# DedalusProject/dedalus

Measured on AMD Instinct MI355X. Metric: timesteps/sec, 3D Rayleigh-Benard 512x512x256 (Fourier x Fourier x Chebyshev, RK222), higher is better.
Workload: dtype f64; 1 GPU; 3-D Rayleigh-Benard IVP 512x512x256, dealias 3/2, RK222, fixed dt=0.001, Ra=2e6 Pr=1, example-script initial condition (fill_random seed 42); pencils=65536, rows_per_pencil_real=5156, parallelism=1 GPU

## Files before the change

### dedalus_amd/core/solvers.py

```python

import time

import os

import numpy as np

from . import operators as ops
from . import timesteppers as ts_mod
from .evaluator import Evaluator, SystemBuffer, _full_sep
from .field import Field
from .ivp_common import IVPLifecycle
from .polyop import flatten
from .problems import LinCtx

import logging
logger = logging.getLogger(__name__)


class SolverBase:
    def __init__(self, problem, **kw):
        self.problem = problem
        self.dist = dist = problem.dist
        self.ex = dist.executor
        self.variables = list(problem.variables)
# ... 816 lines not shown
            elif any(v.domain.by_axis[ax] is not None for ax in sep):
                return False
        return True

    def _enable_state_tiling(self):
        self.x_tiled = 0
        if not self._state_tiling_ok():
            return
        ex = self.ex
        mode = 2 if os.environ.get("DDH_X_TILED", "1") == "2" else 1
        self.sync_state_to_device()
        tmp = ex.empty((self.R, self.nx, self.ny))
        ex.tile_rows(self.X, tmp, self.R, self.nx, self.ny, True, self.R if mode == 2 else 0)
        ex.copy(self.X, tmp)
        del tmp
        sb = self.sysbuf
        sb.tiled = int(self.ny)
        sb.banded = int(self.R) if mode == 2 else 0
        for info in self.var_info:
            sb.ranges.append((info["row0"], info["rows"]))
            sb.valid[info["row0"]] = False
            if info["aliased"]:
                v = info["field"]
                v._tiled, v._nrows = sb, info["rows"]
                v._c = sb.state_rows(info["row0"], info["rows"])
        self.pack.set_state_tiled(mode)
        self.x_tiled = int(self.ny)
        self.x_banded = sb.banded

    def state_natural(self):
        return self.sysbuf.natural(self.ex)

    def rhs_tiling(self, lus):
        if getattr(self, "_rhs_tiling_problem", None) is None:
            self._rhs_tiling_problem = self._rhs_tiling_of_problem()
        if not self._rhs_tiling_problem:
            return 0
        for lu in ([lus] if isinstance(lus, (int, np.integer)) else list(lus)):
            info = self.pack.lu_info(lu)
            if info["forward"] != "lean" or not info["real"]:
                return 0
        return self._rhs_tiling_problem

    def _rhs_tiling_of_problem(self):
        ex = self.ex
        if (os.environ.get("DDH_NO_RHS_TILING") is not None or not getattr(self.pack, "supports_tiled_rhs", False)
                or self.nf != 2 or self.nx % 8 or self.ny % 8 or self.F_direct is None or self.P_id is None
                or self.real_grading is None or self.nx * self.ny < int(os.environ.get("DDH_RHS_TILING_MIN", 4 * 16384))
                or not hasattr(ex, "tiled_forward_ok")):
            return 0
        if self.F_const is not None and np.any(np.asarray(self._F_const_index) % (self.nx * self.ny) != 0):
            return 0
        tr = self.dist.transformer
        for einfo, _scale in self.F_direct.values():
            edom = einfo["eq"]["domain"]
            pos, b, spec = tr._steps(edom, edom.dealias)[0]
            if pos != 0 or not ex.tiled_forward_ok(spec, b, self.nx * self.ny, self.ny):
                return 0
        return int(self.ny)

    def untile_rows(self, vec, banded=False):
        R, nx, ny = self.R, self.nx, self.ny
        if banded:
            return vec.reshape(nx // 8, R, ny // 8, 8, 8).permute(1, 0, 3, 2, 4).contiguous().reshape(R, nx, ny)
        v = vec.reshape(R, nx // 8, ny // 8, 8, 8)
        if hasattr(v, "permute"):
            return v.permute(0, 1, 3, 2, 4).contiguous().reshape(R, nx, ny)
        return np.ascontiguousarray(np.transpose(v, (0, 1, 3, 2, 4))).reshape(R, nx, ny)

    def solve(self, lu, rhs, out):
        if getattr(self, "modal", None) is not None:
            a, b = self._modal_lus[lu]
            self.modal.solve(a, b, [rhs], [1.0], out)
        elif self.P_id is None:
            self.pack.solve(lu, rhs, out)
        elif hasattr(self.pack, "solve_recombined"):
            Y = self.ex.empty((self.R, self.nx, self.ny))
            self.pack.solve_recombined(lu, [rhs], [1.0], self.P_id, Y, out)
        else:
            Y = self.ex.empty((self.R, self.nx, self.ny))
            self.pack.solve(lu, rhs, Y)
            self.pack.matvec(self.P_id, Y, out)
        if getattr(self, "solve_probe", None) is not None:
            self._probe_record(lu, rhs, out, path="ddh_pencil_solve_recombined (one materialised right-hand side)")

    def _probe_record(self, lu, rhs, out, path, skip_rows=None, terms=1, zero_rows=None):
        probe = self.solve_probe
        a, b = self._lu_params[lu]
        if getattr(self, "x_tiled", 0):
            out = self.untile_rows(out, banded=bool(getattr(self, "x_banded", 0)))
        rec = dict(a=a, b=b, path=path, terms=int(terms), zero_rows=bool(zero_rows), skip_rows=skip_rows is not None,
                   rhs=[self.gather_pencil(rhs, "equations", gx, gy) for gx, gy in probe["groups"]],
                   x=[self.gather_pencil(out, "variables", gx, gy) for gx, gy in probe["groups"]])
        if skip_rows is not None:
            rec["skipped"] = [self.gather_rows_mask(skip_rows, "variables", gx, gy) for gx, gy in probe["groups"]]
        probe["records"].append(rec)

    def zero_rows_host(self):
        if self.F_direct is None:
            return None
        mask = np.ones(self.R, dtype=np.uint8)
        mask[np.unique(np.asarray(self.M_tl.row))] = 0
        for einfo, _scale in self.F_direct.values():
            mask[einfo["row0"]:einfo["row0"] + einfo["rows"]] = 0
        if self.F_const is not None:
            mask[self._F_const_rows] = 0
        return mask

    def skip_rows_host(self):
        used = set()
        for einfo in self.eq_info:
            F = einfo["eq"]["F"]
            if F is not None and hasattr(F, "leaves"):
                used |= {id(f) for f in F.leaves()}
        mask = np.zeros(self.R, dtype=np.uint8)
        mcols = np.zeros(self.R, dtype=bool)
        mcols[np.unique(np.asarray(self.M_tl.col))] = True
        for info in self.var_info:
            r0, r1 = info["row0"], info["row0"] + info["rows"]
            if id(info["field"]) not in used and not mcols[r0:r1].any():
                mask[r0:r1] = 1
        return mask

    def _device_mask(self, mask):
        t = self.ex.torch
        return (t.as_tensor(mask, device=self.ex.dev.tdev), float(mask.mean()))

    def mx_f_zero_rows(self):
        if getattr(self, "_zrows", "unset") != "unset":
            return self._zrows
        self._zrows = None
        if not getattr(self.pack, "supports_zero_rows", False) or self.P_id is None:
            return None
        if os.environ.get("DDH_NO_ZERO_ROWS") is not None:
            return None
        mask = self.zero_rows_host()
        if mask is not None and mask.any():
            self._zrows = self._device_mask(mask)
        return self._zrows

    def intermediate_skip_rows(self):
        if getattr(self, "_skiprows", "unset") != "unset":
            return self._skiprows
        self._skiprows = None
        if not getattr(self.pack, "supports_zero_rows", False) or self.P_id is None or self.F_direct is None:
            return None
        if os.environ.get("DDH_NO_SKIP_ROWS") is not None:
            return None
        mask = self.skip_rows_host()
        if mask.any():
            self._skiprows = self._device_mask(mask)
        return self._skiprows

    def solve_lincomb(self, lu, xs, alphas, out, zero_rows=None, skip_rows=None, tiled=False):
        probe = getattr(self, "solve_probe", None)
        if getattr(self, "modal", None) is not None and probe is None and len(xs) <= self.modal.MAX_RHS_TERMS and not tiled:
            a, b = self._modal_lus[lu]
            self.modal.solve(a, b, xs, alphas, out)
            return
        if getattr(self, "modal", None) is not None:
            if tiled:
                raise RuntimeError("tile-major right-hand sides need the fused recombined solve")
            rhs = self.ex.empty((self.R, self.nx, self.ny))
            self.ex.lincomb(rhs, xs, alphas)
            self._last_rhs = rhs
            return self.solve(lu, rhs, out)
        if tiled and (self.P_id is None or not hasattr(self.pack, "solve_recombined") or len(xs) > self.pack.MAX_RHS_TERMS):
            raise RuntimeError("tile-major right-hand sides need the fused recombined solve")
        if len(xs) > self.pack.MAX_RHS_TERMS or not hasattr(self.pack, "solve_lincomb"):
            rhs = self.ex.empty((self.R, self.nx, self.ny))
            self.ex.lincomb(rhs, xs, alphas)
            self._last_rhs = rhs
            return self.solve(lu, rhs, out)
        rhs_rec = None
        if probe is not None:
            rhs_rec = self.ex.empty((self.R, self.nx, self.ny))
            self.ex.lincomb(rhs_rec, xs, alphas)
            if tiled:
                rhs_rec = self.untile_rows(rhs_rec)
            self._last_rhs = rhs_rec
        path = "ddh_pencil_solve_lincomb"
        if self.P_id is None:
            self.pack.solve_lincomb(lu, xs, alphas, out)
        elif hasattr(self.pack, "solve_recombined"):
            Y = self.ex.empty((self.R, self.nx, self.ny))
            if tiled:
                self.pack.solve_recombined(lu, xs, alphas, self.P_id, Y, out, zero_rows=zero_rows, skip_rows=skip_rows,
                                           tiled=True)
                path = "ddh_pencil_solve_recombined_tiled"
            elif zero_rows is not None or skip_rows is not None:
                self.pack.solve_recombined(lu, xs, alphas, self.P_id, Y, out, zero_rows=zero_rows, skip_rows=skip_rows)
                path = "ddh_pencil_solve_recombined_sparse"
            else:
                self.pack.solve_recombined(lu, xs, alphas, self.P_id, Y, out)
                path = "ddh_pencil_solve_recombined"
        else:
            Y = self.ex.empty((self.R, self.nx, self.ny))
            self.pack.solve_lincomb(lu, xs, alphas, Y)
            self.pack.matvec(self.P_id, Y, out)
        if probe is not None:
            skip_h = None
            if skip_rows is not None:
                skip_h = np.asarray(skip_rows[0].cpu().numpy() if hasattr(skip_rows[0], "cpu") else skip_rows[0], dtype=np.uint8)
            self._probe_record(lu, rhs_rec, out, path + " (%d fused terms%s%s)" % (
                len(xs), ", zero_rows" if zero_rows is not None else "", ", skip_rows" if skip_rows is not None else ""),
                skip_rows=skip_h, terms=len(xs), zero_rows=zero_rows is not None)
        if skip_rows is not None and os.environ.get("DDH_POISON_SKIPPED") is not None:
            t = self.ex.torch
            idx = t.nonzero(skip_rows[0]).flatten()
            if getattr(self, "x_banded", 0):
                out.reshape(self.nx // 8, self.R, -1)[:, idx] = float("nan")
            else:
                out.reshape(self.R, -1)[idx] = float("nan")

    def gather_pencil(self, vec, which, gx, gy=0):
        lx = gx - (self.dist._mx_offset if self.nf >= 1 else 0)
        cx = slice(2 * lx, 2 * lx + 2) if self.nf >= 1 else slice(0, 1)
        cy = slice(2 * gy, 2 * gy + 2) if self.nf >= 2 else slice(0, 1)
        slab = vec.reshape(self.R, self.nx, self.ny)[:, cx, cy]
        cell = np.array(self.ex.download(slab.contiguous() if hasattr(slab, "contiguous") else slab), dtype=float)
        cell = cell.reshape(self.R, cell.shape[-2], cell.shape[-1])
        if which != "variables" and self.eq_Tinv is not None:
            rows = self._eq_T_rows
            cell[rows] = (self.eq_Tinv[rows][:, rows] @ cell[rows].reshape(len(rows), -1)).reshape(cell[rows].shape)
        return self._gather_cell(cell, which, gx, gy)

    def gather_rows_mask(self, mask, which, gx, gy=0):
        wx = 2 if self.nf >= 1 else 1
        wy = 2 if self.nf >= 2 else 1
        cell = np.broadcast_to(np.asarray(mask, dtype=float)[:, None, None], (self.R, wx, wy))
        return self._gather_cell(cell, which, gx, gy) != 0

    def _gather_cell(self, cell, which, gx, gy):
        infos = self.var_info if which == "variables" else self.eq_info
        parts = []
        for info in infos:
            bits = info["bits"]
            if self.nf >= 1:
                sx = slice(0, 2) if (bits & 1) else (slice(0, 1) if gx == 0 else slice(0, 0))
            else:
                sx = slice(0, 1)
            if self.nf >= 2:
                sy = slice(0, 2) if (bits & 2) else (slice(0, 1) if gy == 0 else slice(0, 0))
            else:
                sy = slice(0, 1)
            blk = cell[info["row0"]:info["row0"] + info["rows"]].reshape(info["ncomp"], info["nz"], cell.shape[1], cell.shape[2])
            blk = blk[:, :, sx, sy].transpose(0, 2, 3, 1)
            if self.nf < 2:
                blk = blk[:, :, 0, :] if self.nf == 1 else blk[:, 0, 0, :]
            parts.append(np.ascontiguousarray(blk).ravel())
        return np.concatenate(parts)

    def factor(self, a, b, reuse=-1):
        if getattr(self, "modal", None) is not None:
            if reuse >= 0:
                lu = reuse
                self._modal_lus[lu] = (float(a), float(b))
            else:
                lu = len(self._modal_lus)
                self._modal_lus.append((float(a), float(b)))
            self.__dict__.setdefault("_lu_params", {})[lu] = (float(a), float(b))
            return lu
        self.factor_calls = getattr(self, "factor_calls", 0) + 1
        lu = self.pack.factor(self.MP_id, self.LP_id, a, b, self.row_perm, self.col_perm, self.n_interior,
                              self.kl, self.ku, self.row_axes, self.col_axes, reuse=reuse,
                              real=self.real_grading)
        if not hasattr(self, "_lu_params"):
            self._lu_params = {}
        self._lu_params[lu] = (float(a), float(b))
        self._block_inverses(lu, a, b)
        return lu

    def _block_inverse_plan(self, any_executor=False):
        if getattr(self, "_binv", None) is not None:
            return self._binv
        self._binv = False
        rg, n = self.real_grading, self.n_interior
        if not getattr(self, "allow_block_inverse", False):
            return False
        if os.environ.get("DDH_BLOCK_INVERSE", "1") == "0" or self.nf != 1 or rg is None or getattr(self.dist, "size", 1) > 1 or n < 128:
            return False
        if not any_executor and (getattr(self.ex, "name", "") != "hip" or not hasattr(self.pack, "set_block_inverse")):
            return False
        ns = self.n_blocks if (self.n_blocks > 1 and len(set(self.block_sizes)) == 1 and os.environ.get("DDH_SPLIT_THREADS", "1") != "0") else 1
        nh = n // ns
        ncells = self.nx // 2
        nb = self.R - n
        if nb and (np.any(self.row_axes[self.row_perm[n:]] & 1) or np.any(self.col_axes[self.col_perm[n:]] & 1)):
            return False
        ng = ncells * ns
        if ns * nh != n or nh > 1024 or ng * nh * nh * 8 > 2.5e9 or ng * (nh + 112) * (nh + 63) * 8 > 3e9:
            return False
        rinv, cinv = np.empty(self.R, dtype=np.int64), np.empty(self.R, dtype=np.int64)
        rinv[self.row_perm] = np.arange(self.R)
        cinv[self.col_perm] = np.arange(self.R)
        kx = np.asarray(self.pack.kx, dtype=np.float64)[:ncells]
        gmx = np.arange(ncells) + self.dist._mx_offset
        sel = []
        for mid in (rg["matM"], rg["matL"]):
            tl = self.pack.matrices[mid]
            i, j = rinv[tl.row], cinv[tl.col]
            ok = (i < n) & (j < n)
            if np.any(ok & (i // nh != j // nh)):
                return False
            sel.append((tl, i, j, ok))
        kl_b = max(int((i[ok] - j[ok]).max()) if ok.any() else 0 for (_, i, j, ok) in sel)
        ku_b = max(int((j[ok] - i[ok]).max()) if ok.any() else 0 for (_, i, j, ok) in sel)
        klT, kuT = max(ku_b, 0), max(kl_b, 0)
        if klT > 35 or klT + kuT > 96:
            return False
        W = klT + kuT + 1
        bands = []
        for (tl, i, j, ok) in sel:
            B = np.zeros((ng, nh, W))
            t = np.flatnonzero(ok)
            val = tl.coef[t].real[None, :] * kx[:, None] ** tl.ex[t].astype(float)[None, :]
            val = np.where((tl.dx[t] != 0)[None, :] & (gmx != 0)[:, None], 0.0, val)
            blk, ii, jj = i[t] // nh, i[t] % nh, j[t] % nh
            g = np.arange(ncells)[:, None] * ns + blk[None, :]
            np.add.at(B, (g, np.broadcast_to(jj, g.shape), np.broadcast_to(ii - jj + klT, g.shape)), val)
            bands.append(B)
        plan = type("BlockBandPlan", (), {})()
        plan.nl, plan.nmax, plan.kl, plan.ku, plan.mp, plan.nbc = ng, nh, klT, kuT, 0, 0
        plan.n = np.full(ng, nh, dtype=np.int32)
        plan.nbc_of = np.zeros(ng, dtype=np.int32)
        plan.T = np.zeros((ng, 1, 1))
        plan.P = np.zeros((ng, nh, 1))
        plan.MB, plan.LB = bands
        plan.row_index = plan.col_index = None
        self._binv = dict(plan=plan, ns=ns, nh=nh, ng=ng, ncells=ncells, dev=None, rhs=None, x={}, n_set=None)
        return self._binv

    def _drop_block_inverses(self, bi=None):
        bi = bi if isinstance(bi, dict) else getattr(self, "_binv", None)
        if isinstance(bi, dict):
            for k in list(bi["x"]):
                self.pack.set_block_inverse(k, None)
            bi["x"] = {}

    def _block_inverses(self, lu, a, b):
        bi = self._block_inverse_plan()
        if not bi:
            return
        ex, plan, ns, nh, ng = self.ex, bi["plan"], bi["ns"], bi["nh"], bi["ng"]
        self.pack.set_block_inverse(lu, None)
        info = self.pack.lu_info(lu)
        if info["nsplit"] != ns or info["rows_per_block"] != nh or not info["real"] or info["pair"]:
            self._drop_block_inverses(bi)
            self._binv = False
            return
        flagged = sorted(getattr(self.pack, "flagged", {}).get(lu, []))
        nb = self.R - self.n_interior
        if nb:
            k0 = np.flatnonzero(np.arange(bi["ncells"]) + self.dist._mx_offset == 0)
            if any(int(c) not in flagged for c in k0):
                return
        if bi["dev"] is None or bi["n_set"] != flagged:
            self._drop_block_inverses(bi)
            plan.n = np.full(ng, nh, dtype=np.int32)
            for cell in flagged:
                plan.n[cell * ns:(cell + 1) * ns] = 0
            rowoff = np.broadcast_to(np.arange(nh, dtype=np.int64)[None, :] * nh, (ng, nh))
            coloff = np.arange(ng, dtype=np.int64)[:, None] * (nh * nh) + np.arange(nh, dtype=np.int64)[None, :] * nh
            try:
                bi["dev"] = ex.make_ell_band(plan, 1, nh, ng, nh, [nh] * ng, offsets=(rowoff, coloff, 1))
            except Exception as e:
                logger.info("block inverses not available (%s): the sweeps stay" % (e,))
                self._binv = False
                return
            bi["rhs"] = ex.from_host(np.eye(nh))
            bi["n_set"] = flagged
            logger.info("LHS of %d pencils: explicit inverses of %d x %d diagonal blocks (%d rows), %.2f GB per factorization"
                        % (bi["ncells"], ng, ns, nh, ng * nh * nh * 8 / 1e9))
        if lu not in bi["x"]:
            if len(bi["x"]) >= 2:
                return
            bi["x"][lu] = (len(bi["x"]), ex.zeros((ng, nh, nh)))
        idx, x = bi["x"][lu]
        try:
            bi["dev"].factor(a, b, index=idx)
        except Exception as e:
            logger.warning("block inverses switched off (%s)" % (e,))
            self._drop_block_inverses(bi)
            self._binv = False
            return
        bi["dev"].solve(idx, bi["rhs"], x)
        if not self._block_inverse_residual_ok(bi, idx, x, a, b):
            self._drop_block_inverses(bi)
            self._binv = False
            return
        self.pack.set_block_inverse(lu, x)

    def _block_inverse_residual_ok(self, bi, idx, x, a, b, tol=1e-8):
        if os.environ.get("DDH_BLOCK_INVERSE_CHECK", "1") == "0":
            return True
        plan, nh = bi["plan"], bi["nh"]
        live = np.flatnonzero(plan.n > 0)
        if live.size == 0:
            return True
        worst = left = 0.0
        for g in sorted({int(live[0]), int(live[live.size // 2]), int(live[-1])}):
            band = a * plan.MB[g] + b * plan.LB[g]
            Bt = np.zeros((nh, nh))
            for d in range(band.shape[1]):
                off = d - plan.kl
                i = np.arange(max(0, -off), min(nh, nh - off))
                Bt[i, i + off] = band[i, d]
            Xg = self.ex.download(x[g])
            scale = max(1.0, float(np.abs(Bt).max()))
            worst = max(worst, float(np.abs(Bt @ Xg - np.eye(nh)).max()) / scale)
            left = max(left, float(np.abs(Xg @ Bt - np.eye(nh)).max()))
        bi["residual"], bi["left_residual"] = worst, left
        if not (worst <= tol):
            logger.warning("explicit block inverses: ||B^T X - I|| = %.1e > %.0e, the sweeps stay" % (worst, tol))
            return False
        return True


def _two_colour(n, row, col, label):
    from collections import deque
    adj_r = [[] for _ in range(n)]
    adj_c = [[] for _ in range(n)]
    seen = {}
    for r, c, l in zip(row.tolist(), col.tolist(), np.asarray(label).tolist()):
        key = (r, c)
        if key in seen:
            if seen[key] != l:
                return None
            continue
        seen[key] = l
        adj_r[r].append((c, l))
        adj_c[c].append((r, l))
    xr = np.full(n, -1, dtype=int)
    xc = np.full(n, -1, dtype=int)
    for start in range(n):
        if xr[start] != -1 or not adj_r[start]:
            continue
        xr[start] = 0
        dq = deque([("r", start)])
        while dq:
            kind, i = dq.popleft()
            if kind == "r":
                for c, l in adj_r[i]:
                    want = (l - xr[i]) % 2
                    if xc[c] == -1:
                        xc[c] = want
                        dq.append(("c", c))
                    elif xc[c] != want:
                        return None
            else:
                for r, l in adj_c[i]:
                    want = (l - xc[i]) % 2
                    if xr[r] == -1:
                        xr[r] = want
                        dq.append(("r", r))
                    elif xr[r] != want:
                        return None
    xr[xr == -1] = 0
    xc[xc == -1] = 0
    return xr, xc


def _matrix_times_termlist(T, tl):
    from ..pencilpack import TermList
    if tl.nterms == 0:
        return tl
    T = T.tocsc()
    ident = np.ones(T.shape[0], dtype=bool)
    coo = T.tocoo()
    off = (coo.row != coo.col) | (coo.data != 1.0)
    ident[coo.row[off]] = False
    ident[coo.col[off]] = False
    plain = ident[tl.row]
    parts = [[tl.row[plain]], [tl.col[plain]], [tl.coef[plain]], [tl.ex[plain]], [tl.ey[plain]], [tl.dx[plain]], [tl.dy[plain]]]
    for t in np.flatnonzero(~plain):
        c = T.getcol(int(tl.row[t])).tocoo()
        n = c.nnz
        parts[0].append(c.row); parts[1].append(np.full(n, tl.col[t])); parts[2].append(c.data * tl.coef[t])
        for k, name in enumerate(("ex", "ey", "dx", "dy")):
            parts[3 + k].append(np.full(n, getattr(tl, name)[t]))
    out = TermList(tl.nrows, tl.ncols, *[np.concatenate(x) for x in parts])
    if (~plain).any():
        out = out.consolidated(0.0)
        rowmax = np.zeros(tl.nrows)
        np.maximum.at(rowmax, out.row, np.abs(out.coef))
        keep = ident[out.row] | (np.abs(out.coef) > 1e-14 * rowmax[out.row])
        out = TermList(out.nrows, out.ncols, out.row[keep], out.col[keep], out.coef[keep], out.ex[keep], out.ey[keep],
                       out.dx[keep], out.dy[keep])
    return out


def _termlist_times_matrix(tl, P, cutoff=1e-12):
    from scipy import sparse
    from ..pencilpack import TermList
    if tl.nterms == 0:
        return tl
    key = np.stack([tl.ex, tl.ey, tl.dx, tl.dy], axis=1).astype(np.int64)
    uniq, inv = np.unique(key, axis=0, return_inverse=True)
    inv = inv.ravel()
    rows, cols, coefs, exs = [], [], [], []
    for u in range(len(uniq)):
        sel = inv == u
        A = sparse.coo_matrix((tl.coef[sel], (tl.row[sel], tl.col[sel])), shape=(tl.nrows, tl.ncols)).tocsr()
        AP = (A @ P).tocoo()
        keep = np.abs(AP.data) > cutoff * (np.abs(AP.data).max() if AP.nnz else 1.0)
        rows.append(AP.row[keep]); cols.append(AP.col[keep]); coefs.append(AP.data[keep])
        exs.append(np.tile(uniq[u], (int(keep.sum()), 1)))
    e = np.concatenate(exs)
    return TermList(tl.nrows, tl.ncols, np.concatenate(rows), np.concatenate(cols), np.concatenate(coefs),
                    e[:, 0], e[:, 1], e[:, 2], e[:, 3])


class InitialValueSolver(IVPLifecycle, SolverBase):

    def __init__(self, problem, timestepper, enforce_real_cadence=100, warmup_iterations=10, **kw):
        t0 = time.time()
        SolverBase.__init__(self, problem, **kw)
        self._enable_state_tiling()
        self.sim_time_field = problem.time
        self._sim_time = 0.0
        self._init_lifecycle(enforce_real_cadence, warmup_iterations)
        if isinstance(timestepper, str):
            timestepper = ts_mod.schemes[timestepper]
        self.allow_block_inverse = True
        self.timestepper = timestepper(self)
        self.setup_time = time.time() - t0
        self.total_modes = self.R * self.nx * self.ny
        state_ids = {id(v) for v in self.variables}
        rhs_fields, opaque = set(), False
        for eq in self.equations:
            F = eq["F"]
            if F is None or isinstance(F, (int, float, complex)):
                continue
            if hasattr(F, "leaves"):
                rhs_fields |= {id(f) for f in F.leaves() if not getattr(f, "_is_number", False)}
            else:
                opaque = True
        if not opaque and rhs_fields <= state_ids:
            self.step_graph_auto_modes = 1 << 22
        self.handlers = []
        from .output import OutputEvaluator
        self.evaluator = OutputEvaluator(self)
        self._step_hooks = [self.evaluator.step_hook]

    @property
    def sim_time(self):
        return self._sim_time

    @sim_time.setter
    def sim_time(self, t):
        self._sim_time = float(t)
        self.sim_time_field["g"] = float(t)

    def _hermitian_round_trip(self, f):
        if self.dist.size > 1 and any(b is None for b in f.domain.by_axis):
            return
        scales = f.scales
        f.require_grid_space(f.domain.dealias)
        f.require_coeff_space()
        f.change_scales(scales)


class LinearBoundaryValueSolver(SolverBase):

    _lu = None

    def solve(self, rebuild_matrices=False):
        self.sync_state_to_device()
        if getattr(self, "_F_lbvp", None) is None:
            self._F_lbvp = self.ex.empty((self.R, self.nx, self.ny))
        F = self._F_lbvp
# ... 6 lines not shown
```

### dedalus_amd/core/timesteppers.py

```python

import math
from collections import deque

import numpy as np

schemes = {}


def add_scheme(cls):
    schemes[cls.__name__] = cls
    return cls


def _fd_weights(nodes, x0, deriv):
    nodes = np.asarray(nodes, dtype=np.longdouble) - np.longdouble(x0)
    n = len(nodes)
    V = np.vander(nodes, n, increasing=True).T
    rhs = np.zeros(n, dtype=np.longdouble)
    rhs[deriv] = math.factorial(deriv)
    return _solve_ld(V, rhs)


def _solve_ld(A, b):
    A = np.array(A, dtype=np.longdouble)
    b = np.array(b, dtype=np.longdouble)
    n = len(b)
    for k in range(n):
        p = k + int(np.argmax(np.abs(A[k:, k])))
        if p != k:
            A[[k, p]] = A[[p, k]]
            b[[k, p]] = b[[p, k]]
        for i in range(k + 1, n):
            m = A[i, k] / A[k, k]
            A[i, k:] -= m * A[k, k:]
            b[i] -= m * b[k]
    x = np.zeros(n, dtype=np.longdouble)
    for k in range(n - 1, -1, -1):
        x[k] = (b[k] - A[k, k + 1:] @ x[k + 1:]) / A[k, k]
    return x.astype(np.float64)


def _times(timesteps, n):
    t = [0.0]
    for j in range(n):
        t.append(t[-1] - timesteps[j])
    return t



class _SolveMixin:
    _RHS = None

    @property
    def RHS(self):
        if self._RHS is None:
            s = self.solver
            self._RHS = s.ex.zeros((s.R, s.nx, s.ny))
        return self._RHS

    def _solve_combination(self, xs, al, lu, zero_rows=None, skip_rows=None, tiled=False):
        s = self.solver
        if hasattr(s, "solve_lincomb"):
            if tiled:
                s.solve_lincomb(lu, xs, al, s.X, zero_rows=zero_rows, skip_rows=skip_rows, tiled=True)
            elif zero_rows is not None or skip_rows is not None:
                s.solve_lincomb(lu, xs, al, s.X, zero_rows=zero_rows, skip_rows=skip_rows)
            else:
                s.solve_lincomb(lu, xs, al, s.X)
        else:
            s.ex.lincomb(self.RHS, xs, al)
            s.solve(lu, self.RHS, s.X)


class MultistepIMEX(_SolveMixin):
    stages = 1

    def __init__(self, solver):
        self.solver = solver
        ex, shape = solver.ex, (solver.R, solver.nx, solver.ny)
        self.dt = deque([0.0] * self.steps)
        self.MX = deque(ex.zeros(shape) for _ in range(self.amax))
        self.F = deque(ex.zeros(shape) for _ in range(self.cmax))
        if hasattr(solver, "_F_zeroed"):
            solver._F_zeroed = set()
        self._iteration = 0
        self._LHS_params = None
        self._lu = -1
        self._need_lx = False
        for it in range(self.steps + 1):
            _, b, _ = self.compute_coefficients([1.0] * self.steps, it)
            self._need_lx = self._need_lx or bool(np.any(np.asarray(b)[1:] != 0.0))
        self.LX = deque((ex.zeros(shape) if self._need_lx else None) for _ in range(self.bmax))

    def graph_phase(self, dt):
        if self._iteration < self.steps + 1 or any(h != dt for h in self.dt):
            return None
        period = int(np.lcm.reduce([len(self.MX), len(self.LX), len(self.F)]))
        return period, self._iteration % period

    def graph_snapshot(self):
        return (list(self.dt), self._iteration, list(self.MX), list(self.LX), list(self.F), self._LHS_params, self._lu)

    def graph_rollback(self, snap):
        dts, self._iteration, mx, lx, f, self._LHS_params, self._lu = snap
        self.dt, self.MX, self.LX, self.F = deque(dts), deque(mx), deque(lx), deque(f)

    def graph_advance(self, dt):
        self.dt.rotate()
        self.dt[0] = dt
        self._iteration += 1
        self.MX.rotate()
        self.LX.rotate()
        self.F.rotate()

    def step(self, dt, wall_time=None):
        s = self.solver
        ex, pack = s.ex, s.pack
        self.dt.rotate()
        self.dt[0] = dt
        a, b, c = self.compute_coefficients(list(self.dt), self._iteration)
        self._iteration += 1
        self.MX.rotate()
        self.LX.rotate()
        self.F.rotate()
        s.sync_state_to_device()
        pack.matvec(s.M_id, s.X, self.MX[0])
        if self._need_lx:
            pack.matvec(s.L_id, s.X, self.LX[0])
        s.evaluate_F(self.F[0], persistent=True)
        xs, al = [], []
        for j in range(1, len(c)):
            if c[j] != 0.0:
                xs.append(self.F[j - 1]); al.append(c[j])
        for j in range(1, len(a)):
            if a[j] != 0.0:
                xs.append(self.MX[j - 1]); al.append(-a[j])
        for j in range(1, len(b)):
            if b[j] != 0.0:
                xs.append(self.LX[j - 1]); al.append(-b[j])
        if (a[0], b[0]) != self._LHS_params:
            self._lu = s.factor(a[0], b[0], reuse=self._lu)
            self._LHS_params = (a[0], b[0])
        self._solve_combination(xs, al, self._lu)
        s.mark_state_current()
        s.sim_time = s.sim_time + dt


def _pad(v, n):
    out = np.zeros(n + 1)
    out[:len(v)] = v
    return out


@add_scheme
class CNAB1(MultistepIMEX):
    amax = bmax = cmax = steps = 1

    @classmethod
    def compute_coefficients(cls, timesteps, iteration):
        k0 = timesteps[0]
        a = _fd_weights(_times(timesteps, 1), 0.0, 1)
        return _pad(a, cls.amax), _pad([0.5, 0.5], cls.bmax), _pad([0.0, 1.0], cls.cmax)


@add_scheme
class SBDF1(MultistepIMEX):
    amax = bmax = cmax = steps = 1

    @classmethod
    def compute_coefficients(cls, timesteps, iteration):
        a = _fd_weights(_times(timesteps, 1), 0.0, 1)
        return _pad(a, cls.amax), _pad([1.0], cls.bmax), _pad([0.0, 1.0], cls.cmax)


def _adams_bashforth(timesteps, order):
    t = _times(timesteps, order)
    nodes = np.array(t[1:order + 1], dtype=np.longdouble)
    k = np.longdouble(timesteps[0])
    V = np.vander(nodes, order, increasing=True).T
    p = np.arange(order, dtype=np.longdouble)
    rhs = (np.longdouble(t[0]) ** (p + 1) - np.longdouble(t[1]) ** (p + 1)) / (p + 1) / k
    return np.concatenate([[0.0], _solve_ld(V, rhs)])


def _extrapolation(timesteps, order):
    t = _times(timesteps, order)
    w = _fd_weights(t[1:order + 1], t[0], 0)
    return np.concatenate([[0.0], w])


@add_scheme
class CNAB2(MultistepIMEX):
    amax = bmax = cmax = steps = 2

    @classmethod
    def compute_coefficients(cls, timesteps, iteration):
        if iteration < 1:
            a, b, c = CNAB1.compute_coefficients(timesteps, iteration)
            return _pad(a, 2), _pad(b, 2), _pad(c, 2)
        a = _fd_weights(_times(timesteps, 1), 0.0, 1)
        return _pad(a, 2), _pad([0.5, 0.5], 2), _pad(_adams_bashforth(timesteps, 2), 2)


@add_scheme
class MCNAB2(MultistepIMEX):
    amax = bmax = cmax = steps = 2

    @classmethod
    def compute_coefficients(cls, timesteps, iteration):
        if iteration < 1:
            a, b, c = CNAB1.compute_coefficients(timesteps, iteration)
            return _pad(a, 2), _pad(b, 2), _pad(c, 2)
        w = timesteps[0] / timesteps[1]
        a = _fd_weights(_times(timesteps, 1), 0.0, 1)
        b = [(8 + 1 / w) / 16, (7 - 1 / w) / 16, 1 / 16]
        return _pad(a, 2), _pad(b, 2), _pad(_adams_bashforth(timesteps, 2), 2)


class _SBDF(MultistepIMEX):
    @classmethod
    def _coeffs(cls, timesteps, order, size):
        a = _fd_weights(_times(timesteps, order), 0.0, 1)
        return _pad(a, size), _pad([1.0], size), _pad(_extrapolation(timesteps, order), size)


@add_scheme
class SBDF2(_SBDF):
    amax = bmax = cmax = steps = 2

    @classmethod
    def compute_coefficients(cls, timesteps, iteration):
        order = min(2, iteration + 1)
        return cls._coeffs(timesteps, order, 2)


@add_scheme
class CNLF2(MultistepIMEX):
    amax = bmax = cmax = steps = 2

    @classmethod
    def compute_coefficients(cls, timesteps, iteration):
        if iteration < 1:
            a, b, c = CNAB1.compute_coefficients(timesteps, iteration)
            return _pad(a, 2), _pad(b, 2), _pad(c, 2)
        t = _times(timesteps, 2)
        w = timesteps[0] / timesteps[1]
        a = _fd_weights(t, t[1], 1)
        b = [1 / w / 2, (1 - 1 / w) / 2, 1 / 2]
        return _pad(a, 2), _pad(b, 2), _pad([0.0, 1.0], 2)


@add_scheme
class SBDF3(_SBDF):
    amax = bmax = cmax = steps = 3

    @classmethod
    def compute_coefficients(cls, timesteps, iteration):
        order = min(3, iteration + 1)
        return cls._coeffs(timesteps, order, 3)


@add_scheme
class SBDF4(_SBDF):
    amax = bmax = cmax = steps = 4

    @classmethod
    def compute_coefficients(cls, timesteps, iteration):
        order = min(4, iteration + 1)
        return cls._coeffs(timesteps, order, 4)



class RungeKuttaIMEX(_SolveMixin):
    steps = 1

    def __init__(self, solver):
        import os
        self.solver = solver
        ex, shape = solver.ex, (solver.R, solver.nx, solver.ny)
        H = self.H
        self.MX0 = ex.zeros(shape)
        self.F = [ex.zeros(shape) for _ in range(self.stages)]
        if hasattr(solver, "_F_zeroed"):
            solver._F_zeroed = set()
        self._need_lx = [any(H[m, j] != 0.0 for m in range(j + 1, self.stages + 1)) for j in range(self.stages + 1)]
        self._direct = os.environ.get("DDH_RK_DIRECT_LX", "0") == "1"
        self.LX = [ex.zeros(shape) if (self._need_lx[j] and (self._direct or j == 0)) else None
                   for j in range(self.stages + 1)]
        self.MX = [None] + [ex.zeros(shape) if (self._need_lx[j] and not self._direct) else None
                            for j in range(1, self.stages + 1)]
        self._k = None
        self._lus = {}

    def step(self, dt, wall_time=None):
        s = self.solver
        ex, pack = s.ex, s.pack
        k = dt
        A, H, c = self.A, self.H, self.c
        if k != self._k:
            old = self._lus
            self._lus = {}
            reuse = list(old.values())
            for i in range(1, self.stages + 1):
                h = float(H[i, i])
                if h not in self._lus:
                    self._lus[h] = s.factor(1.0, k * h, reuse=(reuse.pop() if reuse else -1))
            self._k = k
        t0 = s.sim_time
        s.sync_state_to_device()
        own = dict(owned=True) if getattr(pack, "supports_zero_rows", False) else {}
        stamp = (tuple(self._lus.values()), getattr(pack, "variant_epoch", 0))
        if getattr(self, "_tiled_stamp", None) != stamp:
            tiled_now = 0
            if own and not self._direct and not any(v is not None for v in self.LX) and hasattr(s, "rhs_tiling"):
                tiled_now = s.rhs_tiling(self._lus.values())
            if getattr(self, "_tiled", None) is not None and bool(tiled_now) != bool(self._tiled):
                for buf in [self.MX0] + self.F + [v for v in self.MX if v is not None]:
                    ex.fill_zero(buf)
                s._F_zeroed = set(b.data_ptr() if hasattr(b, "data_ptr") else id(b) for b in self.F)
            self._tiled, self._tiled_stamp = tiled_now, stamp
        tiled = self._tiled
        if tiled:
            own = dict(owned=True, tiled=True)
        later = []
        defer_mv = bool(getattr(s, "overlaps_rhs_work", lambda: False)())
        (later.append if defer_mv else (lambda f: f()))(lambda: pack.matvec(s.M_id, s.X, self.MX0, **own))
        combs = {}
        for i in range(1, self.stages + 1):
            j = i - 1
            if self._need_lx[j]:
                if self._direct or j == 0:
                    mv = (lambda j=j: pack.matvec(s.L_id, s.X, self.LX[j]))
                else:
                    mv = (lambda j=j: pack.matvec(s.M_id, s.X, self.MX[j], **own))
                (later.append if defer_mv else (lambda f: f()))(mv)
            if later:
                s._overlap_work = list(later)
                del later[:]
            if tiled:
                s.evaluate_F(self.F[i - 1], persistent=True, tiled_row=tiled)
            else:
                s.evaluate_F(self.F[i - 1], persistent=True)
            comb = {("MX0",): 1.0}
            for j in range(i):
                if A[i, j] != 0.0:
                    comb[("F", j)] = comb.get(("F", j), 0.0) + k * A[i, j]
                if H[i, j] != 0.0:
                    if self._direct or j == 0:
                        comb[("LX", j)] = comb.get(("LX", j), 0.0) - k * H[i, j]
                    else:
                        r = H[i, j] / H[j, j]
                        for key, v in combs[j].items():
                            comb[key] = comb.get(key, 0.0) - r * v
                        comb[("MX", j)] = comb.get(("MX", j), 0.0) + r
            combs[i] = comb
            vec = {"MX0": lambda q: self.MX0, "F": lambda q: self.F[q], "LX": lambda q: self.LX[q], "MX": lambda q: self.MX[q]}
            xs = [vec[key[0]](key[1] if len(key) > 1 else None) for key, v in comb.items() if v != 0.0]
            al = [v for v in comb.values() if v != 0.0]
            zrows = None
            if not any(key[0] == "LX" and v != 0.0 for key, v in comb.items()) and hasattr(s, "mx_f_zero_rows"):
                zrows = s.mx_f_zero_rows()
            skip = None
            if i < self.stages and not self._direct and hasattr(s, "intermediate_skip_rows"):
                skip = s.intermediate_skip_rows()
            self._solve_combination(xs, al, self._lus[float(H[i, i])], zero_rows=zrows, skip_rows=skip, tiled=bool(tiled))
            s.mark_state_current()
            s.sim_time = t0 + k * c[i]


@add_scheme
class RK111(RungeKuttaIMEX):
    stages = 1
    c = np.array([0.0, 1.0])
    A = np.array([[0.0, 0.0], [1.0, 0.0]])
    H = np.array([[0.0, 0.0], [0.0, 1.0]])


@add_scheme
class RK222(RungeKuttaIMEX):
    stages = 2
    _g = 1.0 - np.sqrt(0.5)
    _d = 1.0 - 1.0 / (2.0 * _g)
    c = np.array([0.0, _g, 1.0])
    A = np.array([[0.0, 0.0, 0.0], [_g, 0.0, 0.0], [_d, 1.0 - _d, 0.0]])
    H = np.array([[0.0, 0.0, 0.0], [0.0, _g, 0.0], [0.0, 1.0 - _g, _g]])


@add_scheme
class RK443(RungeKuttaIMEX):
    stages = 4
    c = np.array([0.0, 1 / 2, 2 / 3, 1 / 2, 1.0])
    A = np.array([[0, 0, 0, 0, 0],
                  [1 / 2, 0, 0, 0, 0],
                  [11 / 18, 1 / 18, 0, 0, 0],
                  [5 / 6, -5 / 6, 1 / 2, 0, 0],
                  [1 / 4, 7 / 4, 3 / 4, -7 / 4, 0]], dtype=float)
    H = np.array([[0, 0, 0, 0, 0],
                  [0, 1 / 2, 0, 0, 0],
                  [0, 1 / 6, 1 / 2, 0, 0],
                  [0, -1 / 2, 1 / 2, 1 / 2, 0],
                  [0, 3 / 2, -3 / 2, 1 / 2, 1 / 2]], dtype=float)


@add_scheme
class RKSMR(RungeKuttaIMEX):
    stages = 3
    _al = (29 / 96, -3 / 40, 1 / 6)
    _be = (37 / 160, 5 / 24, 1 / 6)
    _ga = (8 / 15, 5 / 12, 3 / 4)
    _ze = (0.0, -17 / 60, -5 / 12)
    c = np.array([0.0, 8 / 15, 2 / 3, 1.0])
    A = np.zeros((4, 4))
    H = np.zeros((4, 4))
    for _i in range(1, 4):
        for _j in range(1, _i + 1):
            A[_i, _j - 1] += _ga[_j - 1]
            if _j >= 2:
                A[_i, _j - 2] += _ze[_j - 1]
            H[_i, _j - 1] += _al[_j - 1]
            H[_i, _j] += _be[_j - 1]
    del _i, _j


class RKGFY(RungeKuttaIMEX):
    stages = 2
    c = np.array([0.0, 1.0, 1.0])
    A = np.array([[0, 0, 0], [1, 0, 0], [0.5, 0.5, 0]], dtype=float)
    H = np.array([[0, 0, 0], [0.5, 0.5, 0], [0.5, 0, 0.5]], dtype=float)
```

### dedalus_amd/csrc/ddh_pencil.hip

```cpp
#include "ddh_common.h"

#include <algorithm>
#include <cmath>
#include <cstdlib>
#include <type_traits>

namespace ddh {

constexpr int KLMAX = 16;
constexpr int NBMAX = 8;

struct PencilDev {
    int nf;
    int S;
    int nrows;
    long nx, ny;
    long ncx, ncy;
    long ncells;
    long G;
    long mx_offset;
    const double *kx, *ky;
    int xtile;
};

struct MatDev {
    int nrows_out;
    int nterms;
    const int *rowptr;
    const int *col;
    const double2 *coef;
    const unsigned *expo;
    const int *order;
    const double *band;
    const int *base;
};
constexpr int MV_W = 5;

struct PostSolve {
    int nz;
    int nbands;
    int off[4];
    const double *bands;
};

struct Matrix {
    MatDev dev;
    std::vector<int> row_h, col_h;
    std::vector<double2> coef_h;
    std::vector<unsigned> expo_h;
    void *d_rowptr = nullptr, *d_col = nullptr, *d_coef = nullptr, *d_expo = nullptr, *d_order = nullptr;
    void *d_band = nullptr, *d_base = nullptr;
};

struct LuDev {
    int n, nb, N, kl, ku, W, BW;
    int real;
    long GL;
    long nblk;
    int rows_aw;
    int pk, pk63;
    int kpad;
    void *Aw;
    void *Ab;
    unsigned char *piv;
    unsigned char *flag;
    double2 *scratch;
    const int *rowperm, *colperm;
    const unsigned char *row_axes, *col_axes;
    const unsigned char *row_code, *col_code;
    const double *pband;
    int nsplit, nh;
    long Gp;
    int pair;
    const int *wrow;
    const long *vcell;
    const int *vslot;
    const long *slot_cell;
    const int *rowperm2, *colperm2;
};

constexpr int PBW = 12;

struct LuFactor {
    LuDev dev;
    size_t bytes = 0;
    void *d_rowperm = nullptr, *d_colperm = nullptr, *d_raxes = nullptr, *d_caxes = nullptr;
    void *d_rcode = nullptr, *d_ccode = nullptr;
    int nflag = 0;
    std::vector<long> flag_cells;
    void *d_flag_cells = nullptr;
    void *d_inv = nullptr;
    void *d_dense_rhs = nullptr;
    std::vector<int> colperm_h;
    std::vector<unsigned char> ccode_h;
    void *d_rhs_tmp = nullptr;
    const double *d_binv = nullptr;
    void *d_pband = nullptr;
    void *d_vcell = nullptr, *d_vslot = nullptr, *d_rowperm2 = nullptr, *d_colperm2 = nullptr;
    void *d_wrow = nullptr;
    std::vector<long> slot_cells_h;
    void *d_slot_cell = nullptr;
    int pband_mat = -1;
};

struct PencilPack : HandleBase {
    PencilDev dev;
    void *d_kx = nullptr, *d_ky = nullptr;
    std::vector<Matrix *> mats;
    std::vector<LuFactor *> lus;
    std::vector<PostSolve> posts;
    std::vector<void *> post_mem;
    int coop_mode = 1, coop_fwd = -1, coop_cb = -1;
    std::vector<int> pair_rows, pair_cols;
    long pair_min = 0;
    int row_blocks = 1;
    std::vector<double> kx_h, ky_h;
    ~PencilPack() override;
};

static void free_lu(LuFactor *lu) {
    if (!lu) return;
    (void)hipFree(lu->dev.Aw);
    (void)hipFree(lu->dev.Ab);
    (void)hipFree(lu->dev.piv);
    (void)hipFree(lu->dev.flag);
    (void)hipFree(lu->dev.scratch);
    (void)hipFree(lu->d_rowperm);
    (void)hipFree(lu->d_colperm);
    (void)hipFree(lu->d_raxes);
    (void)hipFree(lu->d_caxes);
    (void)hipFree(lu->d_rcode);
    (void)hipFree(lu->d_ccode);
    (void)hipFree(lu->d_flag_cells);
    (void)hipFree(lu->d_inv);
    (void)hipFree(lu->d_dense_rhs);
    (void)hipFree(lu->d_pband);
    (void)hipFree(lu->d_rhs_tmp);
    (void)hipFree(lu->d_vcell);
    (void)hipFree(lu->d_vslot);
    (void)hipFree(lu->d_slot_cell);
    (void)hipFree(lu->d_rowperm2);
    (void)hipFree(lu->d_colperm2);
    (void)hipFree(lu->d_wrow);
    delete lu;
}

PencilPack::~PencilPack() {
    (void)hipFree(d_kx);
    (void)hipFree(d_ky);
    for (auto m : mats) {
        (void)hipFree(m->d_rowptr);
        (void)hipFree(m->d_col);
        (void)hipFree(m->d_coef);
        (void)hipFree(m->d_expo);
        if (m->d_order) (void)hipFree(m->d_order);
        if (m->d_band) (void)hipFree(m->d_band);
        if (m->d_base) (void)hipFree(m->d_base);
        delete m;
    }
    for (auto l : lus) free_lu(l);
    for (auto m : post_mem) (void)hipFree(m);
}

__device__ __forceinline__ double2 cmul(double2 a, double2 b) {
    return make_double2(a.x * b.x - a.y * b.y, a.x * b.y + a.y * b.x);
}
__device__ __forceinline__ void cfma(double2 &acc, double2 a, double2 b) {
    acc.x += a.x * b.x - a.y * b.y;
    acc.y += a.x * b.y + a.y * b.x;
}
__device__ __forceinline__ void cfms(double2 &acc, double2 a, double2 b) {
    acc.x -= a.x * b.x - a.y * b.y;
    acc.y -= a.x * b.y + a.y * b.x;
}
__device__ __forceinline__ double cabs2(double2 a) { return a.x * a.x + a.y * a.y; }
__device__ __forceinline__ double2 cinv(double2 a) {
    const double d = 1.0 / (a.x * a.x + a.y * a.y);
    return make_double2(a.x * d, -a.y * d);
}
__device__ __forceinline__ double ipow(double k, unsigned e) {
    double r = 1.0, b = k;
    if (e & 1u) r *= b;
    b *= b;
    if (e & 2u) r *= b;
    b *= b;
    if (e & 4u) r *= b;
    return r;
}

template <bool REAL> struct El;
template <> struct El<false> {
    typedef double2 T;
    static __device__ __forceinline__ T zero() { return make_double2(0.0, 0.0); }
    static __device__ __forceinline__ T one() { return make_double2(1.0, 0.0); }
    static __device__ __forceinline__ T mul(T a, T b) { return cmul(a, b); }
    static __device__ __forceinline__ T inv(T a) { return cinv(a); }
    static __device__ __forceinline__ double abs2(T a) { return cabs2(a); }
    static __device__ __forceinline__ bool is_zero(T a) { return a.x == 0.0 && a.y == 0.0; }
    static __device__ __forceinline__ void fms(T &acc, T m, T v) { cfms(acc, m, v); }
    static __device__ __forceinline__ void add(T &acc, double2 v) { acc.x += v.x; acc.y += v.y; }
    static __device__ __forceinline__ void fms2(double2 &acc, T m, double2 v) { cfms(acc, m, v); }
    static __device__ __forceinline__ void fma2(double2 &acc, T m, double2 v) { cfma(acc, m, v); }
    static __device__ __forceinline__ double2 mul2(double2 a, T m) { return cmul(a, m); }
    static __device__ __forceinline__ T scale(T a, double f) { return make_double2(a.x * f, a.y * f); }
};
template <> struct El<true> {
    typedef double T;
    static __device__ __forceinline__ T zero() { return 0.0; }
    static __device__ __forceinline__ T one() { return 1.0; }
    static __device__ __forceinline__ T mul(T a, T b) { return a * b; }
    static __device__ __forceinline__ T inv(T a) { return 1.0 / a; }
    static __device__ __forceinline__ double abs2(T a) { return a * a; }
    static __device__ __forceinline__ bool is_zero(T a) { return a == 0.0; }
    static __device__ __forceinline__ void fms(T &acc, T m, T v) { acc -= m * v; }
    static __device__ __forceinline__ void add(T &acc, double2 v) { acc += v.x; }
    static __device__ __forceinline__ void fms2(double2 &acc, T m, double2 v) { acc.x -= m * v.x; acc.y -= m * v.y; }
    static __device__ __forceinline__ void fma2(double2 &acc, T m, double2 v) { acc.x += m * v.x; acc.y += m * v.y; }
    static __device__ __forceinline__ double2 mul2(double2 a, T m) { return make_double2(a.x * m, a.y * m); }
    static __device__ __forceinline__ T scale(T a, double f) { return a * f; }
};

typedef unsigned ddh_u4v __attribute__((ext_vector_type(4)));
typedef unsigned ddh_u2v __attribute__((ext_vector_type(2)));
__device__ __forceinline__ __amdgpu_buffer_rsrc_t wave_rsrc(const void *first_lane_ptr) {
    const unsigned long long a = (unsigned long long)first_lane_ptr;
    const unsigned lo = __builtin_amdgcn_readfirstlane((unsigned)a);
    const unsigned hi = __builtin_amdgcn_readfirstlane((unsigned)(a >> 32));
    void *base = (void *)(((unsigned long long)hi << 32) | lo);
    return __builtin_amdgcn_make_buffer_rsrc(base, 0, 0xffffffff, 0x00020000);
}
__device__ __forceinline__ unsigned wave_lane_off(const void *lane_ptr) {
    const unsigned long long a = (unsigned long long)lane_ptr;
    const unsigned lo = __builtin_amdgcn_readfirstlane((unsigned)a);
    const unsigned hi = __builtin_amdgcn_readfirstlane((unsigned)(a >> 32));
    return (unsigned)(a - (((unsigned long long)hi << 32) | lo));
}
__device__ __forceinline__ double2 bload16(__amdgpu_buffer_rsrc_t r, unsigned lane_off, unsigned uni_off) {
    const ddh_u4v q = __builtin_amdgcn_raw_buffer_load_b128(r, lane_off, uni_off, 0);
    return make_double2(__hiloint2double((int)q.y, (int)q.x), __hiloint2double((int)q.w, (int)q.z));
}
__device__ __forceinline__ double bload8(__amdgpu_buffer_rsrc_t r, unsigned lane_off, unsigned uni_off) {
    const ddh_u2v q = __builtin_amdgcn_raw_buffer_load_b64(r, lane_off, uni_off, 0);
    return __hiloint2double((int)q.y, (int)q.x);
}

__device__ __forceinline__ long lu_eoff(const LuDev &L, int e) {
    return ((long)e << 6) - (long)(L.pk63 * (e & 1));
}
__device__ __forceinline__ long lu_aw(const LuDev &L, long gl, int row, int d) {
    return ((((gl >> 6) * (long)L.rows_aw + row) * L.BW) << 6) + lu_eoff(L, d + L.kpad) + ((gl & 63) << (L.pk ? 1 : 0));
}
__device__ __forceinline__ long lu_ab(const LuDev &L, long gl, int col, int rb) {
    return ((((gl >> 6) * (long)L.N + col) * L.nb + rb) << 6) + (gl & 63);
}
__device__ __forceinline__ long lu_pv(const LuDev &L, long gl, int row) {
    return (((gl >> 6) * (long)L.rows_aw + row) << 6) + (gl & 63);
}

struct CellCtx {
    long mx, my;
    long gmx;
    double kx, ky;
};

__device__ __forceinline__ CellCtx cell_ctx(const PencilDev &P, long cell) {
    CellCtx c;
    if (P.nf == 2) {
        c.mx = cell / P.ncy;
        c.my = cell % P.ncy;
    } else {
        c.mx = cell;
        c.my = 0;
    }
    c.gmx = c.mx + P.mx_offset;
    c.kx = (P.nf >= 1) ? P.kx[c.mx] : 0.0;
    c.ky = (P.nf == 2) ? P.ky[c.my] : 0.0;
    return c;
}

struct SysId {
    long cell, gl, G;
    int s;
    bool partner, ok;
};
template <bool REAL>
__device__ __forceinline__ SysId sys_id(const PencilDev &P, const LuDev &L, long g) {
    SysId id;
    id.partner = false;
    id.G = P.G;
    id.ok = g < P.G;
    id.cell = id.ok ? g / P.S : 0;
    id.s = (int)(g % P.S);
    if (L.pair) {
        const int vs = L.vslot[id.cell];
        id.gl = vs >> 1;
        id.partner = (vs & 1) != 0;
// ... 1339 lines not shown
        if (code & 1) v = make_double2(v.y, -v.x);
        return v;
    };

    double2 w[KLT + 1];
#pragma unroll
    for (int d = 0; d <= KLT; ++d) w[d] = make_double2(0.0, 0.0);
#pragma unroll 1
    for (int t = 0; t <= KLT; ++t) {
        const double2 v = (row0 + t < row1) ? load_row(row0 + t) : make_double2(0.0, 0.0);
#pragma unroll
        for (int d = 0; d < KLT; ++d) w[d] = w[d + 1];
        w[KLT] = v;
    }
    double2 gb[NBT];
#pragma unroll
    for (int rb = 0; rb < NBT; ++rb) gb[rb] = make_double2(0.0, 0.0);
#pragma unroll 1
    for (int t = 0; t < NBT; ++t) {
        const double2 v = (t < nb && blk == 0) ? load_row(n + t) : make_double2(0.0, 0.0);
#pragma unroll
        for (int rb = 0; rb + 1 < NBT; ++rb) gb[rb] = gb[rb + 1];
        gb[NBT - 1] = v;
    }
    double m[PD][KLT], ab[PD][NBT];
    int pv[PD];
    double2 raw[PD][NT];
#pragma unroll
    for (int d = 0; d < PD; ++d) {
        pv[d] = 0;
#pragma unroll
        for (int i = 0; i < KLT; ++i) m[d][i] = 0.0;
#pragma unroll
        for (int rb = 0; rb < NBT; ++rb) ab[d][rb] = 0.0;
#pragma unroll
        for (int t = 0; t < NT; ++t) raw[d][t] = make_double2(0.0, 0.0);
    }
    const long cell_off = rhs.tiled ? tile_offset(2 * c.mx + s, 2 * c.my, P.ny) : (2 * c.mx + s) * P.ny + 2 * c.my;
    const double *pt[NT];
    double at[NT];
#pragma unroll
    for (int t = 0; t < NT; ++t) {
        pt[t] = t < rhs.n ? rhs.p[t] : rhs.p[0];
        at[t] = t < rhs.n ? rhs.a[t] : 0.0;
    }
    auto request = [&](int jrow, double *mm, double *aa, int &p, double2 *q) {
        const unsigned jr = (unsigned)((jrow < row1 ? jrow : row1 - 1) - row0);
        const unsigned mo_j = jr * row_step8;
        p = pvp[(long)jr << 6];
#pragma unroll
        for (int i = 0; i < KLT; ++i) mm[i] = *reinterpret_cast<const double *>(awl + (mo_j + md[i]));
        const double *abj = abp + (long)jr * ab_step;
#pragma unroll
        for (int rb = 0; rb < NBT; ++rb) aa[rb] = abj[rb << 6];
        const int nxt = jrow + KLT + 1;
        const long off = (long)my_perm[nxt < row1 ? nxt : row1 - 1] * plane + cell_off;
#pragma unroll
        for (int t = 0; t < NT; ++t) q[t] = *reinterpret_cast<const double2 *>(pt[t] + off);
        __builtin_amdgcn_sched_barrier(0);
    };
    auto entering = [&](int jrow, const double2 *q) -> double2 {
        const int nxt = jrow + KLT + 1;
        if (nxt >= row1 || s_zero[nxt]) return make_double2(0.0, 0.0);
        double2 v;
        if (rhs.n == 1 && !rhs.tiled) {
            const double2 mine = q[0];
            double2 other;
            other.x = __shfl_xor(mine.x, 1);
            other.y = __shfl_xor(mine.y, 1);
            v = s == 0 ? make_double2(mine.x - other.y, mine.y + other.x) : make_double2(other.x + mine.y, other.y - mine.x);
            if (rhs.a[0] != 1.0) v = make_double2(rhs.a[0] * v.x, rhs.a[0] * v.y);
        } else {
            double2 mine = make_double2(0.0, 0.0);
#pragma unroll
            for (int t = 0; t < NT; ++t) {
                mine.x += at[t] * q[t].x;
                mine.y += at[t] * q[t].y;
            }
            double2 other;
            other.x = __shfl_xor(mine.x, 1);
            other.y = __shfl_xor(mine.y, 1);
            v = s == 0 ? make_double2(mine.x - other.y, mine.y + other.x) : make_double2(other.x + mine.y, other.y - mine.x);
        }
        if (conjq) v.y = -v.y;
        const unsigned char code = s_code[nxt];
        if ((code & 2) && s == 1) v = make_double2(-v.x, -v.y);
        if (code & 1) v = make_double2(v.y, -v.x);
        return v;
    };
    auto step = [&](const double *mm, const double *aa, int p, double2 rnew) {
        double2 yj = w[0];
#pragma unroll
        for (int d = 1; d <= KLT; ++d) {
            if (d == p) {
                yj = w[d];
                w[d] = w[0];
            }
        }
        *scr = yj;
        scr += G;
#pragma unroll
        for (int i = 1; i <= KLT; ++i) {
            w[i].x -= mm[i - 1] * yj.x;
            w[i].y -= mm[i - 1] * yj.y;
        }
#pragma unroll
        for (int rb = 0; rb < NBT; ++rb) {
            gb[rb].x -= aa[rb] * yj.x;
            gb[rb].y -= aa[rb] * yj.y;
        }
#pragma unroll
        for (int d = 0; d < KLT; ++d) w[d] = w[d + 1];
        w[KLT] = rnew;
    };
#pragma unroll
    for (int d = 0; d < PD; ++d) request(row0 + d, m[d], ab[d], pv[d], raw[d]);
    int j = row0;
    for (; j + PD - 1 < row1; j += PD) {
#pragma unroll
        for (int d = 0; d < PD; ++d) {
            const double2 rnew = entering(j + d, raw[d]);
            step(m[d], ab[d], pv[d], rnew);
            request(j + d + PD, m[d], ab[d], pv[d], raw[d]);
        }
    }
#pragma unroll
    for (int d = 0; d < PD; ++d)
        if (j + d < row1) step(m[d], ab[d], pv[d], entering(j + d, raw[d]));
    if (L.nsplit > 1) {
#pragma unroll
        for (int r = 0; r < NBT; ++r)
            if (r < nb) L.scratch[(long)(n + nb + blk * nb + r) * G + g] = gb[r];
        return;
    }
    const double *Ab = (const double *)L.Ab;
#pragma unroll
    for (int r = 0; r < NBT; ++r) {
        if (r < nb) {
            double2 acc = make_double2(0.0, 0.0);
#pragma unroll
            for (int cidx = 0; cidx < NBT; ++cidx)
                if (cidx < nb) El<true>::fma2(acc, Ab[lu_ab(L, id.gl, n + cidx, r)], gb[cidx]);
            L.scratch[(long)(n + r) * G + g] = acc;
            double2 v = acc;
            const unsigned char code = s_code[N + r];
            if (code & 1) v = make_double2(-v.y, v.x);
            if ((code & 2) && s == 1) v = make_double2(-v.x, -v.y);
            if (conjq) v.y = -v.y;
            store_sys<NF>(xout, plane, my_perm[N + r], P, c, s, v);
        }
    }
}

template <int NF, int WT, bool REAL, bool PREF, bool PFUSE = false, int MINW = 1>
__global__ void __launch_bounds__(256, MINW)
solve_backward_kernel(PencilDev P, LuDev L, double *__restrict__ xout, const double *__restrict__ pband,
                      const unsigned char *__restrict__ skip) {
    typedef typename El<REAL>::T E;
    extern __shared__ int s_lds[];
    const int n = L.n, nb = L.nb, kl = L.kl, W = L.W;
    int *s_perm = s_lds;
    int *s_perm2 = s_lds + (L.pair ? n : 0);
    unsigned char *s_code = (unsigned char *)(s_perm2 + n);
    unsigned char *s_skip = s_code + n;
    unsigned char *s_nq = s_skip + n;
    for (int i = threadIdx.x; i < n; i += blockDim.x) {
        s_perm[i] = L.colperm[i];
        if (L.pair) s_perm2[i] = L.colperm2[i];
        s_code[i] = REAL ? L.col_code[i] : 0;
        s_skip[i] = skip ? (skip[L.colperm[i]] && (!L.pair || skip[L.colperm2[i]])) : 0;
        if (REAL) {
            const int full = (WT + 2) / 2;
            const int need = L.wrow ? (L.wrow[i] + 2) >> 1 : full;
            s_nq[i] = (unsigned char)(need < full ? need : full);
        }
    }
    __syncthreads();
    const int blk = (REAL && L.nsplit > 1) ? __builtin_amdgcn_readfirstlane((int)(((long)blockIdx.x * blockDim.x) / L.Gp)) : 0;
    const long g = (long)blockIdx.x * blockDim.x + threadIdx.x - (long)blk * L.Gp;
    const int row0 = (REAL && L.nsplit > 1) ? blk * L.nh : 0, row1 = (REAL && L.nsplit > 1) ? row0 + L.nh : n;
    const SysId id = sys_id<REAL>(P, L, g);
    if (!id.ok) return;
    const int s = id.s;
    const CellCtx c = cell_ctx(P, id.cell);
    const long G = id.G;
    const long gl = id.gl;
    const int *my_perm = id.partner ? s_perm2 : s_perm;
    const bool conjq = id.partner && s == 1;
    const E *Aw = (const E *)L.Aw;
    const long plane = P.nx * P.ny;

    double2 win[WT];
#pragma unroll
    for (int d = 0; d < WT; ++d) {
        win[d] = make_double2(0.0, 0.0);
        if (d < nb && row1 == n) win[d] = L.scratch[(long)(n + d) * G + g];
    }
    E ua[WT + 1], ub[WT + 1];
    double pa[PBW], pb[PBW];
    double2 ya = make_double2(0.0, 0.0), yb = ya;
#pragma unroll
    for (int d = 0; d < PBW; ++d) pa[d] = pb[d] = 0.0;
#pragma unroll
    for (int d = 0; d <= WT; ++d) ua[d] = ub[d] = El<REAL>::zero();
    constexpr bool FULL = REAL;
    const E *const ur0 = Aw + lu_aw(L, gl, 0, kl);
    const long ur_stride = (long)L.BW << 6;
    const double2 *const y0 = L.scratch + g;
    const __amdgpu_buffer_rsrc_t ur_rs = wave_rsrc(ur0);
    const unsigned ur_lane = wave_lane_off(ur0);
    const __amdgpu_buffer_rsrc_t y_rs = wave_rsrc(y0);
    const unsigned y_lane = wave_lane_off(y0);
    const unsigned ur_row8 = (unsigned)L.BW << 9, y_row16 = (unsigned)(G * (long)sizeof(double2));
    auto fetch = [&](int j, E *u, double2 &y, double *pr) {
        if constexpr (REAL) y = bload16(y_rs, y_lane, (unsigned)j * y_row16);
        else y = y0[(long)j * G];
        if (PFUSE) {
            const double *prow = pband + (long)j * PBW;
#pragma unroll
            for (int d = 0; d < PBW; ++d) pr[d] = prow[d];
        }
        const E *Ur = ur0 + (long)j * ur_stride;
        if constexpr (REAL) {
            const unsigned urow = (unsigned)j * ur_row8;
            constexpr int NQMIN = (WT >= 13) ? 6 : (WT + 2) / 2;
            const int nq = __builtin_amdgcn_readfirstlane((int)s_nq[j]);
#pragma unroll
            for (int q = 0; 2 * q <= WT; ++q) {
                double2 uu = make_double2(0.0, 0.0);
                if (q < NQMIN || q < nq) uu = bload16(ur_rs, ur_lane, urow + (unsigned)(q << 10));
                u[2 * q] = uu.x;
                if (2 * q + 1 <= WT) u[2 * q + 1] = uu.y;
            }
        } else {
#pragma unroll
            for (int d = 0; d <= WT; ++d)
                if (FULL || d <= W) u[d] = Ur[(long)d << 6];
        }
        __builtin_amdgcn_sched_barrier(0);
    };
    auto emit = [&](int j, double2 v) {
        if (s_skip[j]) return;
        if (REAL) {
            const unsigned char code = s_code[j];
            if (code & 1) v = make_double2(-v.y, v.x);
            if ((code & 2) && s == 1) v = make_double2(-v.x, -v.y);
        }
        if (conjq) v.y = -v.y;
        store_sys<NF>(xout, plane, my_perm[j], P, c, s, v);
    };
    auto row_even = [&](int j, const E *u, double2 y, const double *pr) -> double2 {
        double2 acc = y;
#pragma unroll
        for (int d = 0; d < WT; ++d)
            if (FULL || d < W) El<REAL>::fms2(acc, u[d + 1], win[d]);
        const double2 xj = El<REAL>::mul2(acc, u[0]);
        double2 v = xj;
        if (PFUSE) {
#pragma unroll
            for (int d = 0; d < PBW; ++d)
                if (d < WT) { v.x += pr[d] * win[d].x; v.y += pr[d] * win[d].y; }
        }
        emit(j, v);
        return xj;
    };
    auto row_odd = [&](int j, const E *u, double2 y, double2 xprev, const double *pr) {
        double2 acc = y;
        El<REAL>::fms2(acc, u[1], xprev);
#pragma unroll
        for (int d = 1; d < WT; ++d)
            if (FULL || d < W) El<REAL>::fms2(acc, u[d + 1], win[d - 1]);
        const double2 xj = El<REAL>::mul2(acc, u[0]);
        double2 v = xj;
        if (PFUSE) {
            v.x += pr[0] * xprev.x;
            v.y += pr[0] * xprev.y;
#pragma unroll
            for (int d = 1; d < PBW; ++d)
                if (d - 1 < WT) { v.x += pr[d] * win[d - 1].x; v.y += pr[d] * win[d - 1].y; }
        }
        emit(j, v);
#pragma unroll
        for (int d = WT - 1; d > 1; --d) win[d] = win[d - 2];
        win[1] = xprev;
        win[0] = xj;
    };
    int j = row1 - 1;
    if (PREF) {
        if (j >= row0) fetch(j, ua, ya, pa);
        while (j >= row0 + 1) {
            fetch(j - 1, ub, yb, pb);
            const double2 xe = row_even(j, ua, ya, pa);
            if (j - 2 >= row0) fetch(j - 2, ua, ya, pa);
            row_odd(j - 1, ub, yb, xe, pb);
            j -= 2;
        }
        if (j == row0) row_even(row0, ua, ya, pa);
    } else {
        while (j >= row0 + 1) {
            fetch(j, ua, ya, pa);
            const double2 xe = row_even(j, ua, ya, pa);
            fetch(j - 1, ua, ya, pa);
            row_odd(j - 1, ua, ya, xe, pa);
            j -= 2;
        }
        if (j == row0) {
            fetch(row0, ua, ya, pa);
            row_even(row0, ua, ya, pa);
        }
    }
}

template <int WT, int PD>
__global__ void __launch_bounds__(256, 1)
solve_backward_deep_kernel(PencilDev P, LuDev L, double *__restrict__ xout, const double *__restrict__ pband,
                           const unsigned char *__restrict__ skip) {
    constexpr int NF = 2;
    static_assert(PD >= 2 && PD % 2 == 0, "rows are processed in pairs");
    extern __shared__ int s_lds[];
    const int n = L.n, nb = L.nb, kl = L.kl;
    int *s_perm = s_lds;
    int *s_perm2 = s_lds + (L.pair ? n : 0);
    unsigned char *s_code = (unsigned char *)(s_perm2 + n);
    unsigned char *s_skip = s_code + n;
    for (int i = threadIdx.x; i < n; i += blockDim.x) {
        s_perm[i] = L.colperm[i];
        if (L.pair) s_perm2[i] = L.colperm2[i];
        s_code[i] = L.col_code[i];
        s_skip[i] = skip ? (skip[L.colperm[i]] && (!L.pair || skip[L.colperm2[i]])) : 0;
    }
    __syncthreads();
    const int blk = (L.nsplit > 1) ? __builtin_amdgcn_readfirstlane((int)(((long)blockIdx.x * blockDim.x) / L.Gp)) : 0;
    const long g = (long)blockIdx.x * blockDim.x + threadIdx.x - (long)blk * L.Gp;
    const int row0 = (L.nsplit > 1) ? blk * L.nh : 0, row1 = (L.nsplit > 1) ? row0 + L.nh : n;
    const SysId id = sys_id<true>(P, L, g);
    if (!id.ok) return;
    const int s = id.s;
    const CellCtx c = cell_ctx(P, id.cell);
    const long G = id.G;
    const int *my_perm = id.partner ? s_perm2 : s_perm;
    const bool conjq = id.partner && s == 1;
    const long plane = P.nx * P.ny;

    double2 win[WT];
#pragma unroll
    for (int d = 0; d < WT; ++d) {
        win[d] = make_double2(0.0, 0.0);
        if (d < nb && row1 == n) win[d] = L.scratch[(long)(n + d) * G + g];
    }
    constexpr int NQ = (WT + 2) / 2;
    ddh_u4v u[PD][NQ];
    double pr[PD][PBW];
    ddh_u4v yv[PD];
    const double *const ur0 = (const double *)L.Aw + lu_aw(L, id.gl, 0, kl);
    const double2 *const y0 = L.scratch + g;
    const __amdgpu_buffer_rsrc_t ur_rs = wave_rsrc(ur0);
    const unsigned ur_lane = wave_lane_off(ur0);
    const __amdgpu_buffer_rsrc_t y_rs = wave_rsrc(y0);
    const unsigned y_lane = wave_lane_off(y0);
    const unsigned ur_row8 = (unsigned)L.BW << 9, y_row16 = (unsigned)(G * (long)sizeof(double2));
    auto lo = [](const ddh_u4v &q) -> double { return __hiloint2double((int)q.y, (int)q.x); };
    auto hi = [](const ddh_u4v &q) -> double { return __hiloint2double((int)q.w, (int)q.z); };
    auto fetch = [&](int j, ddh_u4v *uu, ddh_u4v &y, double *p) {
        y = __builtin_amdgcn_raw_buffer_load_b128(y_rs, y_lane, (unsigned)j * y_row16, 0);
        const double *prow = pband + (long)j * PBW;
#pragma unroll
        for (int d = 0; d < PBW; ++d) p[d] = prow[d];
        const unsigned urow = (unsigned)j * ur_row8;
#pragma unroll
        for (int q = 0; q < NQ; ++q) uu[q] = __builtin_amdgcn_raw_buffer_load_b128(ur_rs, ur_lane, urow + (unsigned)(q << 10), 0);
        __builtin_amdgcn_sched_barrier(0);
    };
    auto emit = [&](int j, double2 v) {
        if (s_skip[j]) return;
        const unsigned char code = s_code[j];
        if (code & 1) v = make_double2(-v.y, v.x);
        if ((code & 2) && s == 1) v = make_double2(-v.x, -v.y);
        if (conjq) v.y = -v.y;
        store_sys<NF>(xout, plane, my_perm[j], P, c, s, v);
    };
    auto ent = [&](const ddh_u4v *uu, int e) -> double { return (e & 1) ? hi(uu[e >> 1]) : lo(uu[e >> 1]); };
    auto row_even = [&](int j, const ddh_u4v *uu, const ddh_u4v &yr, const double *p) -> double2 {
        double2 acc = make_double2(lo(yr), hi(yr));
#pragma unroll
        for (int d = 0; d < WT; ++d) El<true>::fms2(acc, ent(uu, d + 1), win[d]);
        const double2 xj = El<true>::mul2(acc, ent(uu, 0));
        double2 v = xj;
#pragma unroll
        for (int d = 0; d < PBW; ++d)
            if (d < WT) { v.x += p[d] * win[d].x; v.y += p[d] * win[d].y; }
        emit(j, v);
        return xj;
    };
    auto row_odd = [&](int j, const ddh_u4v *uu, const ddh_u4v &yr, double2 xprev, const double *p) {
        double2 acc = make_double2(lo(yr), hi(yr));
        El<true>::fms2(acc, ent(uu, 1), xprev);
#pragma unroll
        for (int d = 1; d < WT; ++d) El<true>::fms2(acc, ent(uu, d + 1), win[d - 1]);
        const double2 xj = El<true>::mul2(acc, ent(uu, 0));
        double2 v = xj;
        v.x += p[0] * xprev.x;
        v.y += p[0] * xprev.y;
#pragma unroll
        for (int d = 1; d < PBW; ++d)
            if (d - 1 < WT) { v.x += p[d] * win[d - 1].x; v.y += p[d] * win[d - 1].y; }
        emit(j, v);
#pragma unroll
        for (int d = WT - 1; d > 1; --d) win[d] = win[d - 2];
        win[1] = xprev;
        win[0] = xj;
    };
    int j = row1 - 1;
#pragma unroll
    for (int d = 0; d < PD; ++d) fetch(max(j - d, row0), u[d], yv[d], pr[d]);
    for (; j - (PD - 1) >= row0; j -= PD) {
#pragma unroll
        for (int d = 0; d < PD; d += 2) {
            const double2 xe = row_even(j - d, u[d], yv[d], pr[d]);
            fetch(max(j - d - PD, row0), u[d], yv[d], pr[d]);
            row_odd(j - d - 1, u[d + 1], yv[d + 1], xe, pr[d + 1]);
            fetch(max(j - d - 1 - PD, row0), u[d + 1], yv[d + 1], pr[d + 1]);
        }
    }
#pragma unroll
    for (int d = 0; d < PD; d += 2) {
        if (j - d - 1 >= row0) {
            const double2 xe = row_even(j - d, u[d], yv[d], pr[d]);
            row_odd(j - d - 1, u[d + 1], yv[d + 1], xe, pr[d + 1]);
        } else if (j - d >= row0) {
            row_even(j - d, u[d], yv[d], pr[d]);
        }
    }
}

// ... 244 lines not shown
            pu[slot][t] = u_ptr[(dd << 6) - pk63 * (dd & 1)];
        }
        const bool adv = jj > row0;
        u_ptr -= adv ? aw_rs : 0;
        y_ptr -= adv ? G : 0;
    };
#pragma unroll
    for (int r = 0; r < PD; ++r) issue(row1 - 1 - r, r);
#define DDH_COOP_BWD_ROW(r, j)                                                                                     \
    {                                                                                                              \
        E u[TT];                                                                                                   \
        const int ej = (h - (j) - 1) & (CB - 1);                                                                   \
        _Pragma("unroll") for (int t = 0; t < TT; ++t) u[t] = (1 + ej + CB * t <= W) ? pu[r][t] : El<REAL>::zero(); \
        const E u0 = pu0[r];                                                                                       \
        const double2 y = py[r];                                                                                   \
        issue((j) - PD, r);                                                                                    \
        double2 acc = make_double2(0.0, 0.0);                                                                      \
        _Pragma("unroll") for (int t = 0; t < TT; ++t) El<REAL>::fma2(acc, u[t], xr[t]);                           \
        acc.x = group_sum<CB>(acc.x);                                                                                  \
        acc.y = group_sum<CB>(acc.y);                                                                                  \
        const double2 xj = El<REAL>::mul2(make_double2(y.x - acc.x, y.y - acc.y), u0);                             \
        double2 v = xj;                                                                                            \
        if (REAL) {                                                                                                \
            const unsigned char code = s_code[j];                                                                  \
            if (code & 1) v = make_double2(-v.y, v.x);                                                             \
            if ((code & 2) && s == 1) v = make_double2(-v.x, -v.y);                                                \
        }                                                                                                          \
        store_sys<NF, CB>(xout, plane, s_perm[j], P, c, s, v);       \
        if ((((j) - h) & (CB - 1)) == 0) {                       \
            _Pragma("unroll") for (int t = TT - 1; t > 0; --t) xr[t] = xr[t - 1];                                  \
            xr[0] = xj;                                                                                            \
        }                                                                                                          \
    }
    int jt0 = 0;
    const int nrows = row1 - row0;
    for (; jt0 + PD <= nrows; jt0 += PD) {
#pragma unroll
        for (int r = 0; r < PD; ++r) DDH_COOP_BWD_ROW(r, row1 - 1 - (jt0 + r))
    }
#pragma unroll
    for (int r = 0; r < PD; ++r)
        if (jt0 + r < nrows) DDH_COOP_BWD_ROW(r, row1 - 1 - (jt0 + r))
#undef DDH_COOP_BWD_ROW
}

template <int NF>
__global__ void __launch_bounds__(256)
dense_gather_kernel(PencilDev P, LuDev L, const long *__restrict__ cells, int ncellsf,
                    const RhsSrc rhs, double2 *__restrict__ out) {
    const long t = (long)blockIdx.x * blockDim.x + threadIdx.x;
    const long per = (long)L.N * P.S;
    if (t >= per * ncellsf) return;
    const long f = t / per;
    const int i = (int)((t % per) / P.S);
    const int s = (int)(t % P.S);
    const CellCtx c = cell_ctx(P, cells[f]);
    const double2 v = load_sys<NF>(rhs, P.nx * P.ny, L.rowperm[i], P, c, s);
    out[(f * P.S + s) * L.N + i] = v;
}

__global__ void __launch_bounds__(256)
dense_apply_kernel(int N, const double2 *__restrict__ inv, const double2 *__restrict__ rhs, double2 *__restrict__ x) {
    const int sys = blockIdx.y;
    const int row = blockIdx.x * 4 + (threadIdx.x >> 6);
    const int lane = threadIdx.x & 63;
    if (row >= N) return;
    const double2 *a = inv + ((long)sys * N + row) * N;
    const double2 *b = rhs + (long)sys * N;
    double2 acc = make_double2(0.0, 0.0);
    for (int k = lane; k < N; k += 64) cfma(acc, a[k], b[k]);
    for (int off = 32; off > 0; off >>= 1) {
        acc.x += __shfl_down(acc.x, off);
        acc.y += __shfl_down(acc.y, off);
    }
    if (lane == 0) x[(long)sys * N + row] = acc;
}

template <int NF>
__global__ void __launch_bounds__(256)
dense_scatter_kernel(PencilDev P, LuDev L, const long *__restrict__ cells, int ncellsf,
                     const double2 *__restrict__ xin, double *__restrict__ xout, int apply_p) {
    const long t = (long)blockIdx.x * blockDim.x + threadIdx.x;
    const long per = (long)L.N * P.S;
    if (t >= per * ncellsf) return;
    const long f = t / per;
    const int i = (int)((t % per) / P.S);
    const int s = (int)(t % P.S);
    const CellCtx c = cell_ctx(P, cells[f]);
    const double2 *xs = xin + (f * P.S + s) * L.N;
    double2 v = xs[i];
    if (apply_p && L.pband && i < L.n) {
        const double *pr = L.pband + (long)i * PBW;
        for (int d = 1; d <= PBW; ++d)
            if (i + d < L.n) { v.x += pr[d - 1] * xs[i + d].x; v.y += pr[d - 1] * xs[i + d].y; }
    }
    store_sys<NF>(xout, P.nx * P.ny, L.colperm[i], P, c, s, v);
}

template <typename T>
static int upload_vec(void **dptr, const T *src, size_t count) {
    DDH_HIP(hipMalloc(dptr, count * sizeof(T) + 16));
    if (count) DDH_HIP(hipMemcpy(*dptr, src, count * sizeof(T), hipMemcpyHostToDevice));
    return 0;
}

__global__ void __launch_bounds__(1024)
blockinv_solve_kernel(PencilDev P, LuDev L, const RhsSrc rhs, const double *__restrict__ binv, double *__restrict__ yout) {
    extern __shared__ double2 s_rb[];
    const int nh = L.nh, ns = L.nsplit;
    const long cell = blockIdx.x / ns;
    const int blk = (int)(blockIdx.x - cell * ns);
    if (L.flag[cell]) return;
    const CellCtx c = cell_ctx(P, cell);
    const long plane = P.nx * P.ny;
    const int row0 = blk * nh, tid = threadIdx.x, NT = blockDim.x;
    for (int i = tid; i < nh; i += NT) {
        const int phys = L.rowperm[row0 + i];
        double2 v = make_double2(0.0, 0.0);
        if (!(rhs.zrow && rhs.zrow[phys])) v = load_sys<1>(rhs, plane, phys, P, c, 0);
        if (L.row_code[row0 + i] & 1) v = make_double2(v.y, -v.x);
        s_rb[i] = v;
    }
    __syncthreads();
    const double *B = binv + (size_t)blockIdx.x * nh * nh;
    for (int i = tid; i < nh; i += NT) {
        double2 acc = make_double2(0.0, 0.0);
        const double *bi = B + i;
        int k = 0;
        for (; k + 8 <= nh; k += 8) {
            double b[8];
#pragma unroll
            for (int q = 0; q < 8; ++q) b[q] = bi[(size_t)(k + q) * nh];
#pragma unroll
            for (int q = 0; q < 8; ++q) {
                const double2 r = s_rb[k + q];
                acc.x += b[q] * r.x;
                acc.y += b[q] * r.y;
            }
        }
        for (; k < nh; ++k) {
            const double b = bi[(size_t)k * nh];
            const double2 r = s_rb[k];
            acc.x += b * r.x;
            acc.y += b * r.y;
        }
        double2 v = acc;
        if (L.col_code[row0 + i] & 1) v = make_double2(-v.y, v.x);
        store_sys<1>(yout, plane, L.colperm[row0 + i], P, c, 0, v);
    }
    if (blk == 0)
        for (int r = tid; r < L.nb; r += NT) store_sys<1>(yout, plane, L.colperm[L.n + r], P, c, 0, make_double2(0.0, 0.0));
}

template <int NF>
static int finish_solve(PencilPack *pp, LuFactor *lu, const RhsSrc &rhs, double *x, hipStream_t s, int apply_p) {
    const PencilDev &P = pp->dev;
    const LuDev &d = lu->dev;
    if (lu->nflag) {
        if (!lu->d_inv) return fail("pencil_solve: flagged pencils need ddh_pencil_set_dense_inverse first");
        const int nsys = lu->nflag * P.S;
        double2 *drhs = (double2 *)lu->d_dense_rhs;
        double2 *dx = drhs + (size_t)nsys * d.N;
        const long work = (long)lu->nflag * d.N * P.S;
        const unsigned gb = (unsigned)((work + 255) / 256);
        hipLaunchKernelGGL(dense_gather_kernel<NF>, dim3(gb), dim3(256), 0, s, P, d, (const long *)lu->d_flag_cells,
                           lu->nflag, rhs, drhs);
        hipLaunchKernelGGL(dense_apply_kernel, dim3((unsigned)((d.N + 3) / 4), (unsigned)nsys), dim3(256), 0, s, d.N,
                           (const double2 *)lu->d_inv, (const double2 *)drhs, dx);
        hipLaunchKernelGGL(dense_scatter_kernel<NF>, dim3(gb), dim3(256), 0, s, P, d, (const long *)lu->d_flag_cells,
                           lu->nflag, (const double2 *)dx, x, apply_p);
        DDH_HIP(hipGetLastError());
    }
    return 0;
}

static int forward_window(int kl) { return kl <= 6 ? 6 : (kl <= 12 ? 12 : 16); }
static int backward_window(int W) { return W <= 17 ? 17 : (W <= 32 ? 32 : (W <= 34 ? 34 : (W <= 48 ? 48 : 64))); }

static bool lean_forward_ok(const LuDev &d) {
    return d.real && d.n > 0 && d.kpad + d.kl == forward_window(d.kl) && d.rows_aw >= d.n + forward_window(d.kl) &&
           d.kl <= 12 && d.nb <= 2;
}

static bool sweep_deep(const LuDev &d) {
    static const int env = getenv("DDH_SWEEP_DEEP") ? atoi(getenv("DDH_SWEEP_DEEP")) : -1;
    if (!d.real || d.n <= 0) return false;
    if (env >= 0) return env != 0;
    return (long)d.nsplit * d.Gp <= 2L * 1024 * 64;
}

static unsigned deep_block(long threads) {
    if (threads / 256 >= 256) return 256u;
    return threads / 128 >= 256 ? 128u : 64u;
}

enum class FwdSweep {
    coop,
    deep,
    lean_occ4,
    lean,
    general
};
enum class BwdSweep {
    none,
    coop,
    deep,
    fused_occ4,
    fused,
    plain
};
struct SweepPlan {
    FwdSweep fwd;
    int fwd_kl, fwd_nb;
    bool border_finish;
    BwdSweep bwd;
    int bwd_w;
    int cb, tt;
    bool fuse_p;
    dim3 fwd_grid, fwd_block, bwd_grid, bwd_block;
    size_t lds_f, lds_b;
    bool lean_forward() const { return fwd == FwdSweep::deep || fwd == FwdSweep::lean_occ4 || fwd == FwdSweep::lean; }
};

static SweepPlan sweep_plan(const PencilPack *pp, const LuDev &d, int nterms, bool want_p) {
    const PencilDev &P = pp->dev;
    const int NF = P.nf, W = d.W;
    SweepPlan pl{};
    const size_t per_entry = d.pair ? 9 : 5;
    pl.lds_f = (size_t)(d.N + d.nb) * (per_entry + 1) + 16;
    pl.lds_b = (size_t)(d.n > 0 ? d.n : 1) * (per_entry + 2) + 16;
    const unsigned blocks = (unsigned)((P.G + 255) / 256);
    const long threads = (long)d.nsplit * d.Gp;
    const unsigned blocks_split = (unsigned)((threads + 255) / 256);
    auto coop_grid = [&](int lanes) {
        return (d.real && d.nsplit > 1) ? (unsigned)(threads / (256 / lanes)) : (unsigned)((P.G + (256 / lanes) - 1) / (256 / lanes));
    };

    const int coop_mode = pp->coop_mode;
    const bool coop_auto = coop_mode == 1 && NF > 0;
    bool coop_fwd = coop_mode == 2 || (coop_auto && P.G <= 16384);
    int cb = 0;
    if (coop_mode == 2 || (coop_auto && P.G <= 1024)) cb = 16;
    else if (coop_auto && P.G <= 16384) cb = 4;
    if (coop_auto && d.nsplit > 1 && P.G > 4096) {
        coop_fwd = false;
        cb = 0;
    }
    if (pp->coop_fwd >= 0) coop_fwd = pp->coop_fwd != 0;
    if (pp->coop_cb >= 0) cb = pp->coop_cb;
    if (NF == 0 || d.kl >= CH || d.nb > 8) coop_fwd = false;
    if (NF == 0 || (cb != 4 && cb != 16)) cb = 0;
    if (cb && (W + cb - 1) / cb > (cb == 4 ? 12 : 3)) cb = 0;
    if (d.n <= 0 || d.pair) {
        coop_fwd = false;
        cb = 0;
    }

    pl.fwd_grid = dim3(blocks);
    pl.fwd_block = dim3(256);
    if (coop_fwd) {
        pl.fwd = FwdSweep::coop;
        pl.fwd_nb = d.nb <= 2 ? 2 : 8;
        pl.fwd_grid = dim3(coop_grid(CH));
        pl.border_finish = d.real && d.nsplit > 1 && d.nb > 0;
    } else if (NF == 2 && lean_forward_ok(d)) {
        const bool w6 = forward_window(d.kl) == 6;
        pl.fwd_kl = w6 ? 6 : 12;
        pl.fwd_nb = w6 && d.nb <= 1 ? 1 : 2;
        pl.fwd_grid = dim3(blocks_split);
        if (w6 && d.nb == 1 && nterms >= 1 && nterms <= 4 && sweep_deep(d)) {
            pl.fwd = FwdSweep::deep;
            pl.fwd_block = dim3(deep_block(threads));
            pl.fwd_grid = dim3(blocks_split * (256 / pl.fwd_block.x));
        } else if (w6 && d.nsplit > 1 && d.nb <= 1) {
            pl.fwd = FwdSweep::lean_occ4;
        } else {
            pl.fwd = FwdSweep::lean;
        }
        pl.border_finish = d.nsplit > 1 && d.nb > 0;
    } else {
        pl.fwd = FwdSweep::general;
        pl.fwd_kl = d.kl <= 12 ? 12 : 16;
        pl.fwd_nb = d.nb <= 2 ? 2 : 8;
    }

    pl.bwd_grid = dim3(blocks_split);
    pl.bwd_block = dim3(256);
    if (cb) {
        pl.bwd = BwdSweep::coop;
        pl.cb = cb;
        const int tt = (W + cb - 1) / cb;
        pl.tt = cb == 16 ? (tt <= 2 ? 2 : 3) : (tt <= 9 ? 9 : 12);
        pl.bwd_grid = dim3(coop_grid(cb));
    } else if (d.n <= 0) {
        pl.bwd = BwdSweep::none;
    } else if (NF == 2 && want_p && d.real && d.pband != nullptr && W <= 48) {
        pl.fuse_p = true;
        pl.bwd_w = backward_window(W);
        if (W <= 17 && sweep_deep(d)) {
            pl.bwd = BwdSweep::deep;
            pl.bwd_block = dim3(deep_block(threads));
            pl.bwd_grid = dim3(blocks_split * (256 / pl.bwd_block.x));
        } else if (W <= 17 && d.nsplit > 1) {
            pl.bwd = BwdSweep::fused_occ4;
        } else {
            pl.bwd = BwdSweep::fused;
        }
    } else {
        pl.bwd = BwdSweep::plain;
        pl.bwd_w = backward_window(W);
        if (!d.real) pl.bwd_grid = dim3(blocks);
    }
    return pl;
}

template <int NF>
static int launch_solve(PencilPack *pp, LuFactor *lu, const RhsSrc &rhs, double *x, hipStream_t s, const SweepPlan &pl) {
    const PencilDev &P = pp->dev;
    const LuDev &d = lu->dev;
    if (pl.lds_f > 64 * 1024) return fail("pencil_solve: system too large for the LDS permutation cache");
    const int kl = pl.fwd_kl, nb = pl.fwd_nb, w = pl.bwd_w;
    switch (pl.fwd) {
        case FwdSweep::coop:
            if constexpr (NF > 0) {
                const double *rhs1 = rhs.p[0];
                if (rhs.n != 1 || rhs.a[0] != 1.0) {
                    const long nel = (long)P.nrows * P.nx * P.ny;
                    if (!lu->d_rhs_tmp) DDH_HIP(hipMalloc(&lu->d_rhs_tmp, (size_t)nel * sizeof(double) + 16));
                    if (int st0 = ddh_lincomb((double *)lu->d_rhs_tmp, rhs.n, rhs.p, rhs.a, nel, (void *)s)) return st0;
                    rhs1 = (const double *)lu->d_rhs_tmp;
                }
                auto k = nb == 2 ? solve_forward_coop_kernel<NF, true, 2> : solve_forward_coop_kernel<NF, true, 8>;
                if (!d.real) k = nb == 2 ? solve_forward_coop_kernel<NF, false, 2> : solve_forward_coop_kernel<NF, false, 8>;
                hipLaunchKernelGGL(k, pl.fwd_grid, pl.fwd_block, pl.lds_f, s, P, d, rhs1, x);
            }
            break;
        case FwdSweep::deep:
            if constexpr (NF == 2)
                hipLaunchKernelGGL((solve_forward_deep_kernel<6, 1, 4, 4>), pl.fwd_grid, pl.fwd_block, pl.lds_f, s, P, d, rhs, x);
            break;
        case FwdSweep::lean_occ4:
            if constexpr (NF == 2)
                hipLaunchKernelGGL((solve_forward_lean_kernel<6, 1, 4>), pl.fwd_grid, pl.fwd_block, pl.lds_f, s, P, d, rhs, x);
            break;
        case FwdSweep::lean:
            if constexpr (NF == 2) {
                auto k = kl == 12 ? solve_forward_lean_kernel<12, 2>
                                  : (nb == 1 ? solve_forward_lean_kernel<6, 1> : solve_forward_lean_kernel<6, 2>);
                hipLaunchKernelGGL(k, pl.fwd_grid, pl.fwd_block, pl.lds_f, s, P, d, rhs, x);
            }
            break;
        case FwdSweep::general: {
            auto k = kl == 12 ? (nb == 2 ? solve_forward_kernel<NF, true, 12, 2> : solve_forward_kernel<NF, true, 12, 8>)
                              : (nb == 2 ? solve_forward_kernel<NF, true, 16, 2> : solve_forward_kernel<NF, true, 16, 8>);
            if (!d.real)
                k = kl == 12 ? (nb == 2 ? solve_forward_kernel<NF, false, 12, 2> : solve_forward_kernel<NF, false, 12, 8>)
                             : (nb == 2 ? solve_forward_kernel<NF, false, 16, 2> : solve_forward_kernel<NF, false, 16, 8>);
            hipLaunchKernelGGL(k, pl.fwd_grid, pl.fwd_block, pl.lds_f, s, P, d, rhs, x);
            break;
        }
    }
    if constexpr (NF > 0)
        if (pl.border_finish)
            hipLaunchKernelGGL(border_finish_kernel<NF>, dim3((unsigned)((P.G + 255) / 256)), dim3(256), 0, s, P, d, x);
    switch (pl.bwd) {
        case BwdSweep::none:
            break;
        case BwdSweep::coop:
            if constexpr (NF > 0) {
                auto k = pl.cb == 16 ? (pl.tt == 2 ? solve_backward_coop_kernel<NF, 2, true, 16> : solve_backward_coop_kernel<NF, 3, true, 16>)
                                     : (pl.tt == 9 ? solve_backward_coop_kernel<NF, 9, true, 4> : solve_backward_coop_kernel<NF, 12, true, 4>);
                if (!d.real)
                    k = pl.cb == 16 ? (pl.tt == 2 ? solve_backward_coop_kernel<NF, 2, false, 16> : solve_backward_coop_kernel<NF, 3, false, 16>)
                                    : (pl.tt == 9 ? solve_backward_coop_kernel<NF, 9, false, 4> : solve_backward_coop_kernel<NF, 12, false, 4>);
                hipLaunchKernelGGL(k, pl.bwd_grid, pl.bwd_block, pl.lds_b, s, P, d, x);
            }
            break;
        case BwdSweep::deep:
            if constexpr (NF == 2)
                hipLaunchKernelGGL((solve_backward_deep_kernel<17, 2>), pl.bwd_grid, pl.bwd_block, pl.lds_b, s, P, d, x, d.pband, rhs.skip);
            break;
        case BwdSweep::fused_occ4:
            if constexpr (NF == 2)
                hipLaunchKernelGGL((solve_backward_kernel<NF, 17, true, false, true, 4>), pl.bwd_grid, pl.bwd_block, pl.lds_b, s, P, d, x, d.pband, rhs.skip);
            break;
        case BwdSweep::fused:
            if constexpr (NF == 2) {
                auto k = w == 17 ? solve_backward_kernel<NF, 17, true, false, true> : w == 32 ? solve_backward_kernel<NF, 32, true, false, true>
                       : w == 34 ? solve_backward_kernel<NF, 34, true, false, true> : solve_backward_kernel<NF, 48, true, false, true>;
                hipLaunchKernelGGL(k, pl.bwd_grid, pl.bwd_block, pl.lds_b, s, P, d, x, d.pband, rhs.skip);
            }
            break;
        case BwdSweep::plain: {
            auto k = w == 17 ? solve_backward_kernel<NF, 17, true, false> : w == 32 ? solve_backward_kernel<NF, 32, true, false>
                   : w == 34 ? solve_backward_kernel<NF, 34, true, false> : w == 48 ? solve_backward_kernel<NF, 48, true, false>
                   : solve_backward_kernel<NF, 64, true, false>;
            if (!d.real)
                k = w == 17 ? solve_backward_kernel<NF, 17, false, false> : w == 32 ? solve_backward_kernel<NF, 32, false, false>
                  : w == 34 ? solve_backward_kernel<NF, 34, false, false> : w == 48 ? solve_backward_kernel<NF, 48, false, false>
                  : solve_backward_kernel<NF, 64, false, false>;
            hipLaunchKernelGGL(k, pl.bwd_grid, pl.bwd_block, pl.lds_b, s, P, d, x, d.pband, rhs.skip);
            break;
        }
    }
    DDH_HIP(hipGetLastError());
    return finish_solve<NF>(pp, lu, rhs, x, s, pl.fuse_p ? 1 : 0);
}

constexpr int LUW_ROWS = 32;

template <bool REAL>
__global__ void __launch_bounds__(256)
lu_width_kernel(LuDev L, int *__restrict__ wrow) {
    typedef typename El<REAL>::T E;
    const long gl = (long)blockIdx.x * blockDim.x + threadIdx.x;
    const bool act = gl < L.GL;
    const E *Aw = (const E *)L.Aw;
    const int j0 = (int)blockIdx.y * LUW_ROWS, j1 = min(L.n, j0 + LUW_ROWS);
    for (int j = j0; j < j1; ++j) {
        int w = 0;
        if (act) {
            for (int d = L.W; d > 0; --d)
                if (!El<REAL>::is_zero(Aw[lu_aw(L, gl, j, L.kl + d)])) { w = d; break; }
        }
#pragma unroll
        for (int sft = 32; sft > 0; sft >>= 1) w = max(w, __shfl_xor(w, sft, 64));
        if ((threadIdx.x & 63) == 0) atomicMax(&wrow[j], w);
    }
}

}

using namespace ddh;

extern "C" {

int ddh_pencil_create(ddh_handle *pack, const ddh_pencil_geom *geom) {
    if (!geom || geom->nfourier < 0 || geom->nfourier > 2) return fail("pencil_create: nfourier must be 0, 1 or 2");
    PencilPack *pp = new PencilPack();
    pp->kind = H_PENCIL;
    PencilDev &d = pp->dev;
    d.nf = geom->nfourier;
    d.S = (d.nf == 2) ? 2 : 1;
    d.nrows = geom->nrows;
    d.nx = geom->nx;
    d.ny = geom->ny;
    if (d.nf == 0) {
        d.ncx = d.ncy = 1;
        if (d.nx != 1 || d.ny != 1) { delete pp; return fail("pencil_create: nfourier=0 needs nx=ny=1"); }
    } else if (d.nf == 1) {
        if (d.nx % 2 || d.ny != 1) { delete pp; return fail("pencil_create: nfourier=1 needs even nx and ny=1"); }
        d.ncx = d.nx / 2;
        d.ncy = 1;
    } else {
        if (d.nx % 2 || d.ny % 2) { delete pp; return fail("pencil_create: nfourier=2 needs even nx, ny"); }
        d.ncx = d.nx / 2;
        d.ncy = d.ny / 2;
    }
    d.ncells = d.ncx * d.ncy;
    d.G = d.ncells * d.S;
    d.mx_offset = geom->mx_offset;
    d.xtile = 0;
    int st = 0;
    if (d.nf >= 1) st = upload_vec(&pp->d_kx, geom->kx_h, (size_t)d.ncx);
    if (!st && d.nf == 2) st = upload_vec(&pp->d_ky, geom->ky_h, (size_t)d.ncy);
    if (st) { delete pp; return st; }
    d.kx = (const double *)pp->d_kx;
    d.ky = (const double *)pp->d_ky;
    if (d.nf >= 1) pp->kx_h.assign(geom->kx_h, geom->kx_h + d.ncx);
    if (d.nf == 2) pp->ky_h.assign(geom->ky_h, geom->ky_h + d.ncy);
    *pack = register_handle(pp);
    return 0;
}

int ddh_pencil_set_solve_variant(ddh_handle pack, int mode, int fwd, int backward_lanes) {
    PencilPack *pp = (PencilPack *)lookup_handle(pack, H_PENCIL);
    if (!pp) return -1;
    if (mode < 0 || mode > 2) return fail("pencil_set_solve_variant: mode must be 0, 1 or 2");
    if (backward_lanes > 0 && backward_lanes != 4 && backward_lanes != 16)
        return fail("pencil_set_solve_variant: backward lanes per system must be 0, 4 or 16");
    pp->coop_mode = mode;
    pp->coop_fwd = fwd < 0 ? -1 : (fwd ? 1 : 0);
    pp->coop_cb = backward_lanes < 0 ? -1 : backward_lanes;
    return 0;
}

int ddh_pencil_set_pairing(ddh_handle pack, const int *row_swap_h, const int *col_swap_h, long min_systems) {
    PencilPack *pp = (PencilPack *)lookup_handle(pack, H_PENCIL);
    if (!pp) return -1;
    pp->pair_rows.clear();
    pp->pair_cols.clear();
    if (!row_swap_h || !col_swap_h) return 0;
    const int N = pp->dev.nrows;
    if (pp->dev.nf != 2) return fail("pencil_set_pairing: two Fourier axes required");
    for (int i = 0; i < N; ++i) {
        const int r = row_swap_h[i], c = col_swap_h[i];
        if (r < 0 || r >= N || c < 0 || c >= N || row_swap_h[r] != i || col_swap_h[c] != i)
            return fail("pencil_set_pairing: the row and column maps must be involutions of 0..nrows-1");
    }
    pp->pair_rows.assign(row_swap_h, row_swap_h + N);
    pp->pair_cols.assign(col_swap_h, col_swap_h + N);
    pp->pair_min = min_systems;
    return 0;
}

int ddh_pencil_set_row_blocks(ddh_handle pack, int nblocks) {
    PencilPack *pp = (PencilPack *)lookup_handle(pack, H_PENCIL);
    if (!pp) return -1;
    if (nblocks < 1 || nblocks > 8) return fail("pencil_set_row_blocks: 1 .. 8 blocks");
    pp->row_blocks = nblocks;
    return 0;
}

int ddh_pencil_add_matrix(ddh_handle pack, const ddh_polymat *mat, int nrows_out, int *mat_id) {
    PencilPack *pp = (PencilPack *)lookup_handle(pack, H_PENCIL);
    if (!pp) return -1;
    const int nt = mat->nterms;
    std::vector<int> order(nt);
    for (int i = 0; i < nt; ++i) order[i] = i;
    std::stable_sort(order.begin(), order.end(), [&](int a, int b) { return mat->row_h[a] < mat->row_h[b]; });
    Matrix *m = new Matrix();
    std::vector<int> rowptr(nrows_out + 1, 0);
    m->col_h.resize(nt);
    m->coef_h.resize(nt);
    m->expo_h.resize(nt);
    m->row_h.resize(nt);
    for (int k = 0; k < nt; ++k) {
        const int t = order[k];
        const int r = mat->row_h[t];
        if (r < 0 || r >= nrows_out || mat->col_h[t] < 0 || mat->col_h[t] >= pp->dev.nrows) {
            delete m;
            return fail("pencil_add_matrix: term index out of range");
        }
        if (mat->ex_h[t] < 0 || mat->ex_h[t] > 7 || mat->ey_h[t] < 0 || mat->ey_h[t] > 7) {
            delete m;
            return fail("pencil_add_matrix: exponents must be in 0..7");
        }
        rowptr[r + 1]++;
        m->row_h[k] = r;
        m->col_h[k] = mat->col_h[t];
        m->coef_h[k] = make_double2(mat->coef_re_h[t], mat->coef_im_h[t]);
        m->expo_h[k] = (unsigned)mat->ex_h[t] | ((unsigned)mat->ey_h[t] << 8) |
                       ((unsigned)(mat->dx_h[t] ? 1 : 0) << 16) | ((unsigned)(mat->dy_h[t] ? 1 : 0) << 24);
    }
    for (int r = 0; r < nrows_out; ++r) rowptr[r + 1] += rowptr[r];
    int st = upload_vec(&m->d_rowptr, rowptr.data(), rowptr.size());
    if (!st) st = upload_vec(&m->d_col, m->col_h.data(), (size_t)nt);
    if (!st) st = upload_vec(&m->d_coef, m->coef_h.data(), (size_t)nt);
    if (!st) st = upload_vec(&m->d_expo, m->expo_h.data(), (size_t)nt);
    if (st) { delete m; return st; }
    m->dev.nrows_out = nrows_out;
    m->dev.nterms = nt;
    m->dev.rowptr = (const int *)m->d_rowptr;
    m->dev.col = (const int *)m->d_col;
    m->dev.coef = (const double2 *)m->d_coef;
    m->dev.expo = (const unsigned *)m->d_expo;
    m->dev.order = nullptr;
    {
        const char *e = getenv("DDH_MV_LOCALITY");
// ... 395 lines not shown
int ddh_pencil_factor(ddh_handle pack, int matM_id, int matL_id, double a, double b, const int *row_perm_h,
                      const int *col_perm_h, int n_interior, int kl, int ku, const unsigned char *row_axes_h,
                      const unsigned char *col_axes_h, int reuse_lu_id, int *lu_id, void *stream) {
    return factor_impl(pack, matM_id, matL_id, a, b, row_perm_h, col_perm_h, n_interior, kl, ku, row_axes_h,
                       col_axes_h, nullptr, nullptr, reuse_lu_id, lu_id, stream);
}

int ddh_pencil_factor_real(ddh_handle pack, int matM_id, int matL_id, double a, double b, const int *row_perm_h,
                           const int *col_perm_h, int n_interior, int kl, int ku,
                           const unsigned char *row_axes_h, const unsigned char *col_axes_h,
                           const unsigned char *row_code_h, const unsigned char *col_code_h, int reuse_lu_id,
                           int *lu_id, void *stream) {
    if (!row_code_h || !col_code_h) return fail("pencil_factor_real: grading codes required");
    return factor_impl(pack, matM_id, matL_id, a, b, row_perm_h, col_perm_h, n_interior, kl, ku, row_axes_h,
                       col_axes_h, row_code_h, col_code_h, reuse_lu_id, lu_id, stream);
}

int ddh_pencil_flagged(ddh_handle pack, int lu_id, int *count, long *cells_h, int max_cells) {
    PencilPack *pp = (PencilPack *)lookup_handle(pack, H_PENCIL);
    if (!pp) return -1;
    if (lu_id < 0 || lu_id >= (int)pp->lus.size()) return fail("pencil_flagged: bad LU id");
    LuFactor *lu = pp->lus[lu_id];
    *count = lu->nflag;
    for (int i = 0; i < lu->nflag && i < max_cells; ++i) cells_h[i] = lu->flag_cells[i];
    return 0;
}

int ddh_pencil_set_dense_inverse(ddh_handle pack, int lu_id, const double *inv_h) {
    PencilPack *pp = (PencilPack *)lookup_handle(pack, H_PENCIL);
    if (!pp) return -1;
    if (lu_id < 0 || lu_id >= (int)pp->lus.size()) return fail("pencil_set_dense_inverse: bad LU id");
    LuFactor *lu = pp->lus[lu_id];
    if (!lu->nflag) return 0;
    const size_t N = (size_t)lu->dev.N, nsys = (size_t)lu->nflag * pp->dev.S;
    (void)hipFree(lu->d_inv);
    (void)hipFree(lu->d_dense_rhs);
    DDH_HIP(hipMalloc(&lu->d_inv, nsys * N * N * sizeof(double2)));
    DDH_HIP(hipMalloc(&lu->d_dense_rhs, 2 * nsys * N * sizeof(double2)));
    DDH_HIP(hipMemcpy(lu->d_inv, inv_h, nsys * N * N * sizeof(double2), hipMemcpyHostToDevice));
    return 0;
}

__global__ void __launch_bounds__(256) widen_inverse_kernel(const double *__restrict__ src, double2 *__restrict__ dst, long nn,
                                                            int cx) {
    for (long e = (long)blockIdx.x * 256 + threadIdx.x; e < nn; e += (long)gridDim.x * 256)
        dst[e] = cx ? make_double2(src[2 * e], src[2 * e + 1]) : make_double2(src[e], 0.0);
}

int ddh_pencil_set_dense_inverse_dev(ddh_handle pack, int lu_id, int sys, const double *inv_d, int is_complex, void *stream) {
    PencilPack *pp = (PencilPack *)lookup_handle(pack, H_PENCIL);
    if (!pp) return -1;
    if (lu_id < 0 || lu_id >= (int)pp->lus.size()) return fail("pencil_set_dense_inverse_dev: bad LU id");
    LuFactor *lu = pp->lus[lu_id];
    const size_t N = (size_t)lu->dev.N, nsys = (size_t)lu->nflag * pp->dev.S;
    if (sys < 0 || (size_t)sys >= nsys) return fail("pencil_set_dense_inverse_dev: system index out of range");
    if (!lu->d_inv || !lu->d_dense_rhs) {
        (void)hipFree(lu->d_inv); lu->d_inv = nullptr;
        (void)hipFree(lu->d_dense_rhs); lu->d_dense_rhs = nullptr;
        void *inv = nullptr, *rhs = nullptr;
        int st = check_hip(hipMalloc(&inv, nsys * N * N * sizeof(double2)), "hipMalloc(dense inverse)");
        if (!st) st = check_hip(hipMalloc(&rhs, 2 * nsys * N * sizeof(double2)), "hipMalloc(dense rhs)");
        if (st) {
            (void)hipFree(inv);
            return st;
        }
        lu->d_inv = inv;
        lu->d_dense_rhs = rhs;
    }
    hipLaunchKernelGGL(widen_inverse_kernel, dim3(2048), dim3(256), 0, as_stream(stream), inv_d,
                       (double2 *)lu->d_inv + (size_t)sys * N * N, (long)(N * N), is_complex);
    DDH_HIP(hipGetLastError());
    return 0;
}

int ddh_pencil_set_block_inverse(ddh_handle pack, int lu_id, const double *binv_d) {
    PencilPack *pp = (PencilPack *)lookup_handle(pack, H_PENCIL);
    if (!pp) return -1;
    if (lu_id < 0 || lu_id >= (int)pp->lus.size()) return fail("pencil_set_block_inverse: bad LU id");
    LuFactor *lu = pp->lus[lu_id];
    if (binv_d) {
        const LuDev &d = lu->dev;
        if (pp->dev.nf != 1 || !d.real || d.pair || d.nsplit < 1 || d.n != d.nsplit * d.nh || d.nh > 4096)
            return fail("pencil_set_block_inverse: one Fourier axis, real-graded factors, equal diagonal blocks");
    }
    lu->d_binv = binv_d;
    return 0;
}

int ddh_pencil_solve(ddh_handle pack, int lu_id, const double *rhs, double *x, void *stream) {
    PencilPack *pp = (PencilPack *)lookup_handle(pack, H_PENCIL);
    if (!pp) return -1;
    if (lu_id < 0 || lu_id >= (int)pp->lus.size()) return fail("pencil_solve: bad LU id");
    if (rhs == x) return fail("pencil_solve: in-place unsupported");
    const double one = 1.0;
    return ddh_pencil_solve_lincomb(pack, lu_id, 1, &rhs, &one, x, stream);
}

int ddh_pencil_solve_lincomb(ddh_handle pack, int lu_id, int nterms, const double *const *xs_h, const double *alpha_h,
                             double *x, void *stream) {
    PencilPack *pp = (PencilPack *)lookup_handle(pack, H_PENCIL);
    if (!pp) return -1;
    if (lu_id < 0 || lu_id >= (int)pp->lus.size()) return fail("pencil_solve: bad LU id");
    if (nterms < 1 || nterms > RHS_MAX) return fail("pencil_solve_lincomb: 1 to 8 right-hand-side terms");
    RhsSrc r;
    memset(&r, 0, sizeof(r));
    r.n = nterms;
    for (int t = 0; t < nterms; ++t) {
        if (xs_h[t] == x) return fail("pencil_solve: in-place unsupported");
        r.p[t] = xs_h[t];
        r.a[t] = alpha_h[t];
    }
    LuFactor *lu = pp->lus[lu_id];
    hipStream_t s = as_stream(stream);
    const SweepPlan pl = sweep_plan(pp, lu->dev, nterms, false);
    if (pp->dev.nf == 2) return launch_solve<2>(pp, lu, r, x, s, pl);
    if (pp->dev.nf == 1) return launch_solve<1>(pp, lu, r, x, s, pl);
    return launch_solve<0>(pp, lu, r, x, s, pl);
}

static int build_pband(PencilPack *pp, LuFactor *lu, int p_mat_id) {
    LuDev &d = lu->dev;
    if (lu->pband_mat == p_mat_id && lu->d_pband) { d.pband = (const double *)lu->d_pband; return 0; }
    d.pband = nullptr;
    lu->pband_mat = p_mat_id;
    if (!d.real || d.n <= 0 || lu->colperm_h.empty()) return 0;
    const Matrix *m = pp->mats[p_mat_id];
    const int N = d.N, n = d.n;
    if (m->dev.nrows_out != N) return 0;
    std::vector<int> cinv(N, -1);
    for (int i = 0; i < N; ++i) cinv[lu->colperm_h[i]] = i;
    std::vector<double> band((size_t)n * PBW, 0.0);
    std::vector<char> diag(N, 0);
    for (size_t t = 0; t < m->row_h.size(); ++t) {
        const int r = cinv[m->row_h[t]], c = cinv[m->col_h[t]];
        const double2 cf = m->coef_h[t];
        if (m->expo_h[t] != 0 || cf.y != 0.0) return 0;
        if (r == c) {
            if (cf.x != 1.0 || diag[r]) return 0;
            diag[r] = 1;
            continue;
        }
        if (r >= n || c >= n || c < r || c - r > PBW) return 0;
        if (lu->ccode_h[r] != lu->ccode_h[c]) return 0;
        band[(size_t)r * PBW + (c - r - 1)] += cf.x;
    }
    for (int i = 0; i < N; ++i)
        if (!diag[i]) return 0;
    if (!lu->d_pband) DDH_HIP(hipMalloc(&lu->d_pband, band.size() * sizeof(double) + 16));
    DDH_HIP(hipMemcpy(lu->d_pband, band.data(), band.size() * sizeof(double), hipMemcpyHostToDevice));
    d.pband = (const double *)lu->d_pband;
    return 0;
}

int ddh_pencil_solve_recombined(ddh_handle pack, int lu_id, int nterms, const double *const *xs_h,
                                const double *alpha_h, int p_mat_id, double *work, double *x, void *stream) {
    return ddh_pencil_solve_recombined_sparse(pack, lu_id, nterms, xs_h, alpha_h, p_mat_id, work, x, nullptr, nullptr, stream);
}

static int solve_recombined_impl(ddh_handle pack, int lu_id, int nterms, const double *const *xs_h, const double *alpha_h,
                                 int p_mat_id, double *work, double *x, const unsigned char *zero_rows,
                                 const unsigned char *skip_rows, int terms_tiled, void *stream);

int ddh_pencil_solve_recombined_sparse(ddh_handle pack, int lu_id, int nterms, const double *const *xs_h,
                                       const double *alpha_h, int p_mat_id, double *work, double *x,
                                       const unsigned char *zero_rows, const unsigned char *skip_rows, void *stream) {
    return solve_recombined_impl(pack, lu_id, nterms, xs_h, alpha_h, p_mat_id, work, x, zero_rows, skip_rows, 0, stream);
}

int ddh_pencil_solve_recombined_tiled(ddh_handle pack, int lu_id, int nterms, const double *const *xs_h,
                                      const double *alpha_h, int p_mat_id, double *work, double *x,
                                      const unsigned char *zero_rows, const unsigned char *skip_rows, void *stream) {
    PencilPack *pp = (PencilPack *)lookup_handle(pack, H_PENCIL);
    if (!pp) return -1;
    if (lu_id < 0 || lu_id >= (int)pp->lus.size()) return fail("pencil_solve: bad LU id");
    if (pp->dev.nf != 2 || (pp->dev.nx & 7) || (pp->dev.ny & 7))
        return fail("pencil_solve_recombined_tiled: two Fourier axes with storage sizes that are multiples of 8");
    if (!sweep_plan(pp, pp->lus[lu_id]->dev, nterms, false).lean_forward())
        return fail("pencil_solve_recombined_tiled: this factorization does not run the lean forward sweep, the only one "
                    "that reads tile-major terms (ddh_pencil_lu_info)");
    return solve_recombined_impl(pack, lu_id, nterms, xs_h, alpha_h, p_mat_id, work, x, zero_rows, skip_rows, 1, stream);
}

static int solve_recombined_impl(ddh_handle pack, int lu_id, int nterms, const double *const *xs_h, const double *alpha_h,
                                 int p_mat_id, double *work, double *x, const unsigned char *zero_rows,
                                 const unsigned char *skip_rows, int terms_tiled, void *stream) {
    PencilPack *pp = (PencilPack *)lookup_handle(pack, H_PENCIL);
    if (!pp) return -1;
    if (lu_id < 0 || lu_id >= (int)pp->lus.size()) return fail("pencil_solve: bad LU id");
    if (p_mat_id < 0 || p_mat_id >= (int)pp->mats.size()) return fail("pencil_solve_recombined: bad matrix id");
    if (nterms < 1 || nterms > RHS_MAX) return fail("pencil_solve_recombined: 1 to 8 right-hand-side terms");
    if (work == x || !work) return fail("pencil_solve_recombined: work and x must be distinct buffers");
    RhsSrc r;
    memset(&r, 0, sizeof(r));
    r.n = nterms;
    for (int t = 0; t < nterms; ++t) {
        if (xs_h[t] == x || xs_h[t] == work) return fail("pencil_solve: in-place unsupported");
        r.p[t] = xs_h[t];
        r.a[t] = alpha_h[t];
    }
    r.zrow = zero_rows;
    r.skip = skip_rows;
    r.tiled = terms_tiled;
    LuFactor *lu = pp->lus[lu_id];
    hipStream_t s = as_stream(stream);
    int st;
    if (pp->dev.nf == 2 && (st = build_pband(pp, lu, p_mat_id))) return st;
    const SweepPlan pl = sweep_plan(pp, lu->dev, nterms, true);
    if (pl.fuse_p) return launch_solve<2>(pp, lu, r, x, s, pl);
    r.skip = nullptr;
    if (pp->dev.nf == 1 && lu->d_binv && lu->dev.real && lu->dev.n == lu->dev.nsplit * lu->dev.nh) {
        const LuDev &d = lu->dev;
        const unsigned nt = (unsigned)std::min(1024, (d.nh + 63) / 64 * 64);
        hipLaunchKernelGGL(blockinv_solve_kernel, dim3((unsigned)(pp->dev.ncells * d.nsplit)), dim3(nt), (size_t)d.nh * sizeof(double2),
                           s, pp->dev, d, r, lu->d_binv, work);
        DDH_HIP(hipGetLastError());
        st = finish_solve<1>(pp, lu, r, work, s, 0);
    } else if (pp->dev.nf == 2) st = launch_solve<2>(pp, lu, r, work, s, pl);
    else if (pp->dev.nf == 1) st = launch_solve<1>(pp, lu, r, work, s, pl);
    else st = launch_solve<0>(pp, lu, r, work, s, pl);
    if (st) return st;
    PostSolve none;
    memset(&none, 0, sizeof(none));
    if (pp->dev.xtile == 2) return fail("pencil_solve_recombined: a kx-band-major state needs the fused recombination");
    return launch_matvec(pp, p_mat_id, work, x, none, stream, 0, pp->dev.xtile);
}

int ddh_pencil_lu_row_widths(ddh_handle pack, int lu_id, int *wrow_h) {
    PencilPack *pp = (PencilPack *)lookup_handle(pack, H_PENCIL);
    if (!pp) return -1;
    if (lu_id < 0 || lu_id >= (int)pp->lus.size()) return fail("pencil_lu_row_widths: bad LU id");
    const LuDev &d = pp->lus[lu_id]->dev;
    if (d.n <= 0) return 0;
    int *dw = nullptr;
    DDH_HIP(hipMalloc((void **)&dw, d.n * sizeof(int)));
    DDH_HIP(hipMemset(dw, 0, d.n * sizeof(int)));
    const unsigned blocks = (unsigned)((d.GL + 255) / 256);
    const dim3 wgrid(blocks, (unsigned)((d.n + LUW_ROWS - 1) / LUW_ROWS));
    if (d.real) hipLaunchKernelGGL(lu_width_kernel<true>, wgrid, dim3(256), 0, 0, d, dw);
    else hipLaunchKernelGGL(lu_width_kernel<false>, wgrid, dim3(256), 0, 0, d, dw);
    DDH_HIP(hipGetLastError());
    DDH_HIP(hipMemcpy(wrow_h, dw, d.n * sizeof(int), hipMemcpyDeviceToHost));
    (void)hipFree(dw);
    return 0;
}

int ddh_pencil_lu_info(ddh_handle pack, int lu_id, int *info_h) {
    PencilPack *pp = (PencilPack *)lookup_handle(pack, H_PENCIL);
    if (!pp) return -1;
    if (lu_id < 0 || lu_id >= (int)pp->lus.size()) return fail("pencil_lu_info: bad LU id");
    const LuDev &d = pp->lus[lu_id]->dev;
    const SweepPlan pl = sweep_plan(pp, d, 1, false);
    const int fwd = pl.fwd == FwdSweep::coop ? 2 : (pl.lean_forward() ? 1 : 0);
    const int v[12] = {d.n, d.nb, d.kl, d.ku, d.W, d.BW, d.nsplit, d.nh, fwd, pl.cb, d.pair, d.real};
    for (int i = 0; i < 12; ++i) info_h[i] = v[i];
    return 0;
}

int ddh_pencil_lu_bytes(ddh_handle pack, int lu_id, size_t *bytes) {
    PencilPack *pp = (PencilPack *)lookup_handle(pack, H_PENCIL);
    if (!pp) return -1;
    if (lu_id < 0 || lu_id >= (int)pp->lus.size()) return fail("pencil_lu_bytes: bad LU id");
    *bytes = pp->lus[lu_id]->bytes;
    return 0;
}

}
```

### dedalus_amd/libhip.py

```python

import ctypes as C
import os

import numpy as np

_HERE = os.path.dirname(os.path.abspath(__file__))
LIB_PATH = os.environ.get("DDH_LIB") or os.path.join(_HERE, "csrc", "libdedalus_hip.so")

_lib = None


class DdhError(RuntimeError):
    pass


class PencilGeom(C.Structure):
    _fields_ = [("nfourier", C.c_int), ("nrows", C.c_int), ("nx", C.c_long), ("ny", C.c_long),
                ("kx_h", C.POINTER(C.c_double)), ("ky_h", C.POINTER(C.c_double)), ("mx_offset", C.c_long)]


class PolyMat(C.Structure):
    _fields_ = [("nterms", C.c_int),
                ("row_h", C.POINTER(C.c_int)), ("col_h", C.POINTER(C.c_int)),
                ("coef_re_h", C.POINTER(C.c_double)), ("coef_im_h", C.POINTER(C.c_double)),
                ("ex_h", C.POINTER(C.c_byte)), ("ey_h", C.POINTER(C.c_byte)),
                ("dx_h", C.POINTER(C.c_byte)), ("dy_h", C.POINTER(C.c_byte))]


_vp, _h, _hp = C.c_void_p, C.c_uint64, C.POINTER(C.c_uint64)
_dp, _ip, _l, _i, _d = C.POINTER(C.c_double), C.POINTER(C.c_int), C.c_long, C.c_int, C.c_double

SIGNATURES = {
    "ddh_init": [_i],
    "ddh_device_count": [_ip],
    "ddh_alloc": [C.POINTER(_vp), C.c_size_t],
    "ddh_free": [_vp],
    "ddh_memset": [_vp, _i, C.c_size_t, _vp],
    "ddh_memcpy_h2d": [_vp, _vp, C.c_size_t, _vp],
    "ddh_memcpy_d2h": [_vp, _vp, C.c_size_t, _vp],
    "ddh_memcpy_d2d": [_vp, _vp, C.c_size_t, _vp],
    "ddh_stream_sync": [_vp],
    "ddh_destroy": [_h],
    "ddh_plan_rfft": [_hp, _i, _i],
    "ddh_scatter_add": [_vp, _vp, _vp, _l, _vp],
    "ddh_scatter_set": [_vp, _vp, _vp, _l, _vp],
    "ddh_pencil_set_state_tiled": [_h, _i],
    "ddh_fft_set_coeff_tiled": [_h, _l, _l],
    "ddh_tile_rows": [_vp, _vp, _l, _l, _l, _i, _l, _vp],
    "ddh_plan_grouped_mmt": [_hp, _i, _i, _vp, _i, _ip, C.POINTER(_vp), C.POINTER(_vp)],
    "ddh_grouped_mmt_set_pairs": [_h, _i, _ip, _ip, _ip, _ip],
    "ddh_grouped_mmt_forward": [_h, _vp, _vp, _l, _l, _l, _l, _l, _vp],
    "ddh_grouped_mmt_backward": [_h, _vp, _vp, _l, _l, _l, _l, _l, _vp],
    "ddh_regularity_recombine": [_vp, _i, _l, _l, _l, _vp, _i, _vp, _vp, _vp],
    "ddh_spin_recombine": [_vp, _vp, _i, _l, _l, _dp, _vp],
    "ddh_sphere_terms_create": [_hp, _i, _i, _i, _i, _ip, _ip, _ip, _dp],
    "ddh_sphere_terms_apply": [_h, _vp, _vp, _vp],
    "ddh_cgemv_batch_create": [_hp, _i, _i, _i, _dp],
    "ddh_cgemv_batch_apply": [_h, _vp, _vp, _vp],
    "ddh_ell_terms_create": [_hp, _i, _i, _i, _i, _i, _i, _ip, _ip, _ip, _i, _dp, _ip],
    "ddh_ell_terms_apply": [_h, _vp, _vp, _vp],
    "ddh_dense_inverse_create": [_hp, _i, _ip, _i, _dp, _dp, C.POINTER(C.c_ubyte), C.POINTER(C.c_ubyte)],
    "ddh_dense_inverse_elements": [_h, C.POINTER(_l)],
    "ddh_dense_inverse_compute": [_h, _d, _d, _vp, _ip, _vp],
    "ddh_cgemv_batch_mats": [_h, C.POINTER(_vp)],
    "ddh_ell_terms_create_dense": [_hp, _i, _i, _i, _i],
    "ddh_ell_terms_mats": [_h, C.POINTER(_vp)],
    "ddh_ell_terms_prune": [_h, _vp],
    "ddh_ell_blocks_from_dense": [_vp, _vp, _i, _i, _i, _vp],
    "ddh_ell_terms_apply_acc": [_h, _vp, _vp, _i, _vp],
    "ddh_ell_mix_create": [_hp, _i, _i, _i, _i, _i, _i, _ip, _ip, _i, _dp, _ip],
    "ddh_ell_mix_apply": [_h, _vp, _vp, _vp],
    "ddh_ellband_create": [_hp, _i, _i, _i, _i, _i, _i, _i, _l, _ip, _ip, _ip, C.POINTER(_l), C.POINTER(_l), _dp, _dp, _dp, _dp],
    "ddh_ellband_create_complex": [_hp, _i, _i, _i, _i, _i, _i, _i, _l, _ip, _ip, _ip, C.POINTER(_l), C.POINTER(_l), _dp, _dp, _dp, _dp],
    "ddh_ellband_factor": [_h, _i, _d, _d, _ip, _vp],
    "ddh_ellband_solve": [_h, _i, _vp, _vp, _vp],
    "ddh_ellband_info": [_h, _ip, _ip, C.POINTER(_l)],
    "ddh_ellband_gather_complex_inverse": [_vp, _vp, _vp, _i, _i, _i, _i, _vp],
    "ddh_ellband_bordered_inverse": [_vp, _i, _i, _vp, _vp, _d, _d, _d, _d, _vp, _vp],
    "ddh_rfft_forward": [_h, _vp, _vp, _l, _l, _vp],
    "ddh_rfft_backward": [_h, _vp, _vp, _l, _l, _vp],
    "ddh_rfft_backward_deriv": [_h, _vp, _vp, _l, _l, _d, _vp],
    "ddh_rfft_backward_dual": [_h, _vp, _vp, _vp, _l, _l, _d, _vp],
    "ddh_cheb_backward_dual": [_h, _vp, _vp, _vp, _vp, _l, _l, _vp],
    "ddh_rfft_bilinear_fused": [_h, _i, C.POINTER(_vp), _dp, _i, C.POINTER(_vp), _dp, _i, C.POINTER(_vp), _l, _i,
                                _ip, _ip, _ip, _dp, _vp],
    "ddh_plan_cfft": [_hp, _i, _i],
    "ddh_cfft_forward": [_h, _vp, _vp, _l, _l, _vp],
    "ddh_cfft_backward": [_h, _vp, _vp, _l, _l, _vp],
    "ddh_plan_cheb": [_hp, _i, _i, _i, _ip, _dp],
    "ddh_cheb_forward": [_h, _vp, _vp, _l, _l, _vp],
    "ddh_cheb_forward_tiled": [_h, _vp, _vp, _l, _l, _l, _vp],
    "ddh_fft_set_stage_layout": [_h, _l],
    "ddh_fft_set_stage_block": [_h, _i],
    "ddh_fft_set_stage_window": [_h, _i, _i],
    "ddh_fft_wave_launches": [C.POINTER(_l)],
    "ddh_fft_wave_size": [_i, _i, _i, _ip],
    "ddh_cheb_backward": [_h, _vp, _vp, _l, _l, _vp],
    "ddh_plan_mmt": [_hp, _i, _i, _dp],
    "ddh_mmt_apply": [_h, _vp, _vp, _l, _l, _vp],
    "ddh_lincomb": [_vp, _i, C.POINTER(_vp), _dp, _l, _vp],
    "ddh_grid_bilinear": [_vp, _i, _vp, _vp, _l, _i, _ip, _ip, _ip, _dp, _vp],
    "ddh_grid_cfl": [_vp, _vp, _i, _l, C.POINTER(_vp), _ip, C.POINTER(_l), _i, _vp],
    "ddh_grid_cfl_spherical": [_vp, _vp, _l, _i, _vp, _vp, _vp],
    "ddh_grid_reduce": [_vp, _vp, _l, _vp, _vp],
    "ddh_grid_map": [_vp, _vp, _l, _i, _d, _vp],
    "ddh_grid_broadcast": [_vp, _vp, _i, C.POINTER(_l), _ip, _vp],
    "ddh_grid_map_launches": [C.POINTER(_l)],
    "ddh_axis_contract": [_vp, _vp, _l, _i, _l, _l, _vp, _i, _vp],
    "ddh_axis_contract_rows": [_vp, _vp, _l, _i, _l, _vp, _vp, _vp, _i, _vp],
    "ddh_pencil_create": [_hp, C.POINTER(PencilGeom)],
    "ddh_pencil_add_matrix": [_h, C.POINTER(PolyMat), _i, _ip],
    "ddh_pencil_matvec": [_h, _i, _vp, _vp, _vp],
    "ddh_pencil_matvec_update": [_h, _i, _vp, _vp, _vp],
    "ddh_pencil_add_upper_bands": [_h, _i, _i, _ip, _dp, _ip],
    "ddh_pencil_matvec_solve": [_h, _i, _i, _vp, _vp, _vp],
    "ddh_pencil_factor": [_h, _i, _i, _d, _d, _ip, _ip, _i, _i, _i,
                          C.POINTER(C.c_ubyte), C.POINTER(C.c_ubyte), _i, _ip, _vp],
    "ddh_pencil_factor_real": [_h, _i, _i, _d, _d, _ip, _ip, _i, _i, _i,
                               C.POINTER(C.c_ubyte), C.POINTER(C.c_ubyte), C.POINTER(C.c_ubyte),
                               C.POINTER(C.c_ubyte), _i, _ip, _vp],
    "ddh_pencil_solve": [_h, _i, _vp, _vp, _vp],
    "ddh_pencil_set_solve_variant": [_h, _i, _i, _i],
    "ddh_pencil_set_pairing": [_h, _ip, _ip, _l],
    "ddh_pencil_set_row_blocks": [_h, _i],
    "ddh_pencil_solve_lincomb": [_h, _i, _i, C.POINTER(_vp), _dp, _vp, _vp],
    "ddh_pencil_solve_recombined": [_h, _i, _i, C.POINTER(_vp), _dp, _i, _vp, _vp, _vp],
    "ddh_pencil_solve_recombined_sparse": [_h, _i, _i, C.POINTER(_vp), _dp, _i, _vp, _vp, _vp, _vp, _vp],
    "ddh_pencil_solve_recombined_tiled": [_h, _i, _i, C.POINTER(_vp), _dp, _i, _vp, _vp, _vp, _vp, _vp],
    "ddh_pencil_matvec_update_tiled": [_h, _i, _vp, _vp, _vp],
    "ddh_pencil_flagged": [_h, _i, _ip, C.POINTER(_l), _i],
    "ddh_pencil_set_dense_inverse": [_h, _i, _dp],
    "ddh_pencil_set_dense_inverse_dev": [_h, _i, _i, _vp, _i, _vp],
    "ddh_pencil_set_block_inverse": [_h, _i, _vp],
    "ddh_pencil_lu_bytes": [_h, _i, C.POINTER(C.c_size_t)],
    "ddh_pencil_lu_info": [_h, _i, _ip],
    "ddh_pencil_lu_row_widths": [_h, _i, _ip],
    "ddh_modal_create": [_hp, _i, _l, _l, _l, _dp, _dp, _dp, _l, _i, _i, _ip, _ip, C.POINTER(C.c_ubyte), _i, _ip, _ip,
                         _dp, _dp, C.POINTER(C.c_ubyte), C.POINTER(C.c_ubyte), C.POINTER(C.c_ubyte), C.POINTER(C.c_ubyte)],
    "ddh_pencil_solve_modal": [_h, _d, _d, _i, C.POINTER(_vp), _dp, _i, _vp, _i, _vp],
    "ddh_modal_launches": [C.POINTER(_l)],
    "ddh_comm_probe": [],
    "ddh_comm_unique_id": [C.POINTER(C.c_ubyte)],
    "ddh_comm_create": [_hp, _i, _i, C.POINTER(C.c_ubyte)],
    "ddh_comm_create_loopback": [_hp, _i, _i],
    "ddh_comm_info": [_h, _ip, _ip],
    "ddh_comm_allreduce": [_h, _vp, _l, _i, _vp],
    "ddh_comm_alltoall": [_h, _vp, _vp, _l, _vp],
    "ddh_comm_alltoall_part": [_h, _vp, _vp, _l, _l, _i, _l, _vp],
    "ddh_a2a_plan": [_hp, _h, _l, _l, _l, _l],
    "ddh_a2a_plan_blocks": [_hp, _h, _l, _l, _l, _l, _l, _l],
    "ddh_a2a_localize_rows": [_h, _vp, _vp, _vp],
    "ddh_a2a_localize_columns": [_h, _vp, _vp, _vp],
    "ddh_a2a_forward": [_h, _vp, _vp, _vp],
    "ddh_a2a_backward": [_h, _vp, _vp, _vp],
    "ddh_a2a_pack": [_vp, _vp, _l, _l, _l, _l, _i, _vp],
    "ddh_a2a_unpack": [_vp, _vp, _l, _l, _l, _l, _i, _vp],
    "ddh_a2av_pack": [_vp, _vp, _l, _l, _l, _i, _vp],
    "ddh_a2av_unpack": [_vp, _vp, _l, _l, _l, _i, _vp],
    "ddh_a2av_pack_b": [_vp, _vp, _l, _l, _l, _i, _l, _vp],
    "ddh_a2av_unpack_b": [_vp, _vp, _l, _l, _l, _i, _l, _vp],
}


class MmtGroup(C.Structure):
    _fields_ = [("mat", C.c_int), ("g_start", C.c_int), ("c_start", C.c_int), ("count", C.c_int),
                ("ell_start", C.c_int), ("ell_step", C.c_int), ("n_ell", C.c_int)]


def load(build_if_missing=False):
    global _lib
    if _lib is not None:
        return _lib
    try:
        import torch
    except ImportError:
        pass
    if not os.path.exists(LIB_PATH):
        if build_if_missing:
            from . import build
            build.build_library()
        else:
            raise DdhError("libdedalus_hip.so not found at %s -- run `python -m dedalus_amd.build` "
                           "(there is no CPU fallback)" % LIB_PATH)
    lib = C.CDLL(LIB_PATH)
    for name, argtypes in SIGNATURES.items():
        if os.environ.get("DDH_LIB") and not hasattr(lib, name):
            continue
        fn = getattr(lib, name)
        fn.argtypes = argtypes
        fn.restype = C.c_int
    lib.ddh_last_error.argtypes = []
    lib.ddh_last_error.restype = C.c_char_p
    _lib = lib
    return lib


def check(status, what=""):
    if status != 0:
        msg = load().ddh_last_error().decode("utf-8", "replace")
        raise DdhError("%s failed (status %d): %s" % (what or "libdedalus_hip call", status, msg))


profiler = None
cost_log = None


def call(name, *args):
    lib = load()
    if profiler is not None:
        check(profiler(name, getattr(lib, name), args), name)
        return
    check(getattr(lib, name)(*args), name)


def note_cost(name, flops, nbytes):
    if cost_log is not None:
        cost_log(name, float(flops), float(nbytes))


def as_dp(a):
    return a.ctypes.data_as(_dp)


def as_ip(a):
    return a.ctypes.data_as(_ip)


def as_bp(a):
    return a.ctypes.data_as(C.POINTER(C.c_byte))


def as_ubp(a):
    return a.ctypes.data_as(C.POINTER(C.c_ubyte))
```

### dedalus_amd/pencilpack.py

```python

import ctypes as C

import numpy as np

from . import libhip
from .device import ptr


class TermList:

    __slots__ = ("nrows", "ncols", "row", "col", "coef", "ex", "ey", "dx", "dy")

    def __init__(self, nrows, ncols, row=(), col=(), coef=(), ex=(), ey=(), dx=(), dy=()):
        self.nrows, self.ncols = int(nrows), int(ncols)
        self.row = np.asarray(row, dtype=np.int32).ravel()
        self.col = np.asarray(col, dtype=np.int32).ravel()
        self.coef = np.asarray(coef, dtype=np.complex128).ravel()
        n = self.row.size
        self.ex = np.asarray(ex, dtype=np.int8).ravel() if np.size(ex) else np.zeros(n, np.int8)
        self.ey = np.asarray(ey, dtype=np.int8).ravel() if np.size(ey) else np.zeros(n, np.int8)
        self.dx = np.asarray(dx, dtype=np.int8).ravel() if np.size(dx) else np.zeros(n, np.int8)
        self.dy = np.asarray(dy, dtype=np.int8).ravel() if np.size(dy) else np.zeros(n, np.int8)

    @property
# ... 88 lines not shown
        t = self._timer()
        if t is not None:
            return t.run("pencil_matvec", (x.numel() + y.numel()) * 8, self._matvec_solve, mat_id, bands_id, x, y)
        return self._matvec_solve(mat_id, bands_id, x, y)

    def _matvec_solve(self, mat_id, bands_id, x, y):
        libhip.call("ddh_pencil_matvec_solve", self.handle, mat_id, bands_id, ptr(x), ptr(y), self.dev.stream)

    def factor(self, matM, matL, a, b, row_perm, col_perm, n_interior, kl, ku, row_axes, col_axes, reuse=-1,
               real=None):
        row_perm = np.ascontiguousarray(row_perm, dtype=np.int32)
        col_perm = np.ascontiguousarray(col_perm, dtype=np.int32)
        ra = np.ascontiguousarray(np.asarray(row_axes, dtype=np.uint8)[row_perm])
        ca = np.ascontiguousarray(np.asarray(col_axes, dtype=np.uint8)[col_perm])
        lu = C.c_int(-1)
        if real is not None:
            rc = np.ascontiguousarray(np.asarray(real["row_code"], dtype=np.uint8)[row_perm])
            cc = np.ascontiguousarray(np.asarray(real["col_code"], dtype=np.uint8)[col_perm])
            libhip.call("ddh_pencil_factor_real", self.handle, real["matM"], real["matL"], float(a), float(b),
                        libhip.as_ip(row_perm), libhip.as_ip(col_perm), int(n_interior), int(kl), int(ku),
                        libhip.as_ubp(ra), libhip.as_ubp(ca), libhip.as_ubp(rc), libhip.as_ubp(cc),
                        int(reuse), C.byref(lu), self.dev.stream)
        else:
            libhip.call("ddh_pencil_factor", self.handle, matM, matL, float(a), float(b), libhip.as_ip(row_perm),
                        libhip.as_ip(col_perm), int(n_interior), int(kl), int(ku), libhip.as_ubp(ra),
                        libhip.as_ubp(ca), int(reuse), C.byref(lu), self.dev.stream)
        lu_id = lu.value
        count = C.c_int(0)
        cells = np.zeros(4096, dtype=np.int64)
        libhip.call("ddh_pencil_flagged", self.handle, lu_id, C.byref(count),
                    cells.ctypes.data_as(C.POINTER(C.c_long)), cells.size)
        nflag = count.value
        self.flagged = {} if not hasattr(self, "flagged") else self.flagged
        self.flagged[lu_id] = [int(c) for c in cells[:min(nflag, cells.size)]]
        if nflag > cells.size or nflag * self.S * self.nrows ** 2 * 16 > 8e9:
            raise libhip.DdhError("%d pencils have a singular band block: problem structure unsupported by the "
                                  "bordered-band solver" % nflag)
        if nflag:
            self._flagged_inverses(lu_id, matM, matL, a, b, row_perm, col_perm, ra, ca, cells[:nflag], n_interior)
        self.lu_meta[lu_id] = dict(nflag=nflag, a=a, b=b)
        return lu_id

    def _bordered_band(self, Md, Ld, n_interior):
        N, n = Md.shape[0], int(n_interior)
        if N - n != 1 or n < 2:
            return None
        absB = np.abs(Md[:n, :n]) + np.abs(Ld[:n, :n])
        zc = np.flatnonzero(absB.sum(axis=0) == 0.0)
        if len(zc) != 1:
            return None
        j0 = int(zc[0])
        if Md[n, j0] == 0.0 and Ld[n, j0] == 0.0:
            return None
        from .executor import BorderedBandInverse, HipExecutor
        ex = self.executor if self.executor is not None else HipExecutor(self.dev)
        try:
            return BorderedBandInverse(ex, Md, Ld, n, j0)
        except libhip.DdhError:
            return None

    def _flagged_inverses(self, lu_id, matM, matL, a, b, row_perm, col_perm, ra, ca, cells, n_interior=None):
        import os
        N, S = self.nrows, self.S
        if n_interior is None:
            n_interior = N
        key = (matM, matL, row_perm.tobytes(), col_perm.tobytes(), tuple(int(c) for c in cells))
        cache = self.__dict__.setdefault("_flag_dinv", {})
        if key not in cache:
            M, L = self.matrices[matM], self.matrices[matL]
            Ms, Ls, rvs, cvs, slots = [], [], [], [], []
            for f, cell in enumerate(int(c) for c in cells):
                mx, my = (cell // self.ncy, cell % self.ncy) if self.nf == 2 else (cell, 0)
                kxv = self.kx[mx] if self.nf >= 1 else 0.0
                kyv = self.ky[my] if self.nf == 2 else 0.0
                gmx = mx + self.mx_offset
                rv = np.array([_valid(ra[i], gmx, my, self.nf) for i in range(N)], dtype=bool)
                cv = np.array([_valid(ca[i], gmx, my, self.nf) for i in range(N)], dtype=bool)
                for sidx in range(S):
                    if sidx == 1 and kxv == 0.0:
                        slots[-1].append(f * S + 1)
                        continue
                    sign = 1 if sidx == 0 else -1
                    Ms.append(M.dense(kxv, kyv, gmx, my, sign)[np.ix_(row_perm, col_perm)])
                    Ls.append(L.dense(kxv, kyv, gmx, my, sign)[np.ix_(row_perm, col_perm)])
                    rvs.append(rv)
                    cvs.append(cv)
                    slots.append([f * S + sidx])
            cx = any(m.imag.any() for m in Ms) or any(m.imag.any() for m in Ls)
            if not cx:
                Ms, Ls = [m.real.copy() for m in Ms], [m.real.copy() for m in Ls]
            band = None
            if (not cx and os.environ.get("DDH_FLAG_DENSE", "0") != "1" and not getattr(self, "_flag_dense", False)
                    and all(rv.all() and cv.all() for rv, cv in zip(rvs, cvs))):
                band = [self._bordered_band(Md, Ld, n_interior) for Md, Ld in zip(Ms, Ls)]
                if any(bd is None for bd in band):
                    band = None
            if len(cache) > 4:
                cache.clear()
            if band is not None:
                cache[key] = ("band", band, slots)
            else:
                from .executor import DenseInverse, HipExecutor
                ex = self.executor if self.executor is not None else HipExecutor(self.dev)
                cache[key] = ("dev", DenseInverse(ex, Ms, Ls, rvs, cvs, cx), [m.shape[0] for m in Ms], slots, cx)
        ent = cache[key]
        if ent[0] == "band":
            for bd, sl in zip(ent[1], ent[2]):
                inv = bd.compute(a, b)
                if inv is None:
                    self._flag_dense = True
                    cache.pop(key)
                    return self._flagged_inverses(lu_id, matM, matL, a, b, row_perm, col_perm, ra, ca, cells, n_interior)
                for t in sl:
                    libhip.call("ddh_pencil_set_dense_inverse_dev", self.handle, lu_id, int(t), C.c_void_p(inv.data_ptr()), 0,
                                self.dev.stream)
            return
        _, dinv, sizes, slots, cx = ent
        flat = dinv.compute(a, b)
        off = 0
        for n, sl in zip(sizes, slots):
            for t in sl:
                libhip.call("ddh_pencil_set_dense_inverse_dev", self.handle, lu_id, int(t),
                            C.c_void_p(flat.data_ptr() + off * 8), int(cx), self.dev.stream)
            off += n * n * (2 if cx else 1)

    def set_block_inverse(self, lu_id, binv):
        libhip.call("ddh_pencil_set_block_inverse", self.handle, int(lu_id), ptr(binv) if binv is not None else None)
        self.__dict__.setdefault("_binv_bytes", {})[int(lu_id)] = int(binv.numel()) * 8 if binv is not None else 0

    def solve(self, lu_id, rhs, x):
        t = self._timer()
        if t is not None:
            nb = self.lu_bytes(lu_id) + (rhs.numel() + x.numel()) * 8
            return t.run("pencil_solve", nb, self._solve, lu_id, rhs, x)
        return self._solve(lu_id, rhs, x)

    def _solve(self, lu_id, rhs, x):
        libhip.call("ddh_pencil_solve", self.handle, lu_id, ptr(rhs), ptr(x), self.dev.stream)

    def solve_lincomb(self, lu_id, xs, alphas, x):
        t = self._timer()
        if t is not None:
            nb = self.lu_bytes(lu_id) + (sum(v.numel() for v in xs) + x.numel()) * 8
            return t.run("pencil_solve", nb, self._solve_lincomb, lu_id, xs, alphas, x)
        return self._solve_lincomb(lu_id, xs, alphas, x)

    def _solve_lincomb(self, lu_id, xs, alphas, x):
        arr = (C.c_void_p * len(xs))(*[C.c_void_p(v.data_ptr()) for v in xs])
        al = np.ascontiguousarray(alphas, dtype=np.float64)
        libhip.call("ddh_pencil_solve_lincomb", self.handle, lu_id, len(xs), arr, libhip.as_dp(al), ptr(x), self.dev.stream)

    supports_zero_rows = True

    def solve_recombined(self, lu_id, xs, alphas, p_mat_id, work, x, zero_rows=None, skip_rows=None, tiled=False):
        t = self._timer()
        if t is not None:
            info = self.lu_info(lu_id)
            read = 1.0 - (zero_rows[1] if (zero_rows is not None and info["forward"] == "lean") else 0.0)
            wrote = 1.0 - (skip_rows[1] if (skip_rows is not None and info["backward_lanes"] == 0 and info["real"]) else 0.0)
            nb = self.lu_bytes(lu_id) + (sum(v.numel() for v in xs) * read + x.numel() * wrote) * 8
            binv = getattr(self, "_binv_bytes", {}).get(lu_id)
            if binv:
                nb = binv + (sum(v.numel() for v in xs) + 3 * x.numel()) * 8
            return t.run("pencil_solve", nb, self._solve_recombined, lu_id, xs, alphas, p_mat_id, work, x, zero_rows,
                         skip_rows, tiled)
        return self._solve_recombined(lu_id, xs, alphas, p_mat_id, work, x, zero_rows, skip_rows, tiled)

    def _solve_recombined(self, lu_id, xs, alphas, p_mat_id, work, x, zero_rows=None, skip_rows=None, tiled=False):
        arr = (C.c_void_p * len(xs))(*[C.c_void_p(v.data_ptr()) for v in xs])
        al = np.ascontiguousarray(alphas, dtype=np.float64)
        if zero_rows is not None or skip_rows is not None or tiled:
            zp = C.c_void_p(zero_rows[0].data_ptr()) if zero_rows is not None else None
            sp = C.c_void_p(skip_rows[0].data_ptr()) if skip_rows is not None else None
            libhip.call("ddh_pencil_solve_recombined_tiled" if tiled else "ddh_pencil_solve_recombined_sparse", self.handle,
                        lu_id, len(xs), arr, libhip.as_dp(al), int(p_mat_id), ptr(work), ptr(x), zp, sp, self.dev.stream)
            return
        libhip.call("ddh_pencil_solve_recombined", self.handle, lu_id, len(xs), arr, libhip.as_dp(al), int(p_mat_id),
                    ptr(work), ptr(x), self.dev.stream)

    MAX_RHS_TERMS = 8

    def set_solve_variant(self, mode=1, fwd=-1, backward_lanes=-1):
        libhip.call("ddh_pencil_set_solve_variant", self.handle, int(mode), int(fwd), int(backward_lanes))
        self.variant_epoch = getattr(self, "variant_epoch", 0) + 1

    def set_pairing(self, row_swap, col_swap, min_systems=0):
        if row_swap is None or col_swap is None:
            libhip.call("ddh_pencil_set_pairing", self.handle, None, None, 0)
            return
        rs = np.ascontiguousarray(row_swap, dtype=np.int32)
        cs = np.ascontiguousarray(col_swap, dtype=np.int32)
        libhip.call("ddh_pencil_set_pairing", self.handle, libhip.as_ip(rs), libhip.as_ip(cs), int(min_systems))

    def set_row_blocks(self, nblocks):
        libhip.call("ddh_pencil_set_row_blocks", self.handle, int(nblocks))

    def lu_info(self, lu_id):
        v = np.zeros(12, dtype=np.int32)
        libhip.call("ddh_pencil_lu_info", self.handle, lu_id, libhip.as_ip(v))
        keys = ("n", "nb", "kl", "ku", "W", "BW", "nsplit", "rows_per_block", "forward", "backward_lanes", "pair", "real")
        d = dict(zip(keys, (int(x) for x in v)))
        d["forward"] = ("general", "lean", "cooperative")[d["forward"]]
        return d

    def lu_bytes(self, lu_id):
        n = C.c_size_t(0)
        libhip.call("ddh_pencil_lu_bytes", self.handle, lu_id, C.byref(n))
        return n.value


def _valid(bits, mx, my, nf):
    if nf >= 1 and mx != 0 and not (bits & 1):
        return False
    if nf == 2 and my != 0 and not (bits & 2):
        return False
    return True
```

### include/dedalus_hip.h

```cpp
#ifndef DEDALUS_HIP_H
#define DEDALUS_HIP_H

#include <stddef.h>
#include <stdint.h>

#ifdef __cplusplus
extern "C" {
#endif

typedef uint64_t ddh_handle;

int ddh_init(int device);
const char *ddh_last_error(void);
int ddh_device_count(int *count);
int ddh_alloc(void **ptr, size_t bytes);
int ddh_free(void *ptr);
int ddh_memset(void *ptr, int value, size_t bytes, void *stream);
int ddh_memcpy_h2d(void *dst, const void *src_h, size_t bytes, void *stream);
int ddh_memcpy_d2h(void *dst_h, const void *src, size_t bytes, void *stream);
int ddh_memcpy_d2d(void *dst, const void *src, size_t bytes, void *stream);
int ddh_stream_sync(void *stream);
int ddh_destroy(ddh_handle h);

int ddh_plan_rfft(ddh_handle *plan, int n_grid, int n_coeff);
// ... 23 lines not shown
int ddh_cheb_forward_tiled(ddh_handle plan, const double *g, double *c, long outer, long inner, long row_len, void *stream);
int ddh_fft_set_stage_layout(ddh_handle plan, long value);
int ddh_fft_set_stage_block(ddh_handle plan, int rows);
int ddh_fft_wave_launches(long *count);
int ddh_fft_wave_size(int kind, int n_grid, int n_coeff, int *covered);
int ddh_cheb_backward(ddh_handle plan, const double *c, double *g, long outer, long inner, void *stream);

int ddh_plan_mmt(ddh_handle *plan, int n_out, int n_in, const double *mat_h);
int ddh_mmt_apply(ddh_handle plan, const double *in, double *out, long outer, long inner, void *stream);

typedef struct {
    int mat;
    int g_start, c_start, count;
    int ell_start, ell_step, n_ell;
} ddh_mmt_group;
int ddh_plan_grouped_mmt(ddh_handle *plan, int n_grid, int ngroups, const ddh_mmt_group *groups_h, int nmats,
                         const int *mat_rows_h, const double *const *fwd_h, const double *const *bwd_h);
int ddh_grouped_mmt_set_pairs(ddh_handle plan, int ngroups, const int *pair_g_h, const int *pair_c_h,
                              const int *pair_mode_h, const int *parity_h);
int ddh_grouped_mmt_forward(ddh_handle plan, const double *g, double *c, long n0, long n1g, long n1c, long n2c,
                            long n3, void *stream);
int ddh_grouped_mmt_backward(ddh_handle plan, const double *c, double *g, long n0, long n1g, long n1c, long n2c,
                             long n3, void *stream);

int ddh_regularity_recombine(double *data, int ncomp, long n1, long n2, long n3, const int *slot_map_d, int nmats,
                             const double *mats_d, const double *radial_factor_d, void *stream);

int ddh_spin_recombine(const double *in, double *out, int ncomp, long npairs, long inner, const double *mat_h,
                       void *stream);
int ddh_sphere_terms_create(ddh_handle *h, int nm, int nl, int ncomp_out, int nterms, const int *co_h, const int *ci_h,
                            const int *d_h, const double *coef_h);
int ddh_sphere_terms_apply(ddh_handle h, const double *x, double *y, void *stream);
int ddh_cgemv_batch_create(ddh_handle *h, int nm, int nl, int ncomp, const double *mats_h);
int ddh_cgemv_batch_apply(ddh_handle h, const double *x, double *y, void *stream);
int ddh_ell_terms_create(ddh_handle *h, int nm, int nl, int nr, int ncomp_out, int ncomp_in, int nterms, const int *co_h,
                         const int *ci_h, const int *rot_h, int nmat, const double *mats_h, const int *slot_map_h);
int ddh_ell_terms_apply(ddh_handle h, const double *x, double *y, void *stream);
int ddh_ell_terms_apply_acc(ddh_handle h, const double *x, double *y, int accumulate, void *stream);
int ddh_ell_mix_create(ddh_handle *h, int nm, int nl, int nr, int ncomp_out, int ncomp_in, int nterms, const int *co_h,
                       const int *ci_h, int nq, const double *q_h, const int *slot_map_h);
int ddh_ell_mix_apply(ddh_handle h, const double *x, double *y, void *stream);

int ddh_dense_inverse_create(ddh_handle *h, int nsys, const int *n_h, int is_complex, const double *M_h,
                             const double *L_h, const unsigned char *row_valid_h, const unsigned char *col_valid_h);
int ddh_dense_inverse_elements(ddh_handle h, long *count_doubles);
int ddh_dense_inverse_compute(ddh_handle h, double a, double b, double *out_d, int *nsingular_h, void *stream);
int ddh_cgemv_batch_mats(ddh_handle h, double **mats_d);
int ddh_ell_terms_create_dense(ddh_handle *h, int nm, int nl, int nr, int ncomp);
int ddh_ell_terms_mats(ddh_handle h, double **mats_d);
int ddh_ell_blocks_from_dense(const double *inv_d, double *mats_d, int nl, int ncomp, int nr, void *stream);
int ddh_ell_terms_prune(ddh_handle h, void *stream);

int ddh_ellband_create(ddh_handle *h, int nl, int nmax, int kl, int ku, int mp, int nbc, int nslots, long slot_stride,
                       const int *n_h, const int *nbc_h, const int *slot_limit_h, const long *rowoff_h,
                       const long *coloff_h, const double *T_h, const double *P_h, const double *MB_h,
                       const double *LB_h);
int ddh_ellband_create_complex(ddh_handle *h, int nl, int nmax, int kl, int ku, int mp, int nbc, int nslots,
                               long slot_stride, const int *n_h, const int *nbc_h, const int *slot_limit_h,
                               const long *rowoff_h, const long *coloff_h, const double *T_h, const double *P_h,
                               const double *MB_h, const double *LB_h);
int ddh_ellband_factor(ddh_handle h, int index, double a, double b, int *nsingular_h, void *stream);
int ddh_ellband_solve(ddh_handle h, int index, const double *rhs_d, double *x_d, void *stream);
int ddh_ellband_info(ddh_handle h, int *nw, int *wt, long *factor_bytes);
int ddh_ellband_gather_complex_inverse(const double *x_d, double *out_d, const long *off_d, int ncomp, int nl, int nm,
                                       int nslots, void *stream);

int ddh_ellband_bordered_inverse(const double *X_d, int n, int j0, const double *wM_d, const double *wL_d, double dM,
                                 double dL, double a, double b, double *out_d, void *stream);

int ddh_scatter_add(double *y, const long *idx_d, const double *vals_d, long n, void *stream);
int ddh_scatter_set(double *y, const long *idx_d, const double *vals_d, long n, void *stream);

int ddh_pencil_set_state_tiled(ddh_handle pack, int on);
int ddh_fft_set_coeff_tiled(ddh_handle plan, long row_len, long band_rows);
int ddh_tile_rows(const double *src, double *dst, long nrows, long nx, long ny, int to_tiled, long band_rows, void *stream);

int ddh_lincomb(double *y, int nterms, const double *const *xs_h, const double *alpha_h,
                long n, void *stream);
int ddh_grid_bilinear(double *out, int ncomp_out, const double *a, const double *b, long n,
                      int nterms, const int *ic_h, const int *ia_h, const int *ib_h,
                      const double *coef_h, void *stream);
int ddh_grid_cfl(double *result_d, const double *u, int ncomp, long n,
                 const double *const *inv_spacing_comp, const int *comp_axis_h,
                 const long *axis_len_h, int naxes, void *stream);

int ddh_grid_cfl_spherical(double *result_d, const double *u, long n_ang, int nr, const double *inv_h_d,
                           const double *inv_dr_d, void *stream);

#define DDH_REDUCE_WORK_DOUBLES 3072
int ddh_grid_reduce(double *out3_d, const double *x, long n, double *work_d, void *stream);

enum ddh_map_op {
    DDH_MAP_ABSOLUTE = 0, DDH_MAP_SIGN, DDH_MAP_EXP, DDH_MAP_EXP2, DDH_MAP_LOG, DDH_MAP_LOG2, DDH_MAP_LOG10, DDH_MAP_SQRT,
    DDH_MAP_SQUARE, DDH_MAP_SIN, DDH_MAP_COS, DDH_MAP_TAN, DDH_MAP_ARCSIN, DDH_MAP_ARCCOS, DDH_MAP_ARCTAN, DDH_MAP_SINH,
    DDH_MAP_COSH, DDH_MAP_TANH, DDH_MAP_ARCSINH, DDH_MAP_ARCCOSH, DDH_MAP_ARCTANH, DDH_MAP_RECIP, DDH_MAP_POW
};
int ddh_grid_map(double *out, const double *in, long n, int op, double param, void *stream);
int ddh_grid_broadcast(double *out, const double *in, int ncomp, const long *shape_h, const int *present_h, void *stream);
int ddh_grid_map_launches(long *count);

int ddh_axis_contract(const double *in_d, double *out_d, long outer, int n, long inner, long ostride,
                      const double *w_d, int nw, void *stream);
int ddh_axis_contract_rows(const double *in_d, double *out_d, long outer, int n, long inner, const double *w_d,
                           const int *row_d, const int *kmin_d, int nrows, void *stream);

typedef struct {
    int nfourier;
    int nrows;
    long nx, ny;
    const double *kx_h;
    const double *ky_h;
    long mx_offset;
} ddh_pencil_geom;

typedef struct {
    int nterms;
    const int *row_h, *col_h;
    const double *coef_re_h, *coef_im_h;
    const signed char *ex_h, *ey_h;
    const signed char *dx_h, *dy_h;
} ddh_polymat;

int ddh_pencil_create(ddh_handle *pack, const ddh_pencil_geom *geom);
int ddh_pencil_add_matrix(ddh_handle pack, const ddh_polymat *mat, int nrows_out, int *mat_id);
int ddh_pencil_matvec(ddh_handle pack, int mat_id, const double *x, double *y, void *stream);
int ddh_pencil_matvec_update(ddh_handle pack, int mat_id, const double *x, double *y, void *stream);
int ddh_pencil_add_upper_bands(ddh_handle pack, int nz, int nbands, const int *offsets_h,
                               const double *bands_h, int *bands_id);
int ddh_pencil_matvec_solve(ddh_handle pack, int mat_id, int bands_id, const double *x, double *y,
                            void *stream);
int ddh_pencil_factor(ddh_handle pack, int matM_id, int matL_id, double a, double b,
                      const int *row_perm_h, const int *col_perm_h, int n_interior, int kl, int ku,
                      const unsigned char *row_axes_h, const unsigned char *col_axes_h,
                      int reuse_lu_id, int *lu_id, void *stream);
int ddh_pencil_factor_real(ddh_handle pack, int matM_id, int matL_id, double a, double b,
                           const int *row_perm_h, const int *col_perm_h, int n_interior, int kl, int ku,
                           const unsigned char *row_axes_h, const unsigned char *col_axes_h,
                           const unsigned char *row_code_h, const unsigned char *col_code_h,
                           int reuse_lu_id, int *lu_id, void *stream);
int ddh_pencil_solve(ddh_handle pack, int lu_id, const double *rhs, double *x, void *stream);
int ddh_pencil_solve_lincomb(ddh_handle pack, int lu_id, int nterms, const double *const *xs_h, const double *alpha_h,
                             double *x, void *stream);
int ddh_pencil_solve_recombined(ddh_handle pack, int lu_id, int nterms, const double *const *xs_h,
                                const double *alpha_h, int p_mat_id, double *work, double *x, void *stream);
int ddh_pencil_solve_recombined_sparse(ddh_handle pack, int lu_id, int nterms, const double *const *xs_h,
                                       const double *alpha_h, int p_mat_id, double *work, double *x,
                                       const unsigned char *zero_rows, const unsigned char *skip_rows, void *stream);
int ddh_pencil_set_solve_variant(ddh_handle pack, int mode, int fwd, int backward_lanes);
int ddh_pencil_set_pairing(ddh_handle pack, const int *row_swap_h, const int *col_swap_h, long min_systems);
int ddh_pencil_matvec_update_tiled(ddh_handle pack, int mat_id, const double *x, double *y, void *stream);
int ddh_pencil_solve_recombined_tiled(ddh_handle pack, int lu_id, int nterms, const double *const *xs_h,
                                      const double *alpha_h, int p_mat_id, double *work, double *x,
                                      const unsigned char *zero_rows, const unsigned char *skip_rows, void *stream);
int ddh_pencil_set_row_blocks(ddh_handle pack, int nblocks);
int ddh_pencil_flagged(ddh_handle pack, int lu_id, int *count, long *cells_h, int max_cells);
int ddh_pencil_set_dense_inverse(ddh_handle pack, int lu_id, const double *inv_h);
int ddh_pencil_set_dense_inverse_dev(ddh_handle pack, int lu_id, int sys, const double *inv_d, int is_complex, void *stream);
int ddh_pencil_set_block_inverse(ddh_handle pack, int lu_id, const double *binv_d);
int ddh_pencil_lu_bytes(ddh_handle pack, int lu_id, size_t *bytes);
int ddh_pencil_lu_info(ddh_handle pack, int lu_id, int *info_h);
int ddh_pencil_lu_row_widths(ddh_handle pack, int lu_id, int *wrow_h);

int ddh_modal_create(ddh_handle *out, int rc, long nx, long ny, long nz, const double *kx_h, const double *ky_h,
                     const double *kz_h, long mx_offset, int nrows_rhs, int nrows_x, const int *rhs_row_h,
                     const int *x_row_h, const unsigned char *axes_h, int nterms, const int *ti_h, const int *tj_h,
                     const double *coef_re_h, const double *coef_im_h, const unsigned char *ex_h,
                     const unsigned char *ey_h, const unsigned char *ez_h, const unsigned char *flags_h);
int ddh_pencil_solve_modal(ddh_handle plan, double a, double b, int nrhs, const double *const *rhs, const double *alphas_h,
                           int rhs_tiled, double *x, int x_tiled, void *stream);
int ddh_modal_launches(long *count);

#define DDH_COMM_ID_BYTES 128
int ddh_comm_probe(void);
int ddh_comm_unique_id(unsigned char *id_h);
int ddh_comm_create(ddh_handle *comm, int rank, int nranks, const unsigned char *id_h);
int ddh_comm_create_loopback(ddh_handle *comm, int rank, int nranks);
int ddh_comm_info(ddh_handle comm, int *rank, int *nranks);
int ddh_comm_allreduce(ddh_handle comm, double *buf, long count, int op, void *stream);
int ddh_comm_alltoall(ddh_handle comm, const double *send, double *recv, long chunk, void *stream);
int ddh_comm_alltoall_part(ddh_handle comm, const double *send, double *recv, long count, long peer_stride, int nbatch,
                           long batch_stride, void *stream);
int ddh_fft_set_stage_window(ddh_handle plan, int z0, int nplanes);

int ddh_a2a_plan(ddh_handle *plan, ddh_handle comm, long n0, long n1, long n2, long n3);
int ddh_a2a_plan_blocks(ddh_handle *plan, ddh_handle comm, long n0, long n1, long n2, long n3, long block1, long block2);
int ddh_a2a_localize_rows(ddh_handle plan, const double *cl, double *rl, void *stream);
int ddh_a2a_localize_columns(ddh_handle plan, const double *rl, double *cl, void *stream);
int ddh_a2a_forward(ddh_handle plan, const double *cl, double *rl, void *stream);
int ddh_a2a_backward(ddh_handle plan, const double *rl, double *cl, void *stream);
int ddh_a2a_pack(const double *src, double *dst, long outer, long na, long nb, long inner,
                 int nparts, void *stream);
int ddh_a2a_unpack(const double *src, double *dst, long outer, long na, long nb, long inner,
                   int nparts, void *stream);
int ddh_a2av_pack(const double *src, double *dst, long outer, long na, long row, int nparts, void *stream);
int ddh_a2av_unpack(const double *src, double *dst, long outer_na, long nb, long inner, int nparts, void *stream);
int ddh_a2av_pack_b(const double *src, double *dst, long outer, long na, long row, int nparts, long block, void *stream);
int ddh_a2av_unpack_b(const double *src, double *dst, long outer_na, long nb, long inner, int nparts, long block, void *stream);

#ifdef __cplusplus
}
#endif
#endif
```

Before: 22.59 timesteps/sec.

## Emit M.X from the backward solve sweep instead of separate matvecs

Builds per-row band tables for the mass matrix M in the permuted LU ordering, so the fused backward sweep can compute M·X from its sliding window of solved values and write it directly. This drops the separate M·X matvec at intermediate RK stages. It also reuses the final-stage M·X as the next step's MX0 when the state has not been touched in between. The cost is extra arithmetic and stores inside the sweep kernel, more LDS and register use, and added host-side bookkeeping to decide when the cached MX0 is still valid.

```diff
diff --git a/dedalus_amd/core/solvers.py b/dedalus_amd/core/solvers.py
--- a/dedalus_amd/core/solvers.py
+++ b/dedalus_amd/core/solvers.py
@@ -992,7 +992,39 @@
             self._skiprows = self._device_mask(mask)
         return self._skiprows
 
-    def solve_lincomb(self, lu, xs, alphas, out, zero_rows=None, skip_rows=None, tiled=False):
+    MX_WINDOW = 18
+
+    def mx_band_tables(self, rows_per_block=None, width=None):
+        if self.P_tl is None or self.real_grading is None or self.n_interior <= 0:
+            return None
+        tl = self.MP_tl.consolidated()
+        if np.any(tl.ex) or np.any(tl.ey) or np.any(tl.dx) or np.any(tl.dy):
+            return None
+        n = int(self.n_interior)
+        return mx_band_tables(tl.row, tl.col, tl.coef, self.row_perm, self.col_perm, n, int(rows_per_block or n),
+                              self.real_grading["row_code"], self.real_grading["col_code"],
+                              int(width or self.MX_WINDOW))
+
+    def prepare_mx_emission(self, lu):
+        if not hasattr(self.pack, "emits_mx") or self.P_id is None or getattr(self, "modal", None) is not None:
+            return False
+        if not self.pack.emits_mx(lu, self.P_id):
+            return False
+        info = self.pack.lu_info(lu)
+        tables = self.mx_band_tables(info["rows_per_block"] if info["nsplit"] > 1 else None)
+        if tables is None:
+            return False
+        self.pack.set_mx_band(lu, self.M_id, tables[0], tables[1])
+        return True
+
+    def sweep_emits_mx(self, lus):
+        if self.dist.size > 1 or not getattr(self, "x_tiled", 0):
+            return False
+        return all(self.prepare_mx_emission(lu) for lu in lus)
+
+    def solve_lincomb(self, lu, xs, alphas, out, zero_rows=None, skip_rows=None, tiled=False, mx_out=None):
+        if mx_out is not None and not (tiled and self.P_id is not None and len(xs) <= self.pack.MAX_RHS_TERMS):
+            raise RuntimeError("M.X from the sweep needs the tiled fused recombined solve")
         probe = getattr(self, "solve_probe", None)
         if getattr(self, "modal", None) is not None and probe is None and len(xs) <= self.modal.MAX_RHS_TERMS and not tiled:
             a, b = self._modal_lus[lu]
@@ -1025,9 +1057,14 @@
         elif hasattr(self.pack, "solve_recombined"):
             Y = self.ex.empty((self.R, self.nx, self.ny))
             if tiled:
-                self.pack.solve_recombined(lu, xs, alphas, self.P_id, Y, out, zero_rows=zero_rows, skip_rows=skip_rows,
-                                           tiled=True)
-                path = "ddh_pencil_solve_recombined_tiled"
+                if mx_out is not None:
+                    self.pack.solve_recombined(lu, xs, alphas, self.P_id, Y, out, zero_rows=zero_rows, skip_rows=skip_rows,
+                                               tiled=True, mx=(self.M_id, mx_out))
+                    path = "ddh_pencil_solve_recombined_tiled_mx"
+                else:
+                    self.pack.solve_recombined(lu, xs, alphas, self.P_id, Y, out, zero_rows=zero_rows, skip_rows=skip_rows,
+                                               tiled=True)
+                    path = "ddh_pencil_solve_recombined_tiled"
             elif zero_rows is not None or skip_rows is not None:
                 self.pack.solve_recombined(lu, xs, alphas, self.P_id, Y, out, zero_rows=zero_rows, skip_rows=skip_rows)
                 path = "ddh_pencil_solve_recombined_sparse"
@@ -1257,6 +1294,47 @@
         return True
 
 
+def mx_band_tables(row, col, coef, row_perm, col_perm, n, nh, row_code, col_code, width):
+    R = len(row_perm)
+    rinv = np.empty(R, dtype=np.int64)
+    cinv = np.empty(R, dtype=np.int64)
+    rinv[np.asarray(row_perm)] = np.arange(R)
+    cinv[np.asarray(col_perm)] = np.arange(R)
+    coef = np.asarray(coef)
+    keep = coef != 0
+    row, col, coef = np.asarray(row)[keep], np.asarray(col)[keep], coef[keep]
+    if coef.size and np.any(np.abs(coef.imag) > 0):
+        return None
+    i, j = rinv[row], cinv[col]
+    if np.any(i >= n) or np.any(j >= n):
+        return None
+    if np.any(np.asarray(row_code)[row] != np.asarray(col_code)[col]):
+        return None
+    step_row = -np.ones(n, dtype=np.int16)
+    band = np.zeros((n, width))
+    if n > 32767:
+        return None
+    rows = []
+    for r in np.unique(i):
+        cols = j[i == r]
+        if np.any(cols // nh != cols[0] // nh):
+            return None
+        if cols.max() - cols.min() >= width:
+            return None
+        rows.append((int(cols.min()), int(cols.max()), int(r)))
+    for cmin, cmax, r in sorted(rows, key=lambda v: (-v[0], -v[1])):
+        lo = max(cmax - (width - 1), 0, (cmin // nh) * nh)
+        t = cmin
+        while t >= lo and step_row[t] >= 0:
+            t -= 1
+        if t < lo:
+            return None
+        step_row[t] = r
+        m = i == r
+        np.add.at(band[t], j[m] - t, coef[m].real)
+    return step_row, band
+
+
 def _two_colour(n, row, col, label):
     from collections import deque
     adj_r = [[] for _ in range(n)]
diff --git a/dedalus_amd/core/timesteppers.py b/dedalus_amd/core/timesteppers.py
--- a/dedalus_amd/core/timesteppers.py
+++ b/dedalus_amd/core/timesteppers.py
@@ -58,10 +58,12 @@
             self._RHS = s.ex.zeros((s.R, s.nx, s.ny))
         return self._RHS
 
-    def _solve_combination(self, xs, al, lu, zero_rows=None, skip_rows=None, tiled=False):
+    def _solve_combination(self, xs, al, lu, zero_rows=None, skip_rows=None, tiled=False, mx_out=None):
         s = self.solver
         if hasattr(s, "solve_lincomb"):
-            if tiled:
+            if mx_out is not None:
+                s.solve_lincomb(lu, xs, al, s.X, zero_rows=zero_rows, skip_rows=skip_rows, tiled=True, mx_out=mx_out)
+            elif tiled:
                 s.solve_lincomb(lu, xs, al, s.X, zero_rows=zero_rows, skip_rows=skip_rows, tiled=True)
             elif zero_rows is not None or skip_rows is not None:
                 s.solve_lincomb(lu, xs, al, s.X, zero_rows=zero_rows, skip_rows=skip_rows)
@@ -291,6 +293,7 @@
                             for j in range(1, self.stages + 1)]
         self._k = None
         self._lus = {}
+        self._mx0_iteration = None
 
     def step(self, dt, wall_time=None):
         s = self.solver
@@ -306,7 +309,9 @@
                 if h not in self._lus:
                     self._lus[h] = s.factor(1.0, k * h, reuse=(reuse.pop() if reuse else -1))
             self._k = k
+            self._mx0_iteration = None
         t0 = s.sim_time
+        state_kept = bool(getattr(s, "_state_is_clean", lambda: False)())
         s.sync_state_to_device()
         own = dict(owned=True) if getattr(pack, "supports_zero_rows", False) else {}
         stamp = (tuple(self._lus.values()), getattr(pack, "variant_epoch", 0))
@@ -319,21 +324,35 @@
                     ex.fill_zero(buf)
                 s._F_zeroed = set(b.data_ptr() if hasattr(b, "data_ptr") else id(b) for b in self.F)
             self._tiled, self._tiled_stamp = tiled_now, stamp
+            self._emit = bool(tiled_now) and hasattr(s, "sweep_emits_mx") and s.sweep_emits_mx(self._lus.values())
+            self._mx0_iteration = None
         tiled = self._tiled
+        emit = self._emit
         if tiled:
             own = dict(owned=True, tiled=True)
+        iteration = getattr(s, "iteration", None)
+        capturing = bool(getattr(s, "_graph_wanted", lambda: False)())
+        mx0_kept = (emit and not capturing and iteration is not None and self._mx0_iteration == iteration
+                    and state_kept)
+        self._mx0_iteration = None
+        cadence = getattr(s, "enforce_real_cadence", 0)
+        mx0_next = (emit and not capturing and iteration is not None and hasattr(s, "_state_is_clean")
+                    and not (cadence and iteration % cadence < self.steps))
         later = []
         defer_mv = bool(getattr(s, "overlaps_rhs_work", lambda: False)())
-        (later.append if defer_mv else (lambda f: f()))(lambda: pack.matvec(s.M_id, s.X, self.MX0, **own))
+        if not mx0_kept:
+            (later.append if defer_mv else (lambda f: f()))(lambda: pack.matvec(s.M_id, s.X, self.MX0, **own))
         combs = {}
         for i in range(1, self.stages + 1):
             j = i - 1
             if self._need_lx[j]:
+                mv = None
                 if self._direct or j == 0:
                     mv = (lambda j=j: pack.matvec(s.L_id, s.X, self.LX[j]))
-                else:
+                elif not emit:
                     mv = (lambda j=j: pack.matvec(s.M_id, s.X, self.MX[j], **own))
-                (later.append if defer_mv else (lambda f: f()))(mv)
+                if mv is not None:
+                    (later.append if defer_mv else (lambda f: f()))(mv)
             if later:
                 s._overlap_work = list(later)
                 del later[:]
@@ -363,9 +382,17 @@
             skip = None
             if i < self.stages and not self._direct and hasattr(s, "intermediate_skip_rows"):
                 skip = s.intermediate_skip_rows()
-            self._solve_combination(xs, al, self._lus[float(H[i, i])], zero_rows=zrows, skip_rows=skip, tiled=bool(tiled))
+            mx_out = None
+            if emit and i < self.stages and self.MX[i] is not None:
+                mx_out = self.MX[i]
+            elif i == self.stages and mx0_next:
+                mx_out = self.MX0
+            self._solve_combination(xs, al, self._lus[float(H[i, i])], zero_rows=zrows, skip_rows=skip, tiled=bool(tiled),
+                                    mx_out=mx_out)
             s.mark_state_current()
             s.sim_time = t0 + k * c[i]
+        if mx0_next:
+            self._mx0_iteration = iteration + 1
 
 
 @add_scheme
diff --git a/dedalus_amd/csrc/ddh_pencil.hip b/dedalus_amd/csrc/ddh_pencil.hip
--- a/dedalus_amd/csrc/ddh_pencil.hip
+++ b/dedalus_amd/csrc/ddh_pencil.hip
@@ -81,6 +81,13 @@
 
 constexpr int PBW = 12;
 
+constexpr int MXW = 18;
+struct MxEmit {
+    double *out;
+    const double *band;
+    const short *row;
+};
+
 struct LuFactor {
     LuDev dev;
     size_t bytes = 0;
@@ -98,6 +105,8 @@
     void *d_pband = nullptr;
     void *d_vcell = nullptr, *d_vslot = nullptr, *d_rowperm2 = nullptr, *d_colperm2 = nullptr;
     void *d_wrow = nullptr;
+    void *d_mxband = nullptr, *d_mxrow = nullptr;
+    int mx_mat = -1, mx_ok = 0;
     std::vector<long> slot_cells_h;
     void *d_slot_cell = nullptr;
     int pband_mat = -1;
@@ -142,6 +151,8 @@
     (void)hipFree(lu->d_rowperm2);
     (void)hipFree(lu->d_colperm2);
     (void)hipFree(lu->d_wrow);
+    (void)hipFree(lu->d_mxband);
+    (void)hipFree(lu->d_mxrow);
     delete lu;
 }
 
@@ -1787,10 +1798,11 @@
     }
 }
 
-template <int NF, int WT, bool REAL, bool PREF, bool PFUSE = false, int MINW = 1>
+template <int NF, int WT, bool REAL, bool PREF, bool PFUSE = false, int MINW = 1, bool EMIT_MX = false>
 __global__ void __launch_bounds__(256, MINW)
 solve_backward_kernel(PencilDev P, LuDev L, double *__restrict__ xout, const double *__restrict__ pband,
-                      const unsigned char *__restrict__ skip) {
+                      const unsigned char *__restrict__ skip, MxEmit mx) {
+    static_assert(!EMIT_MX || (PFUSE && REAL && NF == 2 && WT + 1 == MXW), "M.X is emitted from the window of y = P^-1 x");
     typedef typename El<REAL>::T E;
     extern __shared__ int s_lds[];
     const int n = L.n, nb = L.nb, kl = L.kl, W = L.W;
@@ -1799,7 +1811,9 @@
     unsigned char *s_code = (unsigned char *)(s_perm2 + n);
     unsigned char *s_skip = s_code + n;
     unsigned char *s_nq = s_skip + n;
+    short *s_mxrow = (short *)(s_nq + n + (n & 1));
     for (int i = threadIdx.x; i < n; i += blockDim.x) {
+        if (EMIT_MX) s_mxrow[i] = mx.row[i];
         s_perm[i] = L.colperm[i];
         if (L.pair) s_perm2[i] = L.colperm2[i];
         s_code[i] = REAL ? L.col_code[i] : 0;
@@ -1884,6 +1898,39 @@
         if (conjq) v.y = -v.y;
         store_sys<NF>(xout, plane, my_perm[j], P, c, s, v);
     };
+    const __amdgpu_buffer_rsrc_t mx_rs = wave_rsrc(mx.out);
+    const unsigned mx_lane = EMIT_MX ? (unsigned)(tile_offset(2 * c.mx + s, 2 * c.my, P.ny) * (long)sizeof(double)) : 0u;
+    auto emit_mx = [&](int j, double2 yj, auto wv) {
+        if constexpr (EMIT_MX) {
+            const int mi = __builtin_amdgcn_readfirstlane((int)s_mxrow[j]);
+            if (mi < 0) return;
+            __builtin_amdgcn_sched_barrier(0);
+            const double *cf = mx.band + (long)j * MXW;
+            double2 a = make_double2(cf[0] * yj.x, cf[0] * yj.y);
+#pragma unroll
+            for (int d = 0; d < WT; ++d) {
+                const double2 w = wv(d);
+                a.x += cf[d + 1] * w.x;
+                a.y += cf[d + 1] * w.y;
+            }
+            const unsigned char code = L.row_code[mi];
+            if (code & 1) a = make_double2(-a.y, a.x);
+            if ((code & 2) && s == 1) a = make_double2(-a.x, -a.y);
+            if (conjq) a.y = -a.y;
+            const int prow = (L.pair && id.partner) ? L.rowperm2[mi] : L.rowperm[mi];
+            double2 other;
+            other.x = __shfl_xor(a.x, 1);
+            other.y = __shfl_xor(a.y, 1);
+            double2 out = (s == 0) ? make_double2(0.5 * (a.x + other.x), 0.5 * (a.y + other.y))
+                                   : make_double2(0.5 * (other.y - a.y), 0.5 * (a.x - other.x));
+            if (c.my == 0) out.y = 0.0;
+            if (c.gmx == 0 && s == 1) out = make_double2(0.0, 0.0);
+            ddh_u4v q;
+            q.x = (unsigned)__double2loint(out.x); q.y = (unsigned)__double2hiint(out.x);
+            q.z = (unsigned)__double2loint(out.y); q.w = (unsigned)__double2hiint(out.y);
+            __builtin_amdgcn_raw_buffer_store_b128(q, mx_rs, mx_lane + (unsigned)prow * (unsigned)(plane * (long)sizeof(double)), 0, 0);
+        }
+    };
     auto row_even = [&](int j, const E *u, double2 y, const double *pr) -> double2 {
         double2 acc = y;
 #pragma unroll
@@ -1897,6 +1944,7 @@
                 if (d < WT) { v.x += pr[d] * win[d].x; v.y += pr[d] * win[d].y; }
         }
         emit(j, v);
+        emit_mx(j, xj, [&](int d) { return win[d]; });
         return xj;
     };
     auto row_odd = [&](int j, const E *u, double2 y, double2 xprev, const double *pr) {
@@ -1915,6 +1963,7 @@
                 if (d - 1 < WT) { v.x += pr[d] * win[d - 1].x; v.y += pr[d] * win[d - 1].y; }
         }
         emit(j, v);
+        emit_mx(j, xj, [&](int d) { return d == 0 ? xprev : win[d > 0 ? d - 1 : 0]; });
 #pragma unroll
         for (int d = WT - 1; d > 1; --d) win[d] = win[d - 2];
         win[1] = xprev;
@@ -2465,8 +2514,38 @@
         for (int r = tid; r < L.nb; r += NT) store_sys<1>(yout, plane, L.colperm[L.n + r], P, c, 0, make_double2(0.0, 0.0));
 }
 
+__global__ void __launch_bounds__(256)
+flagged_matvec_tiled_kernel(PencilDev P, MatDev A, const long *__restrict__ cells, int ncellsf, const double *__restrict__ x,
+                            double *__restrict__ y) {
+    const long t = (long)blockIdx.x * blockDim.x + threadIdx.x;
+    if (t >= (long)A.nrows_out * ncellsf) return;
+    const int r = (int)(t % A.nrows_out);
+    const int t0 = A.rowptr[r], t1 = A.rowptr[r + 1];
+    if (t1 == t0) return;
+    const CellCtx c = cell_ctx(P, cells[t / A.nrows_out]);
+    const long xoff0 = state_cell(P, 2 * c.mx, 2 * c.my), xoff1 = state_cell(P, 2 * c.mx + 1, 2 * c.my);
+    double2 accP = make_double2(0.0, 0.0), accQ = accP;
+    for (int k = t0; k < t1; ++k) {
+        const unsigned e = A.expo[k];
+        const double f = term_factor(e, c);
+        const double2 cf = A.coef[k];
+        const double2 v = make_double2(cf.x * f, cf.y * f);
+        const double *xr = x + (long)A.col[k] * state_row_stride(P);
+        const double2 a = *reinterpret_cast<const double2 *>(xr + xoff0);
+        const double2 b = *reinterpret_cast<const double2 *>(xr + xoff1);
+        cfma(accP, v, make_double2(a.x - b.y, a.y + b.x));
+        const double sg = (e & 1u) ? -1.0 : 1.0;
+        cfma(accQ, make_double2(v.x * sg, v.y * sg), make_double2(a.x + b.y, a.y - b.x));
+    }
+    double *yr = y + (long)r * P.nx * P.ny;
+    *reinterpret_cast<double2 *>(yr + tile_offset(2 * c.mx, 2 * c.my, P.ny)) =
+        make_double2(0.5 * (accP.x + accQ.x), 0.5 * (accP.y + accQ.y));
+    *reinterpret_cast<double2 *>(yr + tile_offset(2 * c.mx + 1, 2 * c.my, P.ny)) =
+        make_double2(0.5 * (accP.y - accQ.y), 0.5 * (accQ.x - accP.x));
+}
+
 template <int NF>
-static int finish_solve(PencilPack *pp, LuFactor *lu, const RhsSrc &rhs, double *x, hipStream_t s, int apply_p) {
+static int finish_solve(PencilPack *pp, LuFactor *lu, const RhsSrc &rhs, double *x, hipStream_t s, int apply_p, int phase = 0) {
     const PencilDev &P = pp->dev;
     const LuDev &d = lu->dev;
     if (lu->nflag) {
@@ -2476,12 +2555,15 @@
         double2 *dx = drhs + (size_t)nsys * d.N;
         const long work = (long)lu->nflag * d.N * P.S;
         const unsigned gb = (unsigned)((work + 255) / 256);
-        hipLaunchKernelGGL(dense_gather_kernel<NF>, dim3(gb), dim3(256), 0, s, P, d, (const long *)lu->d_flag_cells,
-                           lu->nflag, rhs, drhs);
-        hipLaunchKernelGGL(dense_apply_kernel, dim3((unsigned)((d.N + 3) / 4), (unsigned)nsys), dim3(256), 0, s, d.N,
-                           (const double2 *)lu->d_inv, (const double2 *)drhs, dx);
-        hipLaunchKernelGGL(dense_scatter_kernel<NF>, dim3(gb), dim3(256), 0, s, P, d, (const long *)lu->d_flag_cells,
-                           lu->nflag, (const double2 *)dx, x, apply_p);
+        if (phase != 2)
+            hipLaunchKernelGGL(dense_gather_kernel<NF>, dim3(gb), dim3(256), 0, s, P, d, (const long *)lu->d_flag_cells,
+                               lu->nflag, rhs, drhs);
+        if (phase != 1) {
+            hipLaunchKernelGGL(dense_apply_kernel, dim3((unsigned)((d.N + 3) / 4), (unsigned)nsys), dim3(256), 0, s, d.N,
+                               (const double2 *)lu->d_inv, (const double2 *)drhs, dx);
+            hipLaunchKernelGGL(dense_scatter_kernel<NF>, dim3(gb), dim3(256), 0, s, P, d, (const long *)lu->d_flag_cells,
+                               lu->nflag, (const double2 *)dx, x, apply_p);
+        }
         DDH_HIP(hipGetLastError());
     }
     return 0;
@@ -2530,18 +2612,19 @@
     int bwd_w;
     int cb, tt;
     bool fuse_p;
+    bool emit_mx;
     dim3 fwd_grid, fwd_block, bwd_grid, bwd_block;
     size_t lds_f, lds_b;
     bool lean_forward() const { return fwd == FwdSweep::deep || fwd == FwdSweep::lean_occ4 || fwd == FwdSweep::lean; }
 };
 
-static SweepPlan sweep_plan(const PencilPack *pp, const LuDev &d, int nterms, bool want_p) {
+static SweepPlan sweep_plan(const PencilPack *pp, const LuDev &d, int nterms, bool want_p, bool want_mx = false) {
     const PencilDev &P = pp->dev;
     const int NF = P.nf, W = d.W;
     SweepPlan pl{};
     const size_t per_entry = d.pair ? 9 : 5;
     pl.lds_f = (size_t)(d.N + d.nb) * (per_entry + 1) + 16;
-    pl.lds_b = (size_t)(d.n > 0 ? d.n : 1) * (per_entry + 2) + 16;
+    pl.lds_b = (size_t)(d.n > 0 ? d.n : 1) * (per_entry + 4) + 16;
     const unsigned blocks = (unsigned)((P.G + 255) / 256);
     const long threads = (long)d.nsplit * d.Gp;
     const unsigned blocks_split = (unsigned)((threads + 255) / 256);
@@ -2619,6 +2702,8 @@
         } else {
             pl.bwd = BwdSweep::fused;
         }
+        pl.emit_mx = want_mx && pl.bwd != BwdSweep::deep && pl.bwd_w == 17 && !(P.nx & 7) && !(P.ny & 7) &&
+                     (double)P.nrows * (double)P.nx * (double)P.ny * 8.0 < 4294967296.0;
     } else {
         pl.bwd = BwdSweep::plain;
         pl.bwd_w = backward_window(W);
@@ -2628,9 +2713,13 @@
 }
 
 template <int NF>
-static int launch_solve(PencilPack *pp, LuFactor *lu, const RhsSrc &rhs, double *x, hipStream_t s, const SweepPlan &pl) {
+static int launch_solve(PencilPack *pp, LuFactor *lu, const RhsSrc &rhs, double *x, hipStream_t s, const SweepPlan &pl,
+                        int m_mat_id = -1, double *mx_out = nullptr) {
     const PencilDev &P = pp->dev;
     const LuDev &d = lu->dev;
+    const MxEmit mx{mx_out, (const double *)lu->d_mxband, (const short *)lu->d_mxrow};
+    const MxEmit nomx{nullptr, nullptr, nullptr};
+    if (pl.emit_mx && (!mx_out || !lu->mx_ok || m_mat_id < 0)) return fail("pencil_solve: M.X emission without its tables");
     if (pl.lds_f > 64 * 1024) return fail("pencil_solve: system too large for the LDS permutation cache");
     const int kl = pl.fwd_kl, nb = pl.fwd_nb, w = pl.bwd_w;
     switch (pl.fwd) {
@@ -2676,6 +2765,8 @@
     if constexpr (NF > 0)
         if (pl.border_finish)
             hipLaunchKernelGGL(border_finish_kernel<NF>, dim3((unsigned)((P.G + 255) / 256)), dim3(256), 0, s, P, d, x);
+    if (pl.emit_mx)
+        if (int st = finish_solve<NF>(pp, lu, rhs, x, s, 0, 1)) return st;
     switch (pl.bwd) {
         case BwdSweep::none:
             break;
@@ -2694,14 +2785,19 @@
                 hipLaunchKernelGGL((solve_backward_deep_kernel<17, 2>), pl.bwd_grid, pl.bwd_block, pl.lds_b, s, P, d, x, d.pband, rhs.skip);
             break;
         case BwdSweep::fused_occ4:
-            if constexpr (NF == 2)
-                hipLaunchKernelGGL((solve_backward_kernel<NF, 17, true, false, true, 4>), pl.bwd_grid, pl.bwd_block, pl.lds_b, s, P, d, x, d.pband, rhs.skip);
+            if constexpr (NF == 2) {
+                if (pl.emit_mx)
+                    hipLaunchKernelGGL((solve_backward_kernel<NF, 17, true, false, true, 4, true>), pl.bwd_grid, pl.bwd_block, pl.lds_b, s, P, d, x, d.pband, rhs.skip, mx);
+                else
+                    hipLaunchKernelGGL((solve_backward_kernel<NF, 17, true, false, true, 4>), pl.bwd_grid, pl.bwd_block, pl.lds_b, s, P, d, x, d.pband, rhs.skip, nomx);
+            }
             break;
         case BwdSweep::fused:
             if constexpr (NF == 2) {
                 auto k = w == 17 ? solve_backward_kernel<NF, 17, true, false, true> : w == 32 ? solve_backward_kernel<NF, 32, true, false, true>
                        : w == 34 ? solve_backward_kernel<NF, 34, true, false, true> : solve_backward_kernel<NF, 48, true, false, true>;
-                hipLaunchKernelGGL(k, pl.bwd_grid, pl.bwd_block, pl.lds_b, s, P, d, x, d.pband, rhs.skip);
+                if (pl.emit_mx) k = solve_backward_kernel<NF, 17, true, false, true, 1, true>;
+                hipLaunchKernelGGL(k, pl.bwd_grid, pl.bwd_block, pl.lds_b, s, P, d, x, d.pband, rhs.skip, pl.emit_mx ? mx : nomx);
             }
             break;
         case BwdSweep::plain: {
@@ -2712,12 +2808,23 @@
                 k = w == 17 ? solve_backward_kernel<NF, 17, false, false> : w == 32 ? solve_backward_kernel<NF, 32, false, false>
                   : w == 34 ? solve_backward_kernel<NF, 34, false, false> : w == 48 ? solve_backward_kernel<NF, 48, false, false>
                   : solve_backward_kernel<NF, 64, false, false>;
-            hipLaunchKernelGGL(k, pl.bwd_grid, pl.bwd_block, pl.lds_b, s, P, d, x, d.pband, rhs.skip);
+            hipLaunchKernelGGL(k, pl.bwd_grid, pl.bwd_block, pl.lds_b, s, P, d, x, d.pband, rhs.skip, nomx);
             break;
         }
     }
     DDH_HIP(hipGetLastError());
-    return finish_solve<NF>(pp, lu, rhs, x, s, pl.fuse_p ? 1 : 0);
+    if (!pl.emit_mx) return finish_solve<NF>(pp, lu, rhs, x, s, pl.fuse_p ? 1 : 0);
+    if (int st = finish_solve<NF>(pp, lu, rhs, x, s, 1, 2)) return st;
+    if constexpr (NF == 2) {
+        if (lu->nflag) {
+            const MatDev &A = pp->mats[m_mat_id]->dev;
+            const long work = (long)A.nrows_out * lu->nflag;
+            hipLaunchKernelGGL(flagged_matvec_tiled_kernel, dim3((unsigned)((work + 255) / 256)), dim3(256), 0, s, P, A,
+                               (const long *)lu->d_flag_cells, lu->nflag, (const double *)x, mx_out);
+            DDH_HIP(hipGetLastError());
+        }
+    }
+    return 0;
 }
 
 constexpr int LUW_ROWS = 32;
@@ -3419,6 +3526,42 @@
     return 0;
 }
 
+int ddh_pencil_set_mx_band(ddh_handle pack, int lu_id, int m_mat_id, int width, const int *step_row_h, const double *band_h) {
+    PencilPack *pp = (PencilPack *)lookup_handle(pack, H_PENCIL);
+    if (!pp) return -1;
+    if (lu_id < 0 || lu_id >= (int)pp->lus.size()) return fail("pencil_set_mx_band: bad LU id");
+    if (m_mat_id < 0 || m_mat_id >= (int)pp->mats.size()) return fail("pencil_set_mx_band: bad matrix id");
+    LuFactor *lu = pp->lus[lu_id];
+    const LuDev &d = lu->dev;
+    lu->mx_ok = 0;
+    lu->mx_mat = -1;
+    const int n = d.n, nh = d.nsplit > 1 ? d.nh : d.n;
+    if (width != MXW || !step_row_h || !band_h) return fail("pencil_set_mx_band: tables of width 18");
+    if (!d.real || n <= 0 || n > 32767) return fail("pencil_set_mx_band: a real-graded factorization with 1 .. 32767 band rows");
+    if (pp->mats[m_mat_id]->dev.nrows_out != d.N) return fail("pencil_set_mx_band: matrix and factorization differ in size");
+    std::vector<char> seen(n, 0);
+    std::vector<short> step_row(n);
+    for (int t = 0; t < n; ++t) {
+        const int i = step_row_h[t];
+        if (i < -1 || i >= n) return fail("pencil_set_mx_band: equation row outside the band rows");
+        if (i >= 0 && seen[i]++) return fail("pencil_set_mx_band: an equation row formed twice");
+        step_row[t] = (short)i;
+        for (int dd = 0; dd < MXW; ++dd) {
+            const double v = band_h[(size_t)t * MXW + dd];
+            if (v == 0.0) continue;
+            if (!(v == v) || i < 0 || t + dd >= n || (t + dd) / nh != t / nh)
+                return fail("pencil_set_mx_band: an entry without a row, beyond the band rows or outside the block of its step");
+        }
+    }
+    if (!lu->d_mxband) DDH_HIP(hipMalloc(&lu->d_mxband, (size_t)n * MXW * sizeof(double) + 16));
+    if (!lu->d_mxrow) DDH_HIP(hipMalloc(&lu->d_mxrow, (size_t)n * sizeof(short) + 16));
+    DDH_HIP(hipMemcpy(lu->d_mxband, band_h, (size_t)n * MXW * sizeof(double), hipMemcpyHostToDevice));
+    DDH_HIP(hipMemcpy(lu->d_mxrow, step_row.data(), (size_t)n * sizeof(short), hipMemcpyHostToDevice));
+    lu->mx_mat = m_mat_id;
+    lu->mx_ok = 1;
+    return 0;
+}
+
 int ddh_pencil_solve_recombined(ddh_handle pack, int lu_id, int nterms, const double *const *xs_h,
                                 const double *alpha_h, int p_mat_id, double *work, double *x, void *stream) {
     return ddh_pencil_solve_recombined_sparse(pack, lu_id, nterms, xs_h, alpha_h, p_mat_id, work, x, nullptr, nullptr, stream);
@@ -3426,7 +3569,8 @@
 
 static int solve_recombined_impl(ddh_handle pack, int lu_id, int nterms, const double *const *xs_h, const double *alpha_h,
                                  int p_mat_id, double *work, double *x, const unsigned char *zero_rows,
-                                 const unsigned char *skip_rows, int terms_tiled, void *stream);
+                                 const unsigned char *skip_rows, int terms_tiled, void *stream, int m_mat_id = -1,
+                                 double *mx_out = nullptr);
 
 int ddh_pencil_solve_recombined_sparse(ddh_handle pack, int lu_id, int nterms, const double *const *xs_h,
                                        const double *alpha_h, int p_mat_id, double *work, double *x,
@@ -3448,9 +3592,46 @@
     return solve_recombined_impl(pack, lu_id, nterms, xs_h, alpha_h, p_mat_id, work, x, zero_rows, skip_rows, 1, stream);
 }
 
+static int mx_emission(PencilPack *pp, LuFactor *lu, int p_mat_id, bool *emits) {
+    *emits = false;
+    if (pp->dev.nf != 2 || p_mat_id < 0 || p_mat_id >= (int)pp->mats.size()) return 0;
+    if (int st = build_pband(pp, lu, p_mat_id)) return st;
+    for (int nterms = 1; nterms <= RHS_MAX; ++nterms)
+        if (!sweep_plan(pp, lu->dev, nterms, true, true).emit_mx || !sweep_plan(pp, lu->dev, nterms, false).lean_forward()) return 0;
+    *emits = true;
+    return 0;
+}
+
+int ddh_pencil_lu_emits_mx(ddh_handle pack, int lu_id, int p_mat_id, int *emits) {
+    PencilPack *pp = (PencilPack *)lookup_handle(pack, H_PENCIL);
+    if (!pp) return -1;
+    if (lu_id < 0 || lu_id >= (int)pp->lus.size() || !emits) return fail("pencil_lu_emits_mx: bad LU id");
+    bool e = false;
+    if (int st = mx_emission(pp, pp->lus[lu_id], p_mat_id, &e)) return st;
+    *emits = e ? 1 : 0;
+    return 0;
+}
+
+int ddh_pencil_solve_recombined_tiled_mx(ddh_handle pack, int lu_id, int nterms, const double *const *xs_h,
+                                         const double *alpha_h, int p_mat_id, double *work, double *x,
+                                         const unsigned char *zero_rows, const unsigned char *skip_rows, int m_mat_id,
+                                         double *mx_out, void *stream) {
+    PencilPack *pp = (PencilPack *)lookup_handle(pack, H_PENCIL);
+    if (!pp) return -1;
+    if (lu_id < 0 || lu_id >= (int)pp->lus.size()) return fail("pencil_solve: bad LU id");
+    if (!mx_out || mx_out == x || mx_out == work) return fail("pencil_solve_recombined_tiled_mx: M.x needs a vector of its own");
+    bool e = false;
+    if (int st = mx_emission(pp, pp->lus[lu_id], p_mat_id, &e)) return st;
+    if (!e || !pp->lus[lu_id]->mx_ok || pp->lus[lu_id]->mx_mat != m_mat_id)
+        return fail("pencil_solve_recombined_tiled_mx: the sweeps of this factorization do not emit M.x "
+                    "(ddh_pencil_lu_emits_mx) or have no tables for this matrix (ddh_pencil_set_mx_band)");
+    return solve_recombined_impl(pack, lu_id, nterms, xs_h, alpha_h, p_mat_id, work, x, zero_rows, skip_rows, 1, stream,
+                                 m_mat_id, mx_out);
+}
+
 static int solve_recombined_impl(ddh_handle pack, int lu_id, int nterms, const double *const *xs_h, const double *alpha_h,
                                  int p_mat_id, double *work, double *x, const unsigned char *zero_rows,
-                                 const unsigned char *skip_rows, int terms_tiled, void *stream) {
+                                 const unsigned char *skip_rows, int terms_tiled, void *stream, int m_mat_id, double *mx_out) {
     PencilPack *pp = (PencilPack *)lookup_handle(pack, H_PENCIL);
     if (!pp) return -1;
     if (lu_id < 0 || lu_id >= (int)pp->lus.size()) return fail("pencil_solve: bad LU id");
@@ -3472,8 +3653,8 @@
     hipStream_t s = as_stream(stream);
     int st;
     if (pp->dev.nf == 2 && (st = build_pband(pp, lu, p_mat_id))) return st;
-    const SweepPlan pl = sweep_plan(pp, lu->dev, nterms, true);
-    if (pl.fuse_p) return launch_solve<2>(pp, lu, r, x, s, pl);
+    const SweepPlan pl = sweep_plan(pp, lu->dev, nterms, true, mx_out != nullptr);
+    if (pl.fuse_p) return launch_solve<2>(pp, lu, r, x, s, pl, m_mat_id, mx_out);
     r.skip = nullptr;
     if (pp->dev.nf == 1 && lu->d_binv && lu->dev.real && lu->dev.n == lu->dev.nsplit * lu->dev.nh) {
         const LuDev &d = lu->dev;
diff --git a/dedalus_amd/libhip.py b/dedalus_amd/libhip.py
--- a/dedalus_amd/libhip.py
+++ b/dedalus_amd/libhip.py
@@ -127,6 +127,9 @@
     "ddh_pencil_solve_recombined": [_h, _i, _i, C.POINTER(_vp), _dp, _i, _vp, _vp, _vp],
     "ddh_pencil_solve_recombined_sparse": [_h, _i, _i, C.POINTER(_vp), _dp, _i, _vp, _vp, _vp, _vp, _vp],
     "ddh_pencil_solve_recombined_tiled": [_h, _i, _i, C.POINTER(_vp), _dp, _i, _vp, _vp, _vp, _vp, _vp],
+    "ddh_pencil_solve_recombined_tiled_mx": [_h, _i, _i, C.POINTER(_vp), _dp, _i, _vp, _vp, _vp, _vp, _i, _vp, _vp],
+    "ddh_pencil_lu_emits_mx": [_h, _i, _i, _ip],
+    "ddh_pencil_set_mx_band": [_h, _i, _i, _i, _ip, _dp],
     "ddh_pencil_matvec_update_tiled": [_h, _i, _vp, _vp, _vp],
     "ddh_pencil_flagged": [_h, _i, _ip, C.POINTER(_l), _i],
     "ddh_pencil_set_dense_inverse": [_h, _i, _dp],
diff --git a/dedalus_amd/pencilpack.py b/dedalus_amd/pencilpack.py
--- a/dedalus_amd/pencilpack.py
+++ b/dedalus_amd/pencilpack.py
@@ -264,8 +264,17 @@
 
     supports_zero_rows = True
 
-    def solve_recombined(self, lu_id, xs, alphas, p_mat_id, work, x, zero_rows=None, skip_rows=None, tiled=False):
-        t = self._timer()
+    def solve_recombined(self, lu_id, xs, alphas, p_mat_id, work, x, zero_rows=None, skip_rows=None, tiled=False, mx=None):
+        t = self._timer()
+        if t is not None and mx is not None:
+            info = self.lu_info(lu_id)
+            read = 1.0 - (zero_rows[1] if (zero_rows is not None and info["forward"] == "lean") else 0.0)
+            wrote = 1.0 - (skip_rows[1] if skip_rows is not None else 0.0)
+            mrows = len(np.unique(np.asarray(self.matrices[mx[0]].row)))
+            nb = self.lu_bytes(lu_id) + (sum(v.numel() for v in xs) * read + x.numel() * wrote
+                                         + mx[1].numel() * mrows / float(self.nrows)) * 8
+            return t.run("pencil_solve", nb, self._solve_recombined, lu_id, xs, alphas, p_mat_id, work, x, zero_rows,
+                         skip_rows, tiled, mx)
         if t is not None:
             info = self.lu_info(lu_id)
             read = 1.0 - (zero_rows[1] if (zero_rows is not None and info["forward"] == "lean") else 0.0)
@@ -276,14 +285,20 @@
                 nb = binv + (sum(v.numel() for v in xs) + 3 * x.numel()) * 8
             return t.run("pencil_solve", nb, self._solve_recombined, lu_id, xs, alphas, p_mat_id, work, x, zero_rows,
                          skip_rows, tiled)
-        return self._solve_recombined(lu_id, xs, alphas, p_mat_id, work, x, zero_rows, skip_rows, tiled)
-
-    def _solve_recombined(self, lu_id, xs, alphas, p_mat_id, work, x, zero_rows=None, skip_rows=None, tiled=False):
+        return self._solve_recombined(lu_id, xs, alphas, p_mat_id, work, x, zero_rows, skip_rows, tiled, mx)
+
+    def _solve_recombined(self, lu_id, xs, alphas, p_mat_id, work, x, zero_rows=None, skip_rows=None, tiled=False, mx=None):
         arr = (C.c_void_p * len(xs))(*[C.c_void_p(v.data_ptr()) for v in xs])
         al = np.ascontiguousarray(alphas, dtype=np.float64)
         if zero_rows is not None or skip_rows is not None or tiled:
             zp = C.c_void_p(zero_rows[0].data_ptr()) if zero_rows is not None else None
             sp = C.c_void_p(skip_rows[0].data_ptr()) if skip_rows is not None else None
+            if mx is not None:
+                if not tiled:
+                    raise ValueError("M.x from the sweep needs tile-major terms")
+                libhip.call("ddh_pencil_solve_recombined_tiled_mx", self.handle, lu_id, len(xs), arr, libhip.as_dp(al),
+                            int(p_mat_id), ptr(work), ptr(x), zp, sp, int(mx[0]), ptr(mx[1]), self.dev.stream)
+                return
             libhip.call("ddh_pencil_solve_recombined_tiled" if tiled else "ddh_pencil_solve_recombined_sparse", self.handle,
                         lu_id, len(xs), arr, libhip.as_dp(al), int(p_mat_id), ptr(work), ptr(x), zp, sp, self.dev.stream)
             return
@@ -315,6 +330,19 @@
         d["forward"] = ("general", "lean", "cooperative")[d["forward"]]
         return d
 
+    def emits_mx(self, lu_id, p_mat_id):
+        if not hasattr(libhip.load(), "ddh_pencil_lu_emits_mx"):
+            return False
+        v = C.c_int(0)
+        libhip.call("ddh_pencil_lu_emits_mx", self.handle, int(lu_id), int(p_mat_id), C.byref(v))
+        return bool(v.value)
+
+    def set_mx_band(self, lu_id, m_mat_id, step_row, band):
+        sr = np.ascontiguousarray(step_row, dtype=np.int32)
+        bd = np.ascontiguousarray(band, dtype=np.float64)
+        libhip.call("ddh_pencil_set_mx_band", self.handle, int(lu_id), int(m_mat_id), int(bd.shape[1]), libhip.as_ip(sr),
+                    libhip.as_dp(bd))
+
     def lu_bytes(self, lu_id):
         n = C.c_size_t(0)
         libhip.call("ddh_pencil_lu_bytes", self.handle, lu_id, C.byref(n))
diff --git a/include/dedalus_hip.h b/include/dedalus_hip.h
--- a/include/dedalus_hip.h
+++ b/include/dedalus_hip.h
@@ -199,6 +199,12 @@
 int ddh_pencil_solve_recombined_tiled(ddh_handle pack, int lu_id, int nterms, const double *const *xs_h,
                                       const double *alpha_h, int p_mat_id, double *work, double *x,
                                       const unsigned char *zero_rows, const unsigned char *skip_rows, void *stream);
+int ddh_pencil_solve_recombined_tiled_mx(ddh_handle pack, int lu_id, int nterms, const double *const *xs_h,
+                                         const double *alpha_h, int p_mat_id, double *work, double *x,
+                                         const unsigned char *zero_rows, const unsigned char *skip_rows, int m_mat_id,
+                                         double *mx_out, void *stream);
+int ddh_pencil_lu_emits_mx(ddh_handle pack, int lu_id, int p_mat_id, int *emits);
+int ddh_pencil_set_mx_band(ddh_handle pack, int lu_id, int m_mat_id, int width, const int *step_row_h, const double *band_h);
 int ddh_pencil_set_row_blocks(ddh_handle pack, int nblocks);
 int ddh_pencil_flagged(ddh_handle pack, int lu_id, int *count, long *cells_h, int max_cells);
 int ddh_pencil_set_dense_inverse(ddh_handle pack, int lu_id, const double *inv_h);
```

Result: faster. 22.91 timesteps/sec (median of 6 runs) (+1.4%).
